# Sudaraka88/LDWeaver

Hardware: NVIDIA B200
Metric: weighted SNP-pair MI/sec (higher is better)
Workload: dtype int8 (tcgen05 kind::i8 with int32 accumulation of 28-bit fixed-point weights; fp32 MI epilogue, fp64 refinement of long-range links)

## Files before the change

include/ldw.h:

```cpp
#ifndef LDW_H
#define LDW_H

#include <stddef.h>
#include <stdint.h>

#ifdef __cplusplus
extern "C" {
#endif

#define LDW_ABI_VERSION 2

#if defined(__GNUC__)
#define LDW_API __attribute__((visibility("default")))
#else
#define LDW_API
#endif

enum {
  LDW_OK = 0,
  LDW_ERR_ARG = 1,
  LDW_ERR_CUDA = 2,
  LDW_ERR_NOMEM = 3,
  LDW_ERR_UNSUPPORTED = 4,
  LDW_ERR_INTERNAL = 5
};

enum {
  LDW_SCAN_SR_ONLY = 1,
  LDW_SCAN_IDEAL_Q = 2,
  LDW_SCAN_NO_LINKS = 4,
  LDW_SCAN_NO_D2H = 8,
  LDW_SCAN_SR_EXACT = 16,
  LDW_SCAN_SR_ON_DEVICE = 64,
  LDW_SCAN_LR_ONLY = 32
};

typedef struct ldw_ctx ldw_ctx;
typedef struct ldw_mi_plan ldw_mi_plan;

LDW_API int ldw_abi_version(void);
LDW_API const char* ldw_last_error(void);

LDW_API int ldw_create(int device, ldw_ctx** out);
LDW_API void ldw_destroy(ldw_ctx* ctx);
LDW_API int ldw_device_count(void);

LDW_API int ldw_aln_param(ldw_ctx* ctx, const uint8_t* aln, int64_t nseq, int64_t seq_len, int filter, double gap_thresh,
                  double maf_thresh, int32_t* pos_out, int64_t* n_snp_out, double* counts_out);
LDW_API int ldw_extract_snps(ldw_ctx* ctx, const uint8_t* aln, int64_t nseq, int64_t seq_len, const int32_t* pos,
                     int64_t n_snp, uint8_t* codes_out, double* table_out);
LDW_API int ldw_encode_alignment(ldw_ctx* ctx, const uint8_t* aln, int64_t nseq, int64_t seq_len, int filter, double gap_thresh,
                         double maf_thresh, int64_t* n_snp_out, int32_t** pos_out, uint8_t** codes_out, double** table_out);
LDW_API int ldw_read_fasta(const char* path, int64_t* nseq_out, int64_t* seq_len_out, uint8_t* aln_out, int64_t aln_cap,
                   char* names_out, int64_t names_cap);
LDW_API int ldw_read_fasta_alloc(const char* path, int64_t* nseq_out, int64_t* seq_len_out, uint8_t** aln_out, char** names_out,
                         int64_t* names_len_out);
LDW_API void ldw_buffer_free(void* p);

LDW_API int ldw_acgtn2num(ldw_ctx* ctx, double* nv, const char* ref, int64_t n);

LDW_API int ldw_hdw(ldw_ctx* ctx, const uint8_t* codes, int64_t n_snp, int64_t nseq, double threshold, int32_t* cnt_out,
            double* hdw_out, int32_t* dist_out);

typedef struct ldw_links {
  int64_t n;
  const int32_t* pos1;
  const int32_t* pos2;
  const int32_t* clust1;
  const int32_t* clust2;
  const int32_t* len;
  const double* MI;
  const int32_t* block;
} ldw_links;

typedef struct ldw_scan_stats {
  int64_t n_blocks;
  int64_t n_pairs;
  int64_t n_sr;
  int64_t n_lr_total;
  int64_t n_lr_kept;
  int64_t n_borderline;
  int64_t n_reruns;
  int64_t n_candidates;
  double t_pack_ms, t_scan_ms, t_select_ms, t_d2h_ms;
  double t_kernel_ms;
  int64_t n_scan_launches;
  int64_t n_launches;
  int64_t n_tiles;
  double exec_int8_ops;
  double t_host_prep_ms;
  double exec_mufu_ops;
  double eps_obs_max;
} ldw_scan_stats;

LDW_API int ldw_mi_plan_create(ldw_ctx* ctx, const uint8_t* codes, int64_t n_snp, int64_t nseq, const double* hdw,
                       const int32_t* pos, const int32_t* paint, int64_t blk, ldw_mi_plan** out);
LDW_API void ldw_mi_plan_destroy(ldw_mi_plan* plan);

LDW_API int ldw_mi_scan(ldw_mi_plan* plan, double g, double sr_dist, double lr_retain_links, double lr_links_approx,
                int flags, int n_parts, int part, ldw_links* sr_out, ldw_links* lr_out, ldw_links* borderline_out,
                double* thr_out, double* prob_out, ldw_scan_stats* stats_out);

LDW_API int ldw_write_lr_tsv(const char* path, const ldw_links* lr, int append);
LDW_API int ldw_format_r_real(double x, char* out, int cap);

typedef struct ldw_sr_post {
  int64_t n_df;
  const int32_t* clust_c;
  const int64_t* row;
  const double* srp_max;
  int64_t n_red;
  const int64_t* red;
  int64_t n_chk;
  const int64_t* chk;
  int32_t nclust;
  const int64_t* fit_off;
  const int32_t* fit_len;
  const double* fit_q95;
  const double* fit_val;
  const double* coef;
  const double* shape;
  const double* start;
  const int64_t* n_pos;
  const int32_t* nm_evals;
  const int32_t* nm_fail;
  void* priv;
} ldw_sr_post;
LDW_API int ldw_sr_postprocess(const ldw_links* sr, int32_t nclust, double sr_dist, double srp_cutoff, ldw_sr_post* out);
LDW_API void ldw_sr_post_free(ldw_sr_post* p);

LDW_API int ldw_sr_postprocess_dev(ldw_ctx* ctx, int32_t nclust, double sr_dist, double srp_cutoff, ldw_sr_post* out, ldw_links* df_rows_out);

LDW_API int ldw_nm_rosenbrock(const double* start, double* par_out, double* value_out, int* count_out);
LDW_API int ldw_neg_log_pbeta_upper(const double* x, int64_t n, double shape1, double shape2, double* out);

LDW_API int ldw_run_aracne(int64_t n_chk, const double* chk_pos1, const double* chk_pos2, const double* chk_MI, int64_t n_full,
                   const double* full_pos1, const double* full_pos2, const double* full_MI, uint8_t* aracne_out);

LDW_API int ldw_write_sr_tsv(const char* path, const ldw_links* sr, int64_t n, const int64_t* rows, const int32_t* clust_c,
                     const double* srp_max, const double* aracne, int append);

LDW_API int ldw_read_numeric_tsv(const char* path, int ncols, int64_t* nrows_out, double** cols_out);
LDW_API void ldw_table_free(double* cols);

LDW_API int ldw_links_to_cells(const int32_t* pos, int64_t n_snp, int64_t blk, const ldw_links* links, int32_t* from_local,
                       int32_t* to_local);

LDW_API int ldw_links_copy(const ldw_links* src, int32_t* pos1, int32_t* pos2, int32_t* clust1, int32_t* clust2, int32_t* len,
                   double* MI, int32_t* block);

LDW_API int ldw_mi_block_dense(ldw_mi_plan* plan, int64_t block_index, double* mi_out, int64_t* nf_out, int64_t* nt_out);

LDW_API int ldw_mi_pairs_exact(ldw_mi_plan* plan, int64_t block_index, const int32_t* from_local, const int32_t* to_local,
                       int64_t n_pairs, double* mi_out);

typedef struct ldw_group ldw_group;
#define LDW_GROUP_ID_BYTES 128
enum { LDW_HDW_FORCE_SHARD = 1 };
LDW_API int ldw_group_create(const int* devices, int n_devices, ldw_group** out);
LDW_API int ldw_group_unique_id(char* id_out );
LDW_API int ldw_group_create_rank(int device, int rank, int world, const char* id , ldw_group** out);
LDW_API void ldw_group_destroy(ldw_group* g);
LDW_API int ldw_group_info(const ldw_group* g, int* world_out, int* n_local_out, int* first_rank_out);
LDW_API ldw_ctx* ldw_group_ctx(ldw_group* g, int local_index);
LDW_API int ldw_group_load_codes(ldw_group* g, const uint8_t* codes, int64_t n_snp, int64_t nseq);
LDW_API int ldw_group_hdw(ldw_group* g, double threshold, int flags, int32_t* cnt_out, double* hdw_out, int* sharded_out);
LDW_API int ldw_group_mi_scan(ldw_group* g, const double* hdw, const int32_t* pos, const int32_t* paint, int64_t blk, double g_len,
                      double sr_dist, double lr_retain_links, double lr_links_approx, int flags, ldw_links* sr_out,
                      ldw_links* lr_out, ldw_links* borderline_out, double* thr_out, double* prob_out,
                      ldw_scan_stats* stats_out, double* t_plan_ms_out);

#ifdef __cplusplus
}
#endif
#endif
```

ldweaver_b200/_lib.py:

```python
from __future__ import annotations

import ctypes as C
import os

import numpy as np

_HERE = os.path.dirname(os.path.abspath(__file__))
LIB_PATH = os.environ.get("LDW_LIBRARY_PATH") or os.path.join(_HERE, "libldwgpu.so")

i64 = C.c_int64
f64 = C.c_double
P = C.POINTER


class LdwError(RuntimeError):
    def __init__(self, code: int, msg: str):
        super().__init__(f"libldwgpu error {code}: {msg}")
        self.code = code


class Links(C.Structure):
    _fields_ = [("n", i64), ("pos1", P(C.c_int32)), ("pos2", P(C.c_int32)), ("clust1", P(C.c_int32)),
                ("clust2", P(C.c_int32)), ("len", P(C.c_int32)), ("MI", P(f64)), ("block", P(C.c_int32))]

    @classmethod
    def from_dict(cls, d: dict):
        self = cls()
        keep = {}
        for name, dt, ct in (("pos1", np.int32, C.c_int32), ("pos2", np.int32, C.c_int32), ("clust1", np.int32, C.c_int32),
                             ("clust2", np.int32, C.c_int32), ("len", np.int32, C.c_int32), ("MI", np.float64, f64),
                             ("block", np.int32, C.c_int32)):
            a = np.ascontiguousarray(d[name] if name in d else np.zeros(len(d["MI"]), dtype=dt), dtype=dt)
            keep[name] = a
            setattr(self, name, a.ctypes.data_as(P(ct)))
        self.n = len(keep["MI"])
        self._keep = keep
        return self

    def views(self) -> dict:
        if hasattr(self, "_keep"):
            return self._keep
        n = int(self.n)
        out = {}
        for name, _ in self._fields_[1:]:
            ptr = getattr(self, name)
            if n and ptr:
                out[name] = np.ctypeslib.as_array(ptr, shape=(n,))
        return out

    def to_dict(self) -> dict:
        n = int(self.n)
        cols = (("pos1", np.int32), ("pos2", np.int32), ("clust1", np.int32), ("clust2", np.int32), ("len", np.int32),
                ("MI", np.float64), ("block", np.int32))
        out = {name: np.empty(n if (n and getattr(self, name)) else 0, dtype=dt) for name, dt in cols}
        if n:
            dst = [out[name].ctypes.data_as(C.c_void_p) if len(out[name]) else None for name, _ in cols]
            check(lib().ldw_links_copy(C.byref(self), *dst))
        return out


class ScanStats(C.Structure):
    _fields_ = [("n_blocks", i64), ("n_pairs", i64), ("n_sr", i64), ("n_lr_total", i64), ("n_lr_kept", i64),
                ("n_borderline", i64), ("n_reruns", i64), ("n_candidates", i64), ("t_pack_ms", f64), ("t_scan_ms", f64), ("t_select_ms", f64),
                ("t_d2h_ms", f64), ("t_kernel_ms", f64), ("n_scan_launches", i64), ("n_launches", i64), ("n_tiles", i64),
                ("exec_int8_ops", f64), ("t_host_prep_ms", f64), ("exec_mufu_ops", f64), ("eps_obs_max", f64)]

    def to_dict(self) -> dict:
        return {k: getattr(self, k) for k, _ in self._fields_}


class SrPost(C.Structure):
    _fields_ = [("n_df", i64), ("clust_c", P(C.c_int32)), ("row", P(i64)), ("srp_max", P(f64)),
                ("n_red", i64), ("red", P(i64)), ("n_chk", i64), ("chk", P(i64)), ("nclust", C.c_int32),
                ("fit_off", P(i64)), ("fit_len", P(C.c_int32)), ("fit_q95", P(f64)), ("fit_val", P(f64)),
                ("coef", P(f64)), ("shape", P(f64)), ("start", P(f64)), ("n_pos", P(i64)), ("nm_evals", P(C.c_int32)),
                ("nm_fail", P(C.c_int32)), ("priv", C.c_void_p)]


def copy_array(ptr, n: int, dtype) -> np.ndarray:
    if n == 0 or not ptr:
        return np.zeros(0, dtype=dtype)
    return np.ctypeslib.as_array(ptr, shape=(n,)).astype(dtype, copy=True)


_lib = None


def lib():
    global _lib
    if _lib is not None:
        return _lib
    if not os.path.exists(LIB_PATH):
        raise ImportError(f"{LIB_PATH} not found: build it with `python -c 'import __graft_entry__ as g; g.build()'`. "
                          "ldweaver_b200 has no CPU fallback.")
    L = C.CDLL(LIB_PATH)
    L.ldw_last_error.restype = C.c_char_p
    L.ldw_create.argtypes = [C.c_int, P(C.c_void_p)]
    L.ldw_destroy.argtypes = [C.c_void_p]
    L.ldw_destroy.restype = None
    L.ldw_aln_param.argtypes = [C.c_void_p, C.c_void_p, i64, i64, C.c_int, f64, f64, C.c_void_p, P(i64), C.c_void_p]
    L.ldw_extract_snps.argtypes = [C.c_void_p, C.c_void_p, i64, i64, C.c_void_p, i64, C.c_void_p, C.c_void_p]
    L.ldw_encode_alignment.argtypes = [C.c_void_p, C.c_void_p, i64, i64, C.c_int, f64, f64, P(i64), P(C.c_void_p), P(C.c_void_p),
                                       P(C.c_void_p)]
    L.ldw_read_fasta.argtypes = [C.c_char_p, P(i64), P(i64), C.c_void_p, i64, C.c_void_p, i64]
    L.ldw_read_fasta_alloc.argtypes = [C.c_char_p, P(i64), P(i64), P(C.c_void_p), P(C.c_void_p), P(i64)]
    L.ldw_buffer_free.argtypes = [C.c_void_p]
    L.ldw_buffer_free.restype = None
    L.ldw_acgtn2num.argtypes = [C.c_void_p, C.c_void_p, C.c_char_p, i64]
    L.ldw_hdw.argtypes = [C.c_void_p, C.c_void_p, i64, i64, f64, C.c_void_p, C.c_void_p, C.c_void_p]
    L.ldw_mi_plan_create.argtypes = [C.c_void_p, C.c_void_p, i64, i64, C.c_void_p, C.c_void_p, C.c_void_p, i64,
                                     P(C.c_void_p)]
    L.ldw_mi_plan_destroy.argtypes = [C.c_void_p]
    L.ldw_mi_plan_destroy.restype = None
    L.ldw_mi_scan.argtypes = [C.c_void_p, f64, f64, f64, f64, C.c_int, C.c_int, C.c_int, P(Links), P(Links), P(Links),
                              C.c_void_p, C.c_void_p, P(ScanStats)]
    L.ldw_mi_block_dense.argtypes = [C.c_void_p, i64, C.c_void_p, P(i64), P(i64)]
    L.ldw_write_lr_tsv.argtypes = [C.c_char_p, P(Links), C.c_int]
    L.ldw_format_r_real.argtypes = [f64, C.c_char_p, C.c_int]
    L.ldw_sr_postprocess.argtypes = [P(Links), C.c_int32, f64, f64, P(SrPost)]
    L.ldw_sr_postprocess_dev.argtypes = [C.c_void_p, C.c_int32, f64, f64, P(SrPost), P(Links)]
    L.ldw_sr_post_free.argtypes = [P(SrPost)]
    L.ldw_sr_post_free.restype = None
    L.ldw_run_aracne.argtypes = [i64, C.c_void_p, C.c_void_p, C.c_void_p, i64, C.c_void_p, C.c_void_p, C.c_void_p, C.c_void_p]
    L.ldw_write_sr_tsv.argtypes = [C.c_char_p, P(Links), i64, C.c_void_p, C.c_void_p, C.c_void_p, C.c_void_p, C.c_int]
    L.ldw_read_numeric_tsv.argtypes = [C.c_char_p, C.c_int, P(i64), P(P(f64))]
    L.ldw_table_free.argtypes = [P(f64)]
    L.ldw_table_free.restype = None
    L.ldw_links_to_cells.argtypes = [C.c_void_p, i64, i64, P(Links), C.c_void_p, C.c_void_p]
    L.ldw_links_copy.argtypes = [P(Links)] + [C.c_void_p] * 7
    L.ldw_nm_rosenbrock.argtypes = [C.c_void_p, C.c_void_p, P(f64), P(C.c_int)]
    L.ldw_neg_log_pbeta_upper.argtypes = [C.c_void_p, i64, f64, f64, C.c_void_p]
    L.ldw_mi_pairs_exact.argtypes = [C.c_void_p, i64, C.c_void_p, C.c_void_p, i64, C.c_void_p]
    L.ldw_group_create.argtypes = [C.c_void_p, C.c_int, P(C.c_void_p)]
    L.ldw_group_unique_id.argtypes = [C.c_char_p]
    L.ldw_group_create_rank.argtypes = [C.c_int, C.c_int, C.c_int, C.c_char_p, P(C.c_void_p)]
    L.ldw_group_destroy.argtypes = [C.c_void_p]
    L.ldw_group_destroy.restype = None
    L.ldw_group_info.argtypes = [C.c_void_p, P(C.c_int), P(C.c_int), P(C.c_int)]
    L.ldw_group_ctx.argtypes = [C.c_void_p, C.c_int]
    L.ldw_group_ctx.restype = C.c_void_p
    L.ldw_group_load_codes.argtypes = [C.c_void_p, C.c_void_p, i64, i64]
    L.ldw_group_hdw.argtypes = [C.c_void_p, f64, C.c_int, C.c_void_p, C.c_void_p, P(C.c_int)]
    L.ldw_group_mi_scan.argtypes = [C.c_void_p, C.c_void_p, C.c_void_p, C.c_void_p, i64, f64, f64, f64, f64, C.c_int,
                                    P(Links), P(Links), P(Links), C.c_void_p, C.c_void_p, C.c_void_p, P(f64)]
    _lib = L
    return L


_nccl_preloaded = False


def preload_nccl() -> None:
    global _nccl_preloaded
    if _nccl_preloaded:
        return
    _nccl_preloaded = True
    try:
        import importlib.util
        spec = importlib.util.find_spec("nvidia.nccl")
        for base in (spec.submodule_search_locations if spec and spec.submodule_search_locations else []):
            so = os.path.join(base, "lib", "libnccl.so.2")
            if os.path.exists(so):
                C.CDLL(so, mode=C.RTLD_GLOBAL)
                return
    except Exception:
        pass


def check(rc: int) -> None:
    if rc != 0:
        raise LdwError(rc, lib().ldw_last_error().decode(errors="replace"))


def ptr(a: np.ndarray):
    return a.ctypes.data_as(C.c_void_p)


class Context:

    def __init__(self, device: int = 0):
        self.handle = C.c_void_p()
        check(lib().ldw_create(device, C.byref(self.handle)))
        self.device = device

    def close(self):
        if self.handle:
            lib().ldw_destroy(self.handle)
            self.handle = C.c_void_p()

    def __del__(self):
        try:
            self.close()
        except Exception:
            pass


_default_ctx = {}


def default_context(device: int = 0) -> Context:
    if device not in _default_ctx:
        _default_ctx[device] = Context(device)
    return _default_ctx[device]
```

ldweaver_b200/api.py:

```python
from __future__ import annotations

import ctypes as C
import os
import warnings
from dataclasses import dataclass
from typing import List, Optional, Sequence

import numpy as np

from . import _lib
from ._lib import check, ptr

ALLELES = "ACGTN"


@dataclass
class SnpDat:
    codes: np.ndarray
    g: Optional[int]
    nsnp: int
    nseq: int
    seq_names: List[str]
    r: np.ndarray
    uqe: np.ndarray
    POS: np.ndarray

    def snp_matrix(self, allele: str):
        import scipy.sparse as sp
        return sp.csc_matrix(self.codes == ALLELES.index(allele))

    @property
    def snp_matrix_A(self): return self.snp_matrix("A")
    @property
    def snp_matrix_C(self): return self.snp_matrix("C")
    @property
    def snp_matrix_G(self): return self.snp_matrix("G")
    @property
    def snp_matrix_T(self): return self.snp_matrix("T")
    @property
    def snp_matrix_N(self): return self.snp_matrix("N")


def _method_to_filter(method: str) -> int:
    if method == "default":
        return 0
    if method == "relaxed":
        return 1
    warnings.warn("Unkown filtering method, using default...")
    return 0


class _LibraryBuffer:

    def __init__(self, addr: int, nbytes: int):
        self._addr = addr
        self.__array_interface__ = {"data": (addr, False), "shape": (nbytes,), "typestr": "|u1", "version": 3}

    def __del__(self):
        try:
            _lib.lib().ldw_buffer_free(self._addr)
        except Exception:
            pass


def read_fasta_matrix(aln_path: str):
    L = _lib.lib()
    nseq, slen, nlen = C.c_int64(), C.c_int64(), C.c_int64()
    aln_p, names_p = C.c_void_p(), C.c_void_p()
    check(L.ldw_read_fasta_alloc(os.fsencode(aln_path), C.byref(nseq), C.byref(slen), C.byref(aln_p), C.byref(names_p), C.byref(nlen)))
    try:
        raw = C.string_at(names_p, nlen.value) if names_p else b""
    finally:
        L.ldw_buffer_free(names_p)
    owner = _LibraryBuffer(aln_p.value, nseq.value * max(slen.value, 0)) if aln_p else None
    if slen.value == -1:
        raise ValueError("Error! sequences are of different lengths!")
    if nseq.value == 0:
        raise ValueError("File does not contain any sequences!")
    if owner is None:
        aln = np.empty((nseq.value, 0), dtype=np.uint8)
    else:
        aln = np.asarray(owner).reshape(nseq.value, slen.value)
    name_list = raw.split(b"\0")[:nseq.value]
    return [n.decode(errors="replace") for n in name_list], aln


def _build_snp_dat(aln: np.ndarray, names: Sequence[str], filt: int, gap_freq: float, maf_freq: float,
                   pos: Optional[np.ndarray], device: int) -> SnpDat:
    L = _lib.lib()
    ctx = _lib.default_context(device)
    aln = np.ascontiguousarray(aln, dtype=np.uint8)
    nseq, slen = aln.shape
    n_snp = C.c_int64()
    pos_p, codes_p, table_p = C.c_void_p(), C.c_void_p(), C.c_void_p()
    check(L.ldw_encode_alignment(ctx.handle, ptr(aln), nseq, slen, filt, gap_freq, maf_freq, C.byref(n_snp), C.byref(pos_p),
                                 C.byref(codes_p), C.byref(table_p)))
    n = int(n_snp.value)
    if n == 0:
        raise ValueError("File does not contain any SNPs")
    if pos is not None and len(pos) != slen:
        for p_ in (pos_p, codes_p, table_p):
            L.ldw_buffer_free(p_)
        raise ValueError("Error! Number of positions do not match the fasta sequence length")
    try:
        pos_idx = np.frombuffer(C.string_at(pos_p, n * 4), dtype=np.int32).copy()
        table = np.frombuffer(C.string_at(table_p, n * 5 * 8), dtype=np.float64).copy()
    finally:
        L.ldw_buffer_free(pos_p)
        L.ldw_buffer_free(table_p)
    codes = np.asarray(_LibraryBuffer(codes_p.value, n * nseq)).reshape(n, nseq)
    table = table.reshape(n, 5)
    uqe = (table > 0).astype(np.float64)
    if pos is None:
        POS, g = pos_idx.astype(np.int32), int(slen)
    else:
        POS, g = np.asarray(pos)[pos_idx.astype(np.int64) - 1].astype(np.int32), None
    return SnpDat(codes=codes, g=g, nsnp=n, nseq=int(nseq), seq_names=[s.lstrip(">") for s in names],
                  r=uqe.sum(axis=1), uqe=uqe, POS=POS)


def parse_fasta_alignment(aln_path: str, gap_freq: float = 0.15, maf_freq: float = 0.01, method: str = "default",
                          mega_dset: bool = False, device: int = 0) -> SnpDat:
    aln_path = os.path.abspath(os.path.expanduser(aln_path))
    if not os.path.exists(aln_path):
        raise FileNotFoundError(f"Can't locate file {aln_path}")
    filt = _method_to_filter(method)
    names, aln = read_fasta_matrix(aln_path)
    return _build_snp_dat(aln, names, filt, gap_freq, maf_freq, None, device)


def parse_fasta_SNP_alignment(aln_path: str, pos: Sequence[int], gap_freq: float = 0.15, maf_freq: float = 0.01,
                              method: str = "default", mega_dset: bool = False, device: int = 0) -> SnpDat:
    aln_path = os.path.abspath(os.path.expanduser(aln_path))
    if not os.path.exists(aln_path):
        raise FileNotFoundError(f"Can't locate file {aln_path}")
    filt = _method_to_filter(method)
    names, aln = read_fasta_matrix(aln_path)
    return _build_snp_dat(aln, names, filt, gap_freq, maf_freq, np.asarray(pos), device)


def snp_dat_from_alignment_matrix(aln: np.ndarray, names: Optional[Sequence[str]] = None, pos=None, gap_freq=0.15,
                                  maf_freq=0.01, method="default", device: int = 0) -> SnpDat:
    names = list(names) if names is not None else [f"s{i}" for i in range(aln.shape[0])]
    return _build_snp_dat(aln, names, _method_to_filter(method), gap_freq, maf_freq,
                          None if pos is None else np.asarray(pos), device)


def snp_dat_from_codes(codes: np.ndarray, POS: np.ndarray, g: Optional[int], seq_names=None) -> SnpDat:
    codes = np.ascontiguousarray(codes, dtype=np.uint8)
    nsnp, nseq = codes.shape
    uqe = np.stack([(codes == a).any(axis=1) for a in range(5)], axis=1).astype(np.float64)
    return SnpDat(codes=codes, g=g, nsnp=nsnp, nseq=nseq, seq_names=list(seq_names) if seq_names is not None else
                  [f"s{i}" for i in range(nseq)], r=uqe.sum(axis=1), uqe=uqe, POS=np.asarray(POS, dtype=np.int32))


def acgtn2num(nv: np.ndarray, cv, ncores: int = 1, device: int = 0) -> None:
    if not (nv.dtype == np.float64 and nv.flags["F_CONTIGUOUS"] and nv.shape[0] == 5):
        raise ValueError("nv must be a Fortran-ordered float64 [5, n] matrix (R column-major)")
    ref = "".join((c[0] if len(c) else " ") for c in cv).encode("latin-1") if not isinstance(cv, (bytes, bytearray)) else bytes(cv)
    if len(ref) != nv.shape[1]:
        raise ValueError("cv length does not match ncol(nv)")
    ctx = _lib.default_context(device)
    check(_lib.lib().ldw_acgtn2num(ctx.handle, ptr(nv), ref, nv.shape[1]))


def estimate_Hamming_distance_weights(snp_dat: SnpDat, threshold: float = 0.1, mega_dset: bool = False,
                                      device: int = 0, return_parts: bool = False, devices: Optional[Sequence[int]] = None):
    if devices is None and not return_parts:
        devices = devices_from_env()
    if devices is not None and len(devices) > 1:
        if return_parts:
            raise ValueError("the distance matrix (return_parts) is a single-device output")
        grp = default_group(devices)
        grp.load_codes(snp_dat.codes)
        return grp.hdw(threshold)
    ctx = _lib.default_context(device)
    codes = np.ascontiguousarray(snp_dat.codes, dtype=np.uint8)
    n, S = codes.shape
    cnt = np.empty(S, dtype=np.int32)
    hdw = np.empty(S, dtype=np.float64)
    dist = np.empty((S, S), dtype=np.int32, order="F") if return_parts else None
    check(_lib.lib().ldw_hdw(ctx.handle, ptr(codes), n, S, float(threshold), ptr(cnt), ptr(hdw),
                             ptr(dist) if return_parts else None))
    if return_parts:
        return hdw, cnt, dist
    return hdw


SCAN_SR_ONLY, SCAN_IDEAL_Q, SCAN_NO_LINKS, SCAN_NO_D2H, SCAN_SR_EXACT, SCAN_LR_ONLY, SCAN_SR_ON_DEVICE = 1, 2, 4, 8, 16, 32, 64


@dataclass
class CdsVar:
    paint: np.ndarray
    nclust: int


@dataclass
class MIScanResult:
    sr: dict
    lr: dict
    borderline: dict
    nclust: int
    thr: np.ndarray
    prob: np.ndarray
    stats: dict
    lr_links_approx: Optional[float]
    sr_links_red: Optional[dict] = None
    sr_post: Optional["SrLinks"] = None
    _by_cluster: Optional[List[np.ndarray]] = None

    @property
    def sr_links(self) -> List[np.ndarray]:
        if self._by_cluster is None:
            self._by_cluster = [np.nonzero((self.sr["clust1"] == c) | (self.sr["clust2"] == c))[0]
                                for c in range(1, self.nclust + 1)]
        return self._by_cluster


def round_half_even_thousands(x: float) -> int:
    return int(np.round(x / 1000.0) * 1000)


def make_blocks(nsnp: int, max_blk_sz: int):
    import math
    p = int(math.ceil(nsnp / max_blk_sz))
    fs = [(i - 1) * max_blk_sz + 1 for i in range(1, p + 1)]
    fe = [min(i * max_blk_sz, nsnp) for i in range(1, p + 1)]
    return [(fs[i], fe[i], fs[j], fe[j]) for i in range(p) for j in range(i, p)]


def partition_blocks(nsnp: int, blk: int, n_parts: int, part: int) -> List[int]:
    if n_parts < 1 or not (0 <= part < n_parts):
        raise ValueError("bad partition")
    items = []
    for idx, (fs, fe, ts, te) in enumerate(make_blocks(nsnp, blk)):
        ni, nj = fe - fs + 1, te - ts + 1
        items.append((ni * (ni - 1) // 2 if fs == ts else ni * nj, idx))
    load = [0] * n_parts
    owner = {}
    for cost, idx in sorted(items, key=lambda t: (-t[0], t[1])):
        best = min(range(n_parts), key=lambda p: (load[p], p))
        owner[idx] = best
        load[best] += cost
    return [idx for _, idx in items if owner[idx] == part]


def sr_pair_indices(pos: np.ndarray, blk: int, sr: dict):
    pos = np.asarray(pos)
    blocks = make_blocks(len(pos), blk)
    b = np.asarray(sr["block"])
    n = len(b)
    links = _lib.Links.from_dict({"pos1": sr["pos1"], "pos2": sr["pos2"], "block": b, "MI": np.zeros(n)})
    pos32 = np.ascontiguousarray(pos, dtype=np.int32)
    il, jl = np.zeros(n, dtype=np.int32), np.zeros(n, dtype=np.int32)
    check(_lib.lib().ldw_links_to_cells(ptr(pos32), len(pos32), int(blk), C.byref(links), ptr(il), ptr(jl)))
    if n == 0 or np.all(b[1:] >= b[:-1]):
        order = None
        bounds = np.searchsorted(b, np.arange(len(blocks) + 1))
    else:
        order = np.argsort(b, kind="stable")
        bounds = np.searchsorted(b[order], np.arange(len(blocks) + 1))
    for k in range(len(blocks)):
        if bounds[k + 1] > bounds[k]:
            idx = slice(int(bounds[k]), int(bounds[k + 1])) if order is None else order[bounds[k]:bounds[k + 1]]
            yield k, idx, il[idx], jl[idx]


class MIPlan:

    def __init__(self, snp_dat: SnpDat, hdw: np.ndarray, paint: np.ndarray, blk: int, device: int = 0):
        self.ctx = _lib.default_context(device)
        self.codes = np.ascontiguousarray(snp_dat.codes, dtype=np.uint8)
        self.hdw = np.ascontiguousarray(hdw, dtype=np.float64)
        self.pos = np.ascontiguousarray(snp_dat.POS, dtype=np.int32)
        self.paint = np.ascontiguousarray(paint, dtype=np.int32)
        n, S = self.codes.shape
        if len(self.hdw) != S or len(self.pos) != n or len(self.paint) != n:
            raise ValueError("snp.dat / hdw / cds_var size mismatch")
        self.n, self.S, self.blk = n, S, int(blk)
        self.handle = C.c_void_p()
        check(_lib.lib().ldw_mi_plan_create(self.ctx.handle, ptr(self.codes), n, S, ptr(self.hdw), ptr(self.pos),
                                            ptr(self.paint), int(blk), C.byref(self.handle)))
        nr = -(-n // self.blk)
        self.n_blocks = nr * (nr + 1) // 2

    def close(self):
        if self.handle:
            _lib.lib().ldw_mi_plan_destroy(self.handle)
            self.handle = C.c_void_p()

    def __del__(self):
        try:
            self.close()
        except Exception:
            pass

    def scan(self, g: float, sr_dist: float, lr_retain_links: float, lr_links_approx: float, flags: int = 0,
             n_parts: int = 1, part: int = 0, copy: bool = True):
        sr, lr, bd = _lib.Links(), _lib.Links(), _lib.Links()
        thr = np.full(self.n_blocks, np.nan)
        prob = np.full(self.n_blocks, np.nan)
        st = _lib.ScanStats()
        check(_lib.lib().ldw_mi_scan(self.handle, float(g), float(sr_dist), float(lr_retain_links),
                                     float(lr_links_approx if lr_links_approx else 0.0), int(flags), int(n_parts), int(part),
                                     C.byref(sr), C.byref(lr), C.byref(bd), ptr(thr), ptr(prob), C.byref(st)))
        if copy:
            return sr.to_dict(), lr.to_dict(), bd.to_dict(), thr, prob, st.to_dict()
        return sr, lr, bd, thr, prob, st.to_dict()

    def sr_exact(self, sr: dict, inplace: bool = False) -> np.ndarray:
        mi = sr["MI"]
        if inplace and isinstance(mi, np.ndarray) and mi.dtype == np.float64 and mi.flags.c_contiguous and mi.flags.writeable:
            out = mi
        else:
            out = np.array(mi, dtype=np.float64, copy=True)
        for k, idx, il, jl in sr_pair_indices(self.pos, self.blk, sr):
            if isinstance(idx, slice):
                self.pairs_exact(k, il, jl, out=out[idx])
            else:
                out[idx] = self.pairs_exact(k, il, jl)
        return out

    def block_dense(self, block_index: int) -> np.ndarray:
        nf, nt = C.c_int64(), C.c_int64()
        check(_lib.lib().ldw_mi_block_dense(self.handle, block_index, None, C.byref(nf), C.byref(nt)))
        out = np.zeros((nf.value, nt.value), dtype=np.float64, order="F")
        check(_lib.lib().ldw_mi_block_dense(self.handle, block_index, ptr(out), C.byref(nf), C.byref(nt)))
        return out

    def pairs_exact(self, block_index: int, from_local: np.ndarray, to_local: np.ndarray, out: Optional[np.ndarray] = None) -> np.ndarray:
        f = np.ascontiguousarray(from_local, dtype=np.int32)
        t = np.ascontiguousarray(to_local, dtype=np.int32)
        if out is None:
            out = np.zeros(len(f), dtype=np.float64)
        elif not (out.dtype == np.float64 and out.flags.c_contiguous and out.flags.writeable and out.shape == (len(f),)):
            raise ValueError("out must be a writeable C-contiguous float64 array with one element per pair")
        check(_lib.lib().ldw_mi_pairs_exact(self.handle, block_index, ptr(f), ptr(t), len(f), ptr(out)))
        return out


def _format_r(x) -> str:
    x = float(x)
    if x != x:
        return "NA"
    if x in (float("inf"), float("-inf")):
        return "Inf" if x > 0 else "-Inf"
    if x == 0:
        return "0"
    m, e = f"{x:.14e}".split("e")
    neg = m.startswith("-")
    digits = m.lstrip("-").replace(".", "").rstrip("0") or "0"
    nsig, k = len(digits), int(e)
    left, rgt = (k + 1, max(0, nsig - k - 1)) if k >= 0 else (1, nsig - k - 1)
    if 0 < k <= 22 and abs(x) < 10.0 ** k:
        left -= 1
    w_fixed = neg + left + (rgt + 1 if rgt else 0)
    w_sci = neg + (nsig + 1 if nsig > 1 else 1) + (5 if abs(k) >= 100 else 4)
    return f"{x:.{rgt}f}" if w_fixed <= w_sci else f"{x:.{nsig - 1}e}"


def format_r_real_native(x: float) -> str:
    buf = C.create_string_buffer(512)
    check(_lib.lib().ldw_format_r_real(float(x), buf, 512))
    return buf.value.decode()


def write_lr_tsv(path: str, lr, append: bool = True) -> None:
    links = lr if isinstance(lr, _lib.Links) else _lib.Links.from_dict(lr)
    check(_lib.lib().ldw_write_lr_tsv(os.fsencode(path), C.byref(links), 1 if append else 0))


class DeviceGroup:

    def __init__(self, devices: Sequence[int]):
        devs = np.ascontiguousarray(list(devices), dtype=np.int32)
        self.handle = C.c_void_p()
        if len(devs) > 1:
            _lib.preload_nccl()
        check(_lib.lib().ldw_group_create(ptr(devs), len(devs), C.byref(self.handle)))
        self._after_create()

    def _after_create(self):
        w, nl, fr = C.c_int(), C.c_int(), C.c_int()
        check(_lib.lib().ldw_group_info(self.handle, C.byref(w), C.byref(nl), C.byref(fr)))
        self.world, self.n_local, self.first_rank = w.value, nl.value, fr.value
        self.n_snp = self.nseq = 0

    @staticmethod
    def unique_id() -> bytes:
        buf = C.create_string_buffer(128)
        _lib.preload_nccl()
        check(_lib.lib().ldw_group_unique_id(buf))
        return buf.raw

    @classmethod
    def from_rank(cls, device: int, rank: int, world: int, unique_id: Optional[bytes]):
        self = cls.__new__(cls)
        self.handle = C.c_void_p()
        _lib.preload_nccl()
        check(_lib.lib().ldw_group_create_rank(int(device), int(rank), int(world), unique_id, C.byref(self.handle)))
        self._after_create()
        return self

    def close(self):
        if getattr(self, "handle", None):
            _lib.lib().ldw_group_destroy(self.handle)
            self.handle = C.c_void_p()

    def __del__(self):
        try:
            self.close()
        except Exception:
            pass

    def load_codes(self, codes: Optional[np.ndarray], n_snp: Optional[int] = None, nseq: Optional[int] = None) -> None:
        if codes is not None:
            codes = np.ascontiguousarray(codes, dtype=np.uint8)
            n_snp, nseq = codes.shape
        check(_lib.lib().ldw_group_load_codes(self.handle, ptr(codes) if codes is not None else None, int(n_snp), int(nseq)))
        self.n_snp, self.nseq = int(n_snp), int(nseq)

    def hdw(self, threshold: float = 0.1, force_shard: bool = False, return_parts: bool = False):
        cnt = np.empty(self.nseq, dtype=np.int32)
        w = np.empty(self.nseq, dtype=np.float64)
        sharded = C.c_int()
        check(_lib.lib().ldw_group_hdw(self.handle, float(threshold), 1 if force_shard else 0, ptr(cnt), ptr(w), C.byref(sharded)))
        return (w, cnt, bool(sharded.value)) if return_parts else w

    def mi_scan(self, hdw, pos, paint, blk: int, g: float, sr_dist: float, lr_retain_links: float, lr_links_approx: float,
                flags: int = 0, copy: bool = True):
        hdw = np.ascontiguousarray(hdw, dtype=np.float64)
        pos = np.ascontiguousarray(pos, dtype=np.int32)
        paint = np.ascontiguousarray(paint, dtype=np.int32)
        if len(hdw) != self.nseq or len(pos) != self.n_snp or len(paint) != self.n_snp:
            raise ValueError("hdw / POS / paint do not match the matrix given to load_codes")
        nr = -(-self.n_snp // int(blk))
        nblk = nr * (nr + 1) // 2
        sr, lr, bd = _lib.Links(), _lib.Links(), _lib.Links()
        thr, prob = np.full(nblk, np.nan), np.full(nblk, np.nan)
        stats = (_lib.ScanStats * self.n_local)()
        t_plan = _lib.f64()
        check(_lib.lib().ldw_group_mi_scan(self.handle, ptr(hdw), ptr(pos), ptr(paint), int(blk), float(g), float(sr_dist),
                                           float(lr_retain_links), float(lr_links_approx if lr_links_approx else 0.0), int(flags),
                                           C.byref(sr), C.byref(lr), C.byref(bd), ptr(thr), ptr(prob), stats, C.byref(t_plan)))
        st = [s_.to_dict() for s_ in stats]
        for d in st:
            d["t_plan_ms"] = t_plan.value
        if copy:
            return sr.to_dict(), lr.to_dict(), bd.to_dict(), thr, prob, st
        return sr, lr, bd, thr, prob, st


_groups = {}


def default_group(devices: Sequence[int]) -> DeviceGroup:
    key = tuple(int(d) for d in devices)
    if key not in _groups:
        _groups[key] = DeviceGroup(key)
    return _groups[key]


def devices_from_env() -> Optional[List[int]]:
    v = os.environ.get("LDW_GPUS", "").strip()
    if not v:
        return None
    if "," in v:
        return [int(x) for x in v.split(",") if x.strip() != ""]
    n = int(v)
    return list(range(n)) if n > 1 else None


@dataclass
class SrLinks:
    df: dict
    red: np.ndarray
    chk: np.ndarray
    fits: List[dict]
    borderline_red: Optional[np.ndarray] = None
    borderline_chk: Optional[np.ndarray] = None


def _unpack_sr_post(out, nclust: int, cols: dict, row_is_position: bool, plt_path: Optional[str], srp_cutoff: float) -> SrLinks:
    cp = _lib.copy_array
    row = cp(out.row, out.n_df, np.int64)
    df = {"clust_c": cp(out.clust_c, out.n_df, np.int32), "row": row, "srp_max": cp(out.srp_max, out.n_df, np.float64)}
    for k in ("pos1", "pos2", "clust1", "clust2", "len", "MI"):
        df[k] = np.array(cols[k], copy=True) if row_is_position else np.asarray(cols[k])[row]
    off = cp(out.fit_off, nclust + 1, np.int64)
    nfit = int(off[-1])
    fl, fq, fv = cp(out.fit_len, nfit, np.int32), cp(out.fit_q95, nfit, np.float64), cp(out.fit_val, nfit, np.float64)
    coef, shape, start = (cp(x, 2 * nclust, np.float64).reshape(nclust, 2) for x in (out.coef, out.shape, out.start))
    npos, ev, fail = cp(out.n_pos, nclust, np.int64), cp(out.nm_evals, nclust, np.int32), cp(out.nm_fail, nclust, np.int32)
    fits = [dict(len=fl[off[c]:off[c + 1]], max=fq[off[c]:off[c + 1]], fit=fv[off[c]:off[c + 1]], coef=coef[c],
                 shape=shape[c], start=start[c], n_pos=int(npos[c]), nm_evals=int(ev[c]), nm_fail=int(fail[c]))
            for c in range(nclust)]
    if plt_path is not None:
        os.makedirs(plt_path, exist_ok=True)
        for c, f in enumerate(fits, start=1):
            with open(os.path.join(plt_path, f"c{c}_fit_data.tsv"), "w") as fh:
                fh.write("len\tmax\tfit\n")
                fh.writelines(f"{int(a)}\t{b:.15g}\t{v:.15g}\n" for a, b, v in zip(f["len"], f["max"], f["fit"]))
    red, chk = cp(out.red, out.n_red, np.int64), cp(out.chk, out.n_chk, np.int64)
    b_red = np.nonzero(np.abs(df["srp_max"] - srp_cutoff) <= 1e-9 * max(abs(float(srp_cutoff)), 1.0))[0]
    b_chk = np.nonzero(np.abs(df["MI"] - df["MI"][red].min()) <= 1e-12)[0] if len(red) else np.zeros(0, np.int64)
    return SrLinks(df=df, red=red, chk=chk, fits=fits, borderline_red=b_red, borderline_chk=b_chk)


def mergeNsort_sr_links(cds_var, sr_links, sr_dist: float, plt_path: Optional[str] = None, srp_cutoff: float = 3) -> SrLinks:
    nclust = int(cds_var.nclust if hasattr(cds_var, "nclust") else cds_var["nclust"])
    links = sr_links if isinstance(sr_links, _lib.Links) else _lib.Links.from_dict(sr_links)
    out = _lib.SrPost()
    check(_lib.lib().ldw_sr_postprocess(C.byref(links), nclust, float(sr_dist), float(srp_cutoff), C.byref(out)))
    try:
        return _unpack_sr_post(out, nclust, links.views(), False, plt_path, srp_cutoff)
    finally:
        _lib.lib().ldw_sr_post_free(C.byref(out))


def mergeNsort_sr_links_device(cds_var, sr_dist: float, plt_path: Optional[str] = None, srp_cutoff: float = 3, device: int = 0) -> SrLinks:
    nclust = int(cds_var.nclust if hasattr(cds_var, "nclust") else cds_var["nclust"])
    ctx = _lib.default_context(device)
    out, rows = _lib.SrPost(), _lib.Links()
    check(_lib.lib().ldw_sr_postprocess_dev(ctx.handle, nclust, float(sr_dist), float(srp_cutoff), C.byref(out), C.byref(rows)))
    try:
        return _unpack_sr_post(out, nclust, rows.views() if int(rows.n) else {k: np.zeros(0) for k in ("pos1", "pos2", "clust1", "clust2", "len", "MI")},
                               True, plt_path, srp_cutoff)
    finally:
        _lib.lib().ldw_sr_post_free(C.byref(out))


def runARACNE(links_to_check, links_full) -> np.ndarray:
    f64 = lambda a: np.ascontiguousarray(np.asarray(a), dtype=np.float64)
    c1, c2, cm = f64(links_to_check["pos1"]), f64(links_to_check["pos2"]), f64(links_to_check["MI"])
    p1, p2, pm = f64(links_full["pos1"]), f64(links_full["pos2"]), f64(links_full["MI"])
    out = np.ones(len(c1), dtype=np.uint8)
    check(_lib.lib().ldw_run_aracne(len(c1), ptr(c1), ptr(c2), ptr(cm), len(p1), ptr(p1), ptr(p2), ptr(pm), ptr(out)))
    return out.astype(bool)


def write_sr_tsv(path: str, sr, rows: np.ndarray, clust_c: np.ndarray, srp_max: np.ndarray, aracne: np.ndarray,
                 append: bool = True) -> None:
    links = sr if isinstance(sr, _lib.Links) else _lib.Links.from_dict(sr)
    rows = np.ascontiguousarray(rows, dtype=np.int64)
    cc = np.ascontiguousarray(clust_c, dtype=np.int32)
    sp = np.ascontiguousarray(srp_max, dtype=np.float64)
    ar = np.ascontiguousarray(aracne, dtype=np.float64)
    check(_lib.lib().ldw_write_sr_tsv(os.fsencode(path), C.byref(links), len(rows), ptr(rows), ptr(cc), ptr(sp), ptr(ar),
                                      1 if append else 0))


def _read_numeric_tsv(path: str, names: Sequence[str]) -> dict:
    n, cols = _lib.i64(0), _lib.P(_lib.f64)()
    check(_lib.lib().ldw_read_numeric_tsv(os.fsencode(path), len(names), C.byref(n), C.byref(cols)))
    try:
        flat = _lib.copy_array(cols, int(n.value) * len(names), np.float64).reshape(len(names), int(n.value))
    finally:
        _lib.lib().ldw_table_free(cols)
    return {k: flat[i] for i, k in enumerate(names)}


def read_LongRangeLinks(lr_links_path: str, links_from_spydrpick: bool = False, sr_dist: float = 20000) -> dict:
    if links_from_spydrpick:
        tab = np.loadtxt(lr_links_path, dtype=np.float64, ndmin=2)
        names = {5: ["pos1", "pos2", "len", "ARACNE", "MI"], 4: ["pos1", "pos2", "len", "MI"]}.get(tab.shape[1])
        if names is None:
            raise ValueError(f"spydrpick link files have 4 or 5 columns, {lr_links_path} has {tab.shape[1]}")
        d = {k: np.ascontiguousarray(tab[:, i]) for i, k in enumerate(names)}
    else:
        d = _read_numeric_tsv(lr_links_path, ["pos1", "pos2", "c1", "c2", "len", "MI"])
    keep = ~(d["len"] < sr_dist)
    return {k: v[keep] for k, v in d.items()} if not keep.all() else d


def read_ShortRangeLinks(sr_links_path: str) -> dict:
    return _read_numeric_tsv(sr_links_path, ["clust_c", "pos1", "pos2", "clust1", "clust2", "len", "MI", "srp_max", "ARACNE"])


def _quantile7(x: np.ndarray, prob: float) -> float:
    n = len(x)
    index = 1 + max(n - 1, 0) * prob
    lo, hi = int(np.floor(index)), int(np.ceil(index))
    part = np.partition(x, sorted({lo - 1, hi - 1}))
    qs = float(part[lo - 1])
    if index > lo and part[hi - 1] != qs:
        h = index - lo
        qs = (1 - h) * qs + h * float(part[hi - 1])
    return qs


def analyse_long_range_links(lr_links: dict, sr_links: dict, are_lrlinks_ordered: bool = False) -> dict:
    mi = np.asarray(lr_links["MI"], dtype=np.float64)
    q1, q3 = _quantile7(mi, 0.25), _quantile7(mi, 0.75)
    thresholds = q3 + np.array([1.5, 3.0]) * (q3 - q1)
    red = mi > thresholds.min()
    if red.sum() < 5000 and len(mi) >= 5000:
        import warnings
        warnings.warn("Not enough lr links pass the Tukey criteria, ~5000 top links were retained instead")
        thresholds = np.array([_quantile7(mi, 1 - (1 / len(mi) * k)) for k in (4000, 5000)])
        red = mi > thresholds.min()
    out = {k: np.asarray(v)[red] for k, v in lr_links.items()}
    if "ARACNE" not in lr_links:
        chk = {k: np.concatenate([np.asarray(lr_links[k], dtype=np.float64), np.asarray(sr_links[k], dtype=np.float64)])
               for k in ("pos1", "pos2", "MI")}
        m = chk["MI"] > thresholds.min()
        out["ARACNE"] = runARACNE(out, {k: v[m] for k, v in chk.items()})
    if not are_lrlinks_ordered:
        o = np.argsort(-out["MI"], kind="stable")
        out = {k: v[o] for k, v in out.items()}
    out["thresholds"] = thresholds
    return out


def finish_sr_links(sr: Optional[dict], cds_var, sr_dist: float, srp_cutoff: float = 3, run_aracne: bool = True,
                    order_links: bool = True, sr_save_path: Optional[str] = None, plt_folder: Optional[str] = None,
                    post: Optional[SrLinks] = None):
    if post is None:
        post = mergeNsort_sr_links(cds_var, sr, sr_dist, plt_folder, srp_cutoff)
    red = {k: v[post.red] for k, v in post.df.items()}
    if run_aracne:
        chk = {k: post.df[k][post.chk] for k in ("pos1", "pos2", "MI")}
        red["ARACNE"] = runARACNE(red, chk).astype(np.float64)
    else:
        import warnings
        warnings.warn("ARACNE not run, all values will be set to 1")
        red["ARACNE"] = np.ones(len(post.red))
    if order_links:
        o = np.argsort(-red["srp_max"], kind="stable")
        red = {k: v[o] for k, v in red.items()}
    if sr_save_path is not None:
        write_sr_tsv(sr_save_path, red, np.arange(len(red["row"]), dtype=np.int64), red["clust_c"], red["srp_max"], red["ARACNE"], append=True)
    return red, post


def perform_MI_computation(snp_dat: SnpDat, hdw: np.ndarray, cds_var, ncores: int = 1, lr_save_path: Optional[str] = None,
                           sr_save_path: Optional[str] = None, plt_folder: Optional[str] = None, sr_dist: float = 20000,
                           lr_retain_links: float = 1e6, max_blk_sz: float = 10000, srp_cutoff: float = 3,
                           runARACNE: bool = True, perform_SR_analysis_only: bool = False, order_links: bool = True,
                           mega_dset: bool = False, lr_links_approx: Optional[float] = None, device: int = 0,
                           write_tsv: bool = True, plan: Optional[MIPlan] = None,
                           postprocess: Optional[bool] = None, exact_sr: Optional[bool] = None,
                           devices: Optional[Sequence[int]] = None, scan_flags: int = 0,
                           device_post: bool = False) -> MIScanResult:
    if snp_dat.g is None:
        raise ValueError("snp.dat$g is NULL: set the genome length first (R/BacGWES.R:338-345)")
    paint = np.asarray(cds_var.paint if hasattr(cds_var, "paint") else cds_var["paint"])
    nclust = int(cds_var.nclust if hasattr(cds_var, "nclust") else cds_var["nclust"])
    if lr_save_path is None:
        lr_save_path = os.path.join(os.getcwd(), "lr_links.tsv")
    blk = round_half_even_thousands(max_blk_sz)
    if not perform_SR_analysis_only and lr_links_approx is None:
        from .rrng import lr_links_approx as _lra
        lr_links_approx = _lra(np.asarray(snp_dat.POS), float(snp_dat.g), float(sr_dist))
    if devices is None and plan is None:
        devices = devices_from_env()
    multi = devices is not None and len(devices) > 1
    do_post = postprocess if postprocess is not None else write_tsv
    if multi:
        grp = default_group(devices)
        grp.load_codes(snp_dat.codes)
        flags = (SCAN_SR_ONLY if perform_SR_analysis_only else 0) | int(scan_flags)
        if exact_sr is None:
            exact_sr = do_post
        if exact_sr:
            flags |= SCAN_SR_EXACT
        sr, lr, bd, thr, prob, st_list = grp.mi_scan(hdw, snp_dat.POS, paint, blk, float(snp_dat.g), sr_dist, lr_retain_links,
                                                     lr_links_approx or 0.0, flags)
        stats = dict(st_list[0])
        for k in ("n_blocks", "n_pairs", "n_sr", "n_lr_total", "n_lr_kept", "n_borderline", "n_reruns", "n_candidates",
                  "n_scan_launches", "n_launches", "n_tiles", "exec_int8_ops", "exec_mufu_ops"):
            stats[k] = sum(d[k] for d in st_list)
        for k in ("t_pack_ms", "t_scan_ms", "t_select_ms", "t_d2h_ms", "t_kernel_ms", "t_host_prep_ms"):
            stats[k] = max(d[k] for d in st_list)
        stats["per_device"] = st_list
        return _finish_mi_computation(sr, lr, bd, thr, prob, stats, nclust, lr_links_approx, cds_var, sr_dist, srp_cutoff,
                                      runARACNE, order_links, write_tsv, do_post, lr_save_path, sr_save_path, plt_folder)
    own = plan is None
    import time as _time
    t_phase = {}
    _t0 = _time.perf_counter()
    if own:
        plan = MIPlan(snp_dat, hdw, paint, blk, device)
    t_phase["plan_create_s"] = _time.perf_counter() - _t0
    try:
        flags = (SCAN_SR_ONLY if perform_SR_analysis_only else 0) | int(scan_flags)
        if exact_sr is None:
            exact_sr = ("in_scan" if perform_SR_analysis_only else True) if do_post else False
        if device_post and do_post:
            flags |= SCAN_SR_ON_DEVICE
            if exact_sr:
                exact_sr = "in_scan"
        if exact_sr == "in_scan":
            flags |= SCAN_SR_EXACT
            exact_sr = False
        _t0 = _time.perf_counter()
        sr, lr, bd, thr, prob, stats = plan.scan(float(snp_dat.g), sr_dist, lr_retain_links, lr_links_approx or 0.0, flags, copy=False)
        t_phase["scan_call_s"] = _time.perf_counter() - _t0
        _t0 = _time.perf_counter()
        sr, lr, bd = sr.to_dict(), lr.to_dict(), bd.to_dict()
        t_phase["copy_links_s"] = _time.perf_counter() - _t0
        if exact_sr:
            if perform_SR_analysis_only:
                raise ValueError("exact_sr is not available with perform_SR_analysis_only")
            _t0 = _time.perf_counter()
            sr["MI"] = plan.sr_exact(sr, inplace=True)
            t_phase["exact_sr_host_driven_s"] = _time.perf_counter() - _t0
    finally:
        if own:
            plan.close()
    stats["phases"] = t_phase
    post = None
    if device_post and do_post:
        _t0 = _time.perf_counter()
        post = mergeNsort_sr_links_device(cds_var, sr_dist, plt_folder, srp_cutoff, device)
        t_phase["sr_post_device_s"] = _time.perf_counter() - _t0
    return _finish_mi_computation(sr, lr, bd, thr, prob, stats, nclust, lr_links_approx, cds_var, sr_dist, srp_cutoff,
                                  runARACNE, order_links, write_tsv, do_post, lr_save_path, sr_save_path, plt_folder, post)


def _finish_mi_computation(sr, lr, bd, thr, prob, stats, nclust, lr_links_approx, cds_var, sr_dist, srp_cutoff, run_aracne,
                           order_links, write_tsv, do_post, lr_save_path, sr_save_path, plt_folder, post=None) -> MIScanResult:
    import time as _time
    ph = stats.setdefault("phases", {})
    _t0 = _time.perf_counter()
    if write_tsv and len(lr["MI"]):
        write_lr_tsv(lr_save_path, lr, append=True)
    ph["write_lr_tsv_s"] = _time.perf_counter() - _t0
    _t0 = _time.perf_counter()
    res = MIScanResult(sr=sr, lr=lr, borderline=bd, nclust=nclust, thr=thr, prob=prob, stats=stats,
                       lr_links_approx=lr_links_approx)
    if do_post:
        if write_tsv and sr_save_path is None:
            sr_save_path = os.path.join(os.getcwd(), "sr_links.tsv")
        res.sr_links_red, res.sr_post = finish_sr_links(sr, cds_var, sr_dist, srp_cutoff, run_aracne, order_links,
                                                        sr_save_path if write_tsv else None, plt_folder, post)
    ph["finish_sr_links_s"] = _time.perf_counter() - _t0
    return res
```

ldweaver_b200/csrc/mi_kernel.cuh:

```cuda
#pragma once
#include "mi_types.h"
#include "umma.cuh"

namespace ldw {

constexpr int MI_EXP_WARPS = 6;
constexpr int MI_EXP_THREADS = 32 * MI_EXP_WARPS;
constexpr int MI_EPI_WARP0 = 8;
constexpr int MI_EPI_GROUPS = 4;
constexpr int MI_EPI_WARPS = 4 * MI_EPI_GROUPS;
constexpr int MI_EPI_THREADS = 32 * MI_EPI_WARPS;
constexpr int MI_THREADS = 32 * (MI_EPI_WARP0 + MI_EPI_WARPS);
#define LDW_STR2(x) #x
#define LDW_STR(x) LDW_STR2(x)
#define MI_REGS_CTRL 48
#define MI_REGS_EPI 96
static_assert(MI_EPI_WARP0 * 32 * MI_REGS_CTRL + MI_EPI_THREADS * MI_REGS_EPI <= MI_THREADS * ((65536 / MI_THREADS) & ~7), "register budget");
constexpr int MI_MAX_STAGES = 4;
constexpr uint32_t MI_ARR_BYTES = 128 * 128;
constexpr uint32_t MI_STAGE_REGION = 12 * MI_ARR_BYTES;
__host__ __device__ constexpr uint32_t mi_stage_need(int pa, int pb, int njlog2) {
  return (uint32_t)pa * MI_ARR_BYTES + 4u * (uint32_t)pb * (64u << njlog2);
}
__host__ __device__ constexpr int mi_stage_geo(int pa, int pb, int njlog2) {
  return mi_stage_need(pa, pb, njlog2) <= 3 * MI_ARR_BYTES ? 0 : mi_stage_need(pa, pb, njlog2) <= 4 * MI_ARR_BYTES ? 1 : 2;
}
__host__ __device__ constexpr int mi_geo_stages(int geo) { return 4 - geo; }
__host__ __device__ constexpr uint32_t mi_geo_bytes(int geo) { return geo == 0 ? 3 * MI_ARR_BYTES : geo == 1 ? 4 * MI_ARR_BYTES : 6 * MI_ARR_BYTES; }
constexpr uint32_t MI_JREC_BYTES = 128 * sizeof(Rec);
constexpr uint32_t MI_JDYN_BYTES = 128 * sizeof(ColDyn);
constexpr uint32_t MI_IREC_BYTES = 128 * sizeof(Rec);
constexpr uint32_t MI_IDYN_BYTES = 128 * sizeof(RowDyn);
constexpr uint32_t MI_BAR_BYTES = 512;
constexpr uint32_t MI_SMEM_BYTES = MI_STAGE_REGION + 2 * (MI_JREC_BYTES + MI_JDYN_BYTES) + MI_IREC_BYTES + MI_IDYN_BYTES + MI_BAR_BYTES + 1024;
static_assert(MI_SMEM_BYTES <= 232448, "shared memory budget (227 KB opt-in)");

__device__ __forceinline__ float lg2_fast(float x) {
  float y;
  asm("lg2.approx.ftz.f32 %0, %1;" : "=f"(y) : "f"(x));
  return y;
}
__device__ __forceinline__ uint32_t ld_volatile_u32(const uint32_t* p) {
  uint32_t v;
  asm volatile("ld.volatile.global.u32 %0, [%1];" : "=r"(v) : "l"(p));
  return v;
}

__host__ __device__ constexpr int mi_jc(int pa, int pb) {
  return (pa + 1) * (pb + 1) <= 4 ? 8 : (pa + 1) * (pb + 1) <= 9 ? 4 : (pa + 1) * (pb + 1) <= 12 ? 2 : 1;
}
__host__ __device__ constexpr int mi_njlog2(int pa, int pb) {
  return pa * pb == 1 ? 7 : pa * pb == 2 ? 6 : pa * pb <= 4 ? 5 : 4;
}

__device__ __noinline__ void lr_raise_threshold(const ScanParams& p, int lane) {
  constexpr int PER = MI_HIST_BINS / 32;
  uint32_t s = 0;
  for (int k = 0; k < PER; k++) s += ld_volatile_u32(p.hist + lane * PER + k);
  uint32_t suf = s;
#pragma unroll
  for (int o = 1; o < 32; o <<= 1) {
    uint32_t v = __shfl_down_sync(0xffffffffu, suf, o);
    if (lane + o < 32) suf += v;
  }
  unsigned m = __ballot_sync(0xffffffffu, suf >= p.kprime);
  if (m == 0) return;
  int sel = 31 - __clz(m);
  if (lane == sel) {
    uint32_t run = suf - s;
    for (int k = PER - 1; k >= 0; k--) {
      run += ld_volatile_u32(p.hist + lane * PER + k);
      if (run >= p.kprime) {
        atomicMax(p.tcand_bits, (uint32_t)(lane * PER + k) << 19);
        break;
      }
    }
  }
}

template <bool DBG>
__device__ __forceinline__ void timed_wait(uint64_t* bar, uint32_t parity, int tag, long long& acc) {
  if constexpr (DBG) {
    long long c0 = clock64();
    mbar_wait(bar, parity, tag);
    acc += clock64() - c0;
  } else {
    mbar_wait(bar, parity, tag);
  }
}

struct EpiCtx {
  int q, cg, lane, rank;
  uint32_t tflags;
  uint32_t tmem_base;
  uint32_t jrec_saddr;
  uint32_t jdyn_saddr;
  uint32_t irec_saddr, idyn_saddr;
  uint32_t rempty_saddr;
  uint32_t scr_saddr;
};

__device__ __forceinline__ uint4 lds128(uint32_t saddr) {
  uint4 v;
  asm volatile("ld.shared.v4.u32 {%0, %1, %2, %3}, [%4];" : "=r"(v.x), "=r"(v.y), "=r"(v.z), "=r"(v.w) : "r"(saddr));
  return v;
}

__device__ __forceinline__ uint2 lds64(uint32_t saddr) {
  uint2 v;
  asm volatile("ld.shared.v2.u32 {%0, %1}, [%2];" : "=r"(v.x), "=r"(v.y) : "r"(saddr));
  return v;
}

__device__ __forceinline__ void sts128(uint32_t saddr, uint4 v) {
  asm volatile("st.shared.v4.u32 [%0], {%1, %2, %3, %4};" ::"r"(saddr), "r"(v.x), "r"(v.y), "r"(v.z), "r"(v.w) : "memory");
}

__device__ __forceinline__ float rcp_fast(float x) {
  float y;
  asm("rcp.approx.ftz.f32 %0, %1;" : "=f"(y) : "f"(x));
  return y;
}

template <bool QC>
__device__ __forceinline__ float mi_term(float acc, uint32_t t, float ra, float rb, float dq) {
  const float x = __uint2float_rn(t);
  const float ratio = QC ? x * rcp_fast(fmaf(ra, rb, dq)) : x * (ra * rb);
  return fmaf(x, lg2_fast(ratio), acc);
}

template <bool QC, int NB>
__device__ __forceinline__ float mi_row(float acc, const uint32_t (&t)[NB], float ra, const float (&rb)[NB], float dq) {
  if constexpr (!QC) {
#pragma unroll
    for (int b = 0; b < NB; b++) acc = mi_term<false>(acc, t[b], ra, rb[b], dq);
    return acc;
  } else {
    float d[NB], inv[NB];
#pragma unroll
    for (int b = 0; b < NB; b++) d[b] = fmaf(ra, rb[b], dq);
#pragma unroll
    for (int b = 0; b + 1 < NB; b += 2) {
      const float r = rcp_fast(d[b] * d[b + 1]);
      inv[b] = r * d[b + 1];
      inv[b + 1] = r * d[b];
    }
    if (NB & 1) inv[NB - 1] = rcp_fast(d[NB - 1]);
#pragma unroll
    for (int b = 0; b < NB; b++) {
      const float x = __uint2float_rn(t[b]);
      acc = fmaf(x, lg2_fast(x * inv[b]), acc);
    }
    return acc;
  }
}

__device__ __noinline__ void lr_emit(const ScanParams& p, bool em, int il, int jl, float mi, int lane) {
  const unsigned bal = __ballot_sync(0xffffffffu, em);
  if (bal == 0) return;
  const int leader = __ffs(bal) - 1;
  uint32_t base = 0;
  const uint32_t n_new = (uint32_t)__popc(bal);
  if (lane == leader) base = atomicAdd(p.cand_count, n_new);
  base = __shfl_sync(0xffffffffu, base, leader);
  if (em) {
    uint32_t idx = base + (uint32_t)__popc(bal & ((1u << lane) - 1));
    if (idx < p.cand_cap) {
      Cand cc;
      cc.il = il; cc.jl = jl; cc.mi = mi;
      p.cand[idx] = cc;
    } else {
      *p.overflow = 1;
    }
    uint32_t bits = __float_as_uint(mi);
    atomicAdd(p.hist + ((bits & 0x80000000u) ? 0u : (bits >> 19)), 1u);
  }
  if (!p.emit_all && (base / p.delta) != ((base + n_new) / p.delta)) {
    __threadfence();
    lr_raise_threshold(p, lane);
  }
}

__device__ __noinline__ void sr_store(float* sr_out, uint4 d0, uint4 d1, int il, int jl, float mi) {
  const int a0 = (int)d0.z, a1 = (int)d0.w, b0 = (int)d1.x, b1 = (int)d1.y;
  const int la = a1 - a0, lb = b1 - b0;
  int below = min(max(il - a0, 0), la) + min(max(il - b0, 0), lb);
  uint32_t slot;
  if (il < jl) {
    slot = d1.z + (uint32_t)below;
  } else {
    int bj = min(max(jl + 1 - a0, 0), la) + min(max(jl + 1 - b0, 0), lb);
    slot = d1.w + (uint32_t)(below - bj);
  }
  sr_out[slot] = mi;
}

template <int RA>
struct TileRegs {
  uint32_t Ti[RA];
  float rpad[RA];
  float scale, q0, qod, rtlq, tcand;
  uint32_t mul_a, sb, jl_lim, M;
  int il, nf, nt;
  bool ragged, dense, do_lr, has_sr;
  float* sr_out;
};

template <int PA, int PB, int JC>
__device__ __forceinline__ void epi_load(uint32_t tmem_base, int NJ, int j0, uint32_t (&H)[PA][PB][JC],
                                         uint32_t (&L)[PA][PB][JC]) {
  const int NJh = NJ >> 1;
  const int half = j0 >= NJh ? 1 : 0;
  const uint32_t base = tmem_base + (uint32_t)(half * PB * NJ + (j0 - half * NJh));
#pragma unroll
  for (int a = 0; a < PA; a++)
#pragma unroll
    for (int b = 0; b < PB; b++) {
      tmem_ldn<JC>(base + (uint32_t)(a * 2 * PB * NJ + b * NJh), H[a][b]);
      tmem_ldn<JC>(base + (uint32_t)(a * 2 * PB * NJ + (PB + b) * NJh), L[a][b]);
    }
}

template <int PA, int PB, int JC>
__device__ __forceinline__ void epi_counts(const uint32_t (&H)[PA][PB][JC], const uint32_t (&L)[PA][PB][JC], uint32_t mul_a,
                                           uint32_t sb, uint32_t M, uint32_t (&T)[PA][PB][JC]) {
#pragma unroll
  for (int a = 0; a < PA; a++)
#pragma unroll
    for (int b = 0; b < PB; b++)
#pragma unroll
      for (int jj = 0; jj < JC; jj++) T[a][b][jj] = H[a][b][jj] * mul_a + ((L[a][b][jj] >> sb) + M);
}

template <int PA, int PB, int JC, bool QC, bool RG>
__device__ __forceinline__ void epi_batch(const ScanParams& p, const EpiCtx& c, const TileRegs<PA + 1>& k, int j0,
                                          const uint32_t (&T)[PA][PB][JC]) {
  constexpr int RB = PB + 1;
  uint32_t rpj[JC][RB];
  int jl[JC];
  float dq[JC];
#pragma unroll
  for (int jj = 0; jj < JC; jj++) {
    const uint32_t ra_ = c.jrec_saddr + (uint32_t)(j0 + jj) * (uint32_t)sizeof(Rec);
    const uint4 w1 = lds128(ra_ + (QC ? 32 : 16));
    uint32_t w4 = 0;
    if (RB == 5) asm volatile("ld.shared.u32 %0, [%1];" : "=r"(w4) : "r"(ra_ + (QC ? 56 : 52)));
    const uint32_t tr[5] = {w1.x, w1.y, w1.z, w1.w, w4};
#pragma unroll
    for (int b = 0; b < RB; b++) rpj[jj][b] = tr[b];
    const uint2 d0 = lds64(c.jdyn_saddr + (uint32_t)(j0 + jj) * (uint32_t)sizeof(ColDyn));
    jl[jj] = (int)d0.x;
    dq[jj] = 0.f;
    if (QC) {
      if (RG) {
        float v = k.q0;
        if (k.il >= 0 && jl[jj] >= 0) {
          uint64_t lin = (uint64_t)k.il + (uint64_t)jl[jj] * (uint64_t)k.nf;
          uint32_t cdiv = (uint32_t)(lin / (uint32_t)k.nt), cmod = (uint32_t)(lin % (uint32_t)k.nt);
          v = (float)p.rfl_arr[cdiv] * (float)p.rtl_arr[cmod] * k.qod;
        }
        dq[jj] = v - k.q0;
      } else {
        dq[jj] = fmaf(k.rtlq, __uint_as_float(d0.y), -k.q0);
      }
    }
  }
  float acc[JC];
  uint32_t col[JC][PB], tot[JC];
#pragma unroll
  for (int jj = 0; jj < JC; jj++) {
    acc[jj] = 0.f; tot[jj] = 0;
#pragma unroll
    for (int b = 0; b < PB; b++) col[jj][b] = 0;
  }
#pragma unroll
  for (int a = 0; a < PA; a++) {
    uint32_t row[JC][RB];
#pragma unroll
    for (int jj = 0; jj < JC; jj++) {
      uint32_t rsum = 0;
#pragma unroll
      for (int b = 0; b < PB; b++) {
        const uint32_t t = T[a][b][jj];
        rsum += t;
        col[jj][b] += t;
        row[jj][b] = t;
      }
      row[jj][PB] = k.Ti[a] - rsum;
      tot[jj] += rsum;
    }
#pragma unroll
    for (int jj = 0; jj < JC; jj++) {
      float rbv[RB];
#pragma unroll
      for (int b = 0; b < RB; b++) rbv[b] = __uint_as_float(rpj[jj][b]);
      acc[jj] = mi_row<QC, RB>(acc[jj], row[jj], k.rpad[a], rbv, dq[jj]);
    }
  }
#pragma unroll
  for (int jj = 0; jj < JC; jj++) {
    const uint4 w0 = lds128(c.jrec_saddr + (uint32_t)(j0 + jj) * (uint32_t)sizeof(Rec));
    const uint32_t tj[4] = {w0.x, w0.y, w0.z, w0.w};
    uint32_t row[RB], sj = 0;
    float rbv[RB];
#pragma unroll
    for (int b = 0; b < PB; b++) { row[b] = tj[b] - col[jj][b]; sj += tj[b]; }
#pragma unroll
    for (int b = 0; b < RB; b++) rbv[b] = __uint_as_float(rpj[jj][b]);
    const uint32_t rest = sj - tot[jj];
    row[PB] = k.Ti[PA] >= rest ? max(k.Ti[PA] - rest, k.M) : k.M;
    acc[jj] = mi_row<QC, RB>(acc[jj], row, k.rpad[PA], rbv, dq[jj]);
  }
  float mi[JC];
#pragma unroll
  for (int jj = 0; jj < JC; jj++) mi[jj] = acc[jj] * k.scale;
  if (k.dense) {
#pragma unroll
    for (int jj = 0; jj < JC; jj++)
      if (k.il >= 0 && jl[jj] >= 0) p.dense_out[(size_t)k.il + (size_t)jl[jj] * (size_t)k.nf] = mi[jj];
    return;
  }
  bool live[JC];
#pragma unroll
  for (int jj = 0; jj < JC; jj++) live[jj] = ((uint32_t)jl[jj] < k.jl_lim) && (jl[jj] != k.il);
  if (k.has_sr) {
#pragma unroll
    for (int jj = 0; jj < JC; jj++) {
      const uint4 d0 = lds128(c.jdyn_saddr + (uint32_t)(j0 + jj) * (uint32_t)sizeof(ColDyn));
      const uint4 d1 = lds128(c.jdyn_saddr + (uint32_t)(j0 + jj) * (uint32_t)sizeof(ColDyn) + 16);
      const uint32_t la = d0.w - d0.z, lb = d1.y - d1.x;
      const bool sr = live[jj] && (((uint32_t)k.il - d0.z < la) || ((uint32_t)k.il - d1.x < lb));
      if (sr) sr_store(k.sr_out, d0, d1, k.il, jl[jj], mi[jj]);
      live[jj] = live[jj] && !sr;
    }
  }
  if (k.do_lr) {
    bool any = false;
#pragma unroll
    for (int jj = 0; jj < JC; jj++) {
      live[jj] = live[jj] && (mi[jj] >= k.tcand);
      any = any || live[jj];
    }
    if (__any_sync(0xffffffffu, any)) {
#pragma unroll
      for (int jj = 0; jj < JC; jj++) lr_emit(p, live[jj], k.il, jl[jj], mi[jj], c.lane);
    }
  }
}

template <int PA, int PB, bool QC, bool RG, class Rel>
__device__ __forceinline__ void epi_tile(const ScanParams& p, const EpiCtx& c, Rel&& release_acc) {
  constexpr int RA = PA + 1, RB = PB + 1;
  constexpr int JC = mi_jc(PA, PB);
  constexpr int NJ = 1 << mi_njlog2(PA, PB);
  constexpr int NB = (NJ / MI_EPI_GROUPS) / JC;
  static_assert(NB >= 1 && NB * JC * MI_EPI_GROUPS == NJ, "column split must be exact");
  const int row = c.q * 32 + c.lane;
  TileRegs<RA> k;
  k.scale = p.scale[RA - 2][RB - 2]; k.q0 = p.q0s[RA - 2][RB - 2];
  k.qod = p.qod[RA - 2][RB - 2];
  k.M = p.M;
  k.nf = p.nf; k.nt = p.nt;
  k.mul_a = 1u << p.sa; k.sb = p.sb;
  k.ragged = p.ragged != 0; k.dense = p.dense != 0;
  k.do_lr = !p.sr_only && !p.dense;
  k.has_sr = (c.tflags & TILE_HAS_SR) != 0;
  k.sr_out = p.sr_out;
  k.tcand = (k.do_lr && !p.emit_all) ? __uint_as_float(ld_volatile_u32(p.tcand_bits)) : -3.0e38f;
  uint32_t r0, r1;
  {
    const uint32_t rv = c.irec_saddr + (uint32_t)row * (uint32_t)sizeof(Rec);
    const uint4 v0 = lds128(rv), v1 = lds128(rv + (QC ? 32 : 16));
    uint4 v3 = make_uint4(0, 0, 0, 0);
    if (RA == 5) v3 = lds128(rv + 48);
    asm volatile("ld.shared.v2.u32 {%0, %1}, [%2];" : "=r"(r0), "=r"(r1) : "r"(c.idyn_saddr + (uint32_t)row * (uint32_t)sizeof(RowDyn)));
    {
      const uint32_t dep = (v0.x ^ v0.y ^ v0.z ^ v0.w ^ v1.x ^ v1.y ^ v1.z ^ v1.w ^ v3.x ^ v3.y ^ v3.z ^ r0 ^ r1);
      asm volatile("st.volatile.shared.u32 [%0], %1;" ::"r"(c.scr_saddr), "r"(dep) : "memory");
      __syncwarp();
      if (c.lane == 0) asm volatile("mbarrier.arrive.shared::cta.b64 _, [%0];" ::"r"(c.rempty_saddr) : "memory");
    }
    const uint32_t tt[5] = {v0.x, v0.y, v0.z, v0.w, v3.x}, tr[5] = {v1.x, v1.y, v1.z, v1.w, QC ? v3.z : v3.y};
    const float rf = QC ? p.rp_qc[RA - 2][RB - 2] : p.rp_plain[RA - 2][RB - 2];
#pragma unroll
    for (int a = 0; a < RA; a++) {
      k.Ti[a] = tt[a];
      k.rpad[a] = __uint_as_float(tr[a]) * rf;
    }
  }
  k.il = (int)r0;
  k.rtlq = __uint_as_float(r1) * k.qod;
  k.jl_lim = k.il < 0 ? 0u : (p.diag ? (uint32_t)k.il : (uint32_t)p.nt);

  const int jbeg = c.cg * (NJ / MI_EPI_GROUPS);
  uint32_t H[PA][PB][JC], L[PA][PB][JC];
#pragma unroll 1
  for (int bi = 0; bi < NB; bi++) {
    const int j0 = jbeg + bi * JC;
    epi_load<PA, PB, JC>(c.tmem_base, NJ, j0, H, L);
    tmem_ld_wait();
    if (bi + 1 == NB) release_acc();
    uint32_t T[PA][PB][JC];
    epi_counts<PA, PB, JC>(H, L, k.mul_a, k.sb, k.M, T);
    epi_batch<PA, PB, JC, QC, RG>(p, c, k, j0, T);
  }
}

template <bool QC, bool RG, class Rel>
__device__ __forceinline__ void epi_dispatch(const ScanParams& p, int pa, int pb, const EpiCtx& c, Rel&& rel) {
  switch (pa * 4 + pb - 5) {
    case 0: epi_tile<1, 1, QC, RG>(p, c, rel); break;
    case 1: epi_tile<1, 2, QC, RG>(p, c, rel); break;
    case 2: epi_tile<1, 3, QC, RG>(p, c, rel); break;
    case 3: epi_tile<1, 4, QC, RG>(p, c, rel); break;
    case 4: epi_tile<2, 1, QC, RG>(p, c, rel); break;
    case 5: epi_tile<2, 2, QC, RG>(p, c, rel); break;
    case 6: epi_tile<2, 3, QC, RG>(p, c, rel); break;
    case 7: epi_tile<2, 4, QC, RG>(p, c, rel); break;
    case 8: epi_tile<3, 1, QC, RG>(p, c, rel); break;
    case 9: epi_tile<3, 2, QC, RG>(p, c, rel); break;
    case 10: epi_tile<3, 3, QC, RG>(p, c, rel); break;
    case 11: epi_tile<3, 4, QC, RG>(p, c, rel); break;
    case 12: epi_tile<4, 1, QC, RG>(p, c, rel); break;
    case 13: epi_tile<4, 2, QC, RG>(p, c, rel); break;
    case 14: epi_tile<4, 3, QC, RG>(p, c, rel); break;
    case 15: epi_tile<4, 4, QC, RG>(p, c, rel); break;
    default: break;
  }
}

template <bool DBG>
__global__ void __cluster_dims__(2, 1, 1) __launch_bounds__(MI_THREADS, 1)
mi_scan_kernel(const __grid_constant__ TmapSet tm, const __grid_constant__ ScanParams p) {
  extern __shared__ uint8_t smem_raw[];
  uint8_t* smem = reinterpret_cast<uint8_t*>((reinterpret_cast<uintptr_t>(smem_raw) + 1023) & ~(uintptr_t)1023);
  uint8_t* stage_base = smem;
  Rec* jrec = reinterpret_cast<Rec*>(smem + MI_STAGE_REGION);
  ColDyn* jdyn = reinterpret_cast<ColDyn*>(smem + MI_STAGE_REGION + 2 * MI_JREC_BYTES);
  Rec* irec = reinterpret_cast<Rec*>(smem + MI_STAGE_REGION + 2 * (MI_JREC_BYTES + MI_JDYN_BYTES));
  RowDyn* idyn = reinterpret_cast<RowDyn*>(smem + MI_STAGE_REGION + 2 * (MI_JREC_BYTES + MI_JDYN_BYTES) + MI_IREC_BYTES);
  uint64_t* bars = reinterpret_cast<uint64_t*>(smem + MI_STAGE_REGION + 2 * (MI_JREC_BYTES + MI_JDYN_BYTES) + MI_IREC_BYTES + MI_IDYN_BYTES);
  uint64_t* full = bars;
  uint64_t* empty = bars + 4;
  uint64_t* ready = bars + 8;
  uint64_t* tfull = bars + 12;
  uint64_t* tempty = bars + 14;
  uint64_t* jfull = bars + 16;
  uint64_t* jempty = bars + 18;
  uint64_t* drained = bars + 20;
  uint64_t* rfull = bars + 21;
  uint64_t* rempty = bars + 22;
  uint32_t* tmem_slot = reinterpret_cast<uint32_t*>(bars + 23);
  uint32_t* thdr = reinterpret_cast<uint32_t*>(bars + 24);

  const int warp = threadIdx.x >> 5, lane = threadIdx.x & 31;
  const uint32_t rank = cluster_ctarank();
  if (warp == 0 && lane == 0) {
    tma_prefetch_desc(&tm.a);
    for (int i = 0; i < MI_MAX_STAGES; i++) {
      mbar_init(&full[i], 1); mbar_init(&empty[i], 1); mbar_init(&ready[i], 2 * MI_EXP_WARPS);
    }
    mbar_init(drained, 1);
    mbar_init(rfull, 1); mbar_init(rempty, MI_EPI_WARPS);
    for (int i = 0; i < 2; i++) {
      mbar_init(&tfull[i], 1); mbar_init(&tempty[i], 2 * MI_EPI_WARPS);
      mbar_init(&jfull[i], 1); mbar_init(&jempty[i], MI_EPI_WARPS);
    }
    fence_barrier_init();
  }
  if (warp == 2) tmem_alloc_pair(tmem_slot, 512);
  tc_fence_before();
  cluster_sync_all();
  tc_fence_after();
  const uint32_t tmem_base = *tmem_slot;
  const int tile0 = (int)(blockIdx.x >> 1), tstep = (int)(gridDim.x >> 1);

  if (warp < MI_EPI_WARP0) {
  asm volatile("setmaxnreg.dec.sync.aligned.u32 " LDW_STR(MI_REGS_CTRL) ";");
  if (warp == 0) {
    int st = 0; uint32_t phb = 0; int geo = -1; uint32_t dph = 0;
    int it = 0, rit = 0;
    long long w_jempty = 0, w_empty = 0, t_begin = DBG ? clock64() : 0;
    for (int t = tile0; t < p.n_tiles; t += tstep, it++) {
      const TileDesc td = p.tiles[t];
      const int PA = td.PA, PB = td.PB, NJ = 1 << td.njlog2, NJh = NJ >> 1;
      const int njidx = 7 - td.njlog2;
      const int g = mi_stage_geo(PA, PB, td.njlog2);
      const int nst = mi_geo_stages(g);
      const uint32_t sbytes = mi_geo_bytes(g);
      if (g != geo) {
        if (geo >= 0) { mbar_wait(drained, dph, 12); dph ^= 1; }
        geo = g; st = 0;
      }
      {
        const uint32_t stage_tx = (uint32_t)PA * MI_ARR_BYTES + (uint32_t)(PB * NJh * 128);
        const int a_row = td.a_row0 + (int)rank * 128, b_row = td.b_row0 + (int)rank * NJh;
        for (int kb = 0; kb < p.nkb; kb++) {
          timed_wait<DBG>(&empty[st], ((phb >> st) & 1) ^ 1, 11, w_empty);
          if (elect_one()) {
            uint8_t* sb = stage_base + st * sbytes;
            mbar_arrive_expect_tx(&full[st], stage_tx);
            for (int a = 0; a < PA; a++)
              tma_load_2d(sb + a * MI_ARR_BYTES, &tm.a, &full[st], kb * 128, a_row + a * td.a_pstride);
            uint8_t* sbB = sb + PA * MI_ARR_BYTES;
            for (int b = 0; b < PB; b++)
              tma_load_2d(sbB + b * NJh * 128, &tm.b[njidx], &full[st], kb * 128, b_row + b * td.b_pstride);
          }
          __syncwarp();
          phb ^= 1u << st;
          if (++st == nst) st = 0;
        }
      }
      const int jb = it & 1;
      timed_wait<DBG>(&jempty[jb], ((it >> 1) & 1) ^ 1, 10, w_jempty);
      if (elect_one()) {
        thdr[jb] = (uint32_t)PA | ((uint32_t)PB << 8) | ((uint32_t)td.njlog2 << 16) | ((uint32_t)(rank ? td.flags1 : td.flags) << 24);
        mbar_arrive_expect_tx(&jfull[jb], (uint32_t)NJ * (uint32_t)(sizeof(Rec) + sizeof(ColDyn)));
        bulk_load_1d(jrec + jb * 128, p.rec + (int64_t)(PA + 1 - 2) * p.rec_vstride + td.j_slot0, NJ * sizeof(Rec), &jfull[jb]);
        bulk_load_1d(jdyn + jb * 128, p.coldyn + td.j_dyn0, NJ * sizeof(ColDyn), &jfull[jb]);
      }
      __syncwarp();
      if (!((rank ? td.flags1 : td.flags) & TILE_NULL)) {
        timed_wait<DBG>(rempty, (uint32_t)(rit & 1) ^ 1, 13, w_jempty);
        if (elect_one()) {
          mbar_arrive_expect_tx(rfull, MI_IREC_BYTES + MI_IDYN_BYTES);
          bulk_load_1d(irec, p.rec + (int64_t)(PB + 1 - 2) * p.rec_vstride + td.i_slot0 + (int)rank * 128, MI_IREC_BYTES, rfull);
          bulk_load_1d(idyn, p.rowdyn + td.i_dyn0 + (int)rank * 128, MI_IDYN_BYTES, rfull);
        }
        __syncwarp();
        rit++;
      }
    }
    if (DBG && p.dbg && lane == 0) {
      p.dbg[blockIdx.x * 16 + 0] = (unsigned long long)(clock64() - t_begin);
      p.dbg[blockIdx.x * 16 + 1] = (unsigned long long)w_jempty;
      p.dbg[blockIdx.x * 16 + 2] = (unsigned long long)w_empty;
    }
  } else if (warp == 1) {
    if (rank == 0) {
    int st = 0; uint32_t phb = 0; int geo = -1; int as = 0; uint32_t aph = 0;
    long long w_tempty = 0, w_ready = 0, t_begin = DBG ? clock64() : 0;
    const uint32_t desc_hi = (uint32_t)(make_smem_desc_sw128(0) >> 32);
    for (int t = tile0; t < p.n_tiles; t += tstep) {
      const TileDesc td = p.tiles[t];
      const int PA = td.PA, PB = td.PB, NJ = 1 << td.njlog2;
      const int g = mi_stage_geo(PA, PB, td.njlog2);
      const int nst = mi_geo_stages(g);
      const uint32_t sbytes = mi_geo_bytes(g);
      if (g != geo) { geo = g; st = 0; }
      bool sw = false;
      if (t + tstep < p.n_tiles) {
        const TileDesc tn = p.tiles[t + tstep];
        sw = mi_stage_geo(tn.PA, tn.PB, tn.njlog2) != g;
      }
      const bool big = 2 * PA * PB * NJ > 256;
      const uint32_t ncols = (uint32_t)(2 * PB * NJ);
      const uint32_t idesc_u = make_idesc_u8(256, ncols);
      const uint32_t idesc_s = make_idesc_s8u8(256, ncols);
      uint32_t dbase;
      if (big) {
        for (int s2 = 0; s2 < 2; s2++) {
          timed_wait<DBG>(&tempty[as], aph ^ 1, 20, w_tempty);
          if (++as == 2) { as = 0; aph ^= 1; }
        }
        dbase = tmem_base;
      } else {
        timed_wait<DBG>(&tempty[as], aph ^ 1, 21, w_tempty);
        dbase = tmem_base + as * 256;
      }
      tc_fence_after();
      {
        const uint32_t boff = (uint32_t)PA * MI_ARR_BYTES;
        const uint32_t b2off = boff + (uint32_t)(PB * NJ * 128);
        for (int kb = 0; kb < p.nkb; kb++) {
          timed_wait<DBG>(&ready[st], (phb >> st) & 1, 22, w_ready);
          tc_fence_after();
          const uint32_t lo = ((smem_u32(stage_base + st * sbytes) & 0x3FFFFu) >> 4) | (1u << 16);
          if (elect_one()) {
            const uint64_t dBa = ((uint64_t)desc_hi << 32) | (lo + (boff >> 4));
            const uint64_t dBb = ((uint64_t)desc_hi << 32) | (lo + (b2off >> 4));
            const uint32_t acc0 = kb > 0 ? 1u : 0u;
            for (int a = 0; a < PA; a++) {
              const uint64_t dx = ((uint64_t)desc_hi << 32) | (lo + (uint32_t)((a * MI_ARR_BYTES) >> 4));
              const uint32_t dHL = dbase + (uint32_t)(a * 2 * PB * NJ);
              umma_i8_pair(dHL, dx, dBa, idesc_u, acc0);
              umma_i8_pair(dHL, dx, dBb, idesc_s, 1u);
#pragma unroll
              for (int kk = 1; kk < 4; kk++) {
                umma_i8_pair(dHL, dx + 2 * kk, dBa + 2 * kk, idesc_u, 1u);
                umma_i8_pair(dHL, dx + 2 * kk, dBb + 2 * kk, idesc_s, 1u);
              }
            }
            umma_commit_pair(&empty[st]);
          }
          __syncwarp();
          phb ^= 1u << st;
          if (++st == nst) st = 0;
        }
      }
      if (elect_one()) {
        if (sw) umma_commit_pair(drained);
        if (big) {
          umma_commit_pair(&tfull[0]);
          umma_commit_pair(&tfull[1]);
        } else {
          umma_commit_pair(&tfull[as]);
        }
      }
      __syncwarp();
      if (!big) {
        if (++as == 2) { as = 0; aph ^= 1; }
      }
    }
    if (DBG && p.dbg && lane == 0) {
      p.dbg[blockIdx.x * 16 + 3] = (unsigned long long)(clock64() - t_begin);
      p.dbg[blockIdx.x * 16 + 4] = (unsigned long long)w_tempty;
      p.dbg[blockIdx.x * 16 + 5] = (unsigned long long)w_ready;
    }
    }
  } else {
    const int h = (warp - 2) * 32 + lane;
    int st = 0; uint32_t phb = 0; int geo = -1;
    long long w_full = 0, t_begin = DBG ? clock64() : 0;
    for (int t = tile0; t < p.n_tiles; t += tstep) {
      const TileDesc td = p.tiles[t];
      const int PA = td.PA, PB = td.PB, NJh = (1 << td.njlog2) >> 1;
      const int brows = PB * NJh;
      const int g = mi_stage_geo(PA, PB, td.njlog2);
      const int nst = mi_geo_stages(g);
      const uint32_t sbytes = mi_geo_bytes(g);
      if (g != geo) { geo = g; st = 0; }
      for (int kb = 0; kb < p.nkb; kb++) {
        const int cl = h & 7;
        const uint8_t* dg = p.dig + (int64_t)kb * 128 + cl * 16;
        const uint4 g0 = __ldg(reinterpret_cast<const uint4*>(dg));
        const uint4 g1 = __ldg(reinterpret_cast<const uint4*>(dg + p.kpad));
        const uint4 g2 = __ldg(reinterpret_cast<const uint4*>(dg + 2 * p.kpad));
        const uint4 g3 = __ldg(reinterpret_cast<const uint4*>(dg + 3 * p.kpad));
        timed_wait<DBG>(&full[st], (phb >> st) & 1, 40, w_full);
        const uint32_t yb = smem_u32(stage_base + st * sbytes) + (uint32_t)PA * MI_ARR_BYTES;
        const uint32_t slot = (uint32_t)brows * 128u;
        for (int r = h >> 3; r < brows; r += MI_EXP_THREADS / 8) {
          const uint32_t addr = yb + (uint32_t)r * 128u + (uint32_t)((cl ^ (r & 7)) * 16);
          const uint4 y = lds128(addr);
          sts128(addr + slot, make_uint4(y.x & g1.x, y.y & g1.y, y.z & g1.z, y.w & g1.w));
          sts128(addr + 2 * slot, make_uint4(y.x & g2.x, y.y & g2.y, y.z & g2.z, y.w & g2.w));
          sts128(addr + 3 * slot, make_uint4(y.x & g3.x, y.y & g3.y, y.z & g3.z, y.w & g3.w));
          sts128(addr, make_uint4(y.x & g0.x, y.y & g0.y, y.z & g0.z, y.w & g0.w));
        }
        fence_proxy_async_smem();
        __syncwarp();
        if (lane == 0) mbar_arrive_cluster(&ready[st], 0);
        phb ^= 1u << st;
        if (++st == nst) st = 0;
      }
    }
    if (DBG && p.dbg && h == 0) {
      p.dbg[blockIdx.x * 16 + 12] = (unsigned long long)(clock64() - t_begin);
      p.dbg[blockIdx.x * 16 + 13] = (unsigned long long)w_full;
    }
  }
  } else {
    asm volatile("setmaxnreg.inc.sync.aligned.u32 " LDW_STR(MI_REGS_EPI) ";");
    EpiCtx c;
    c.q = warp & 3;
    c.cg = (warp - MI_EPI_WARP0) >> 2;
    c.lane = lane;
    c.rank = (int)rank;
    int as = 0; uint32_t aph = 0;
    int it = 0, rit = 0;
    long long w_jfull = 0, w_tfull = 0, t_begin = DBG ? clock64() : 0;
    c.irec_saddr = smem_u32(irec);
    c.idyn_saddr = smem_u32(idyn);
    c.rempty_saddr = smem_u32(rempty);
    c.scr_saddr = smem_u32(bars + 32) + (uint32_t)(warp - MI_EPI_WARP0) * 4u;
    for (int t = tile0; t < p.n_tiles; t += tstep, it++) {
      const int jb = it & 1;
      timed_wait<DBG>(&jfull[jb], (it >> 1) & 1, 30, w_jfull);
      uint32_t hdr;
      asm volatile("ld.shared.u32 %0, [%1];" : "=r"(hdr) : "r"(smem_u32(&thdr[jb])));
      const int tPA = (int)(hdr & 0xFF), tPB = (int)((hdr >> 8) & 0xFF);
      c.tflags = hdr >> 24;
      const int NJ = 1 << ((hdr >> 16) & 0xFF);
      const bool big = 2 * tPA * tPB * NJ > 256;
      if (!(c.tflags & TILE_NULL)) { timed_wait<DBG>(rfull, (uint32_t)(rit & 1), 34, w_jfull); rit++; }
      long long c1 = DBG ? clock64() : 0;
      c.jrec_saddr = smem_u32(jrec + jb * 128);
      c.jdyn_saddr = smem_u32(jdyn + jb * 128);
      if (big) {
        uint32_t ph0 = aph;
        mbar_wait(&tfull[as], ph0, 31);
        int as1 = as ^ 1;
        uint32_t ph1 = (as == 1) ? (aph ^ 1) : aph;
        mbar_wait(&tfull[as1], ph1, 32);
        c.tmem_base = tmem_base + ((uint32_t)(c.q * 32) << 16);
      } else {
        mbar_wait(&tfull[as], aph, 33);
        c.tmem_base = tmem_base + ((uint32_t)(c.q * 32) << 16) + as * 256;
      }
      if constexpr (DBG) w_tfull += clock64() - c1;
      tc_fence_after();
      bool released = false;
      auto release_acc = [&]() {
        tc_fence_before();
        __syncwarp();
        if (big) {
          if (lane == 0) { mbar_arrive_cluster(&tempty[0], 0); mbar_arrive_cluster(&tempty[1], 0); }
          aph ^= 1;
        } else {
          if (lane == 0) mbar_arrive_cluster(&tempty[as], 0);
          if (++as == 2) { as = 0; aph ^= 1; }
        }
        released = true;
      };
      if (!(c.tflags & TILE_NULL)) {
        if (!p.qcorr) epi_dispatch<false, false>(p, tPA, tPB, c, release_acc);
        else if (p.ragged) epi_dispatch<true, true>(p, tPA, tPB, c, release_acc);
        else epi_dispatch<true, false>(p, tPA, tPB, c, release_acc);
      }
      if (!released) release_acc();
      __syncwarp();
      if (lane == 0) mbar_arrive(&jempty[jb]);
    }
    if (DBG && p.dbg && lane == 0 && (warp == MI_EPI_WARP0 || warp == MI_EPI_WARP0 + MI_EPI_WARPS - 1)) {
      int o = warp == MI_EPI_WARP0 ? 6 : 9;
      p.dbg[blockIdx.x * 16 + o] = (unsigned long long)(clock64() - t_begin);
      p.dbg[blockIdx.x * 16 + o + 1] = (unsigned long long)w_jfull;
      p.dbg[blockIdx.x * 16 + o + 2] = (unsigned long long)w_tfull;
    }
  }
  tc_fence_before();
  cluster_sync_all();
  if (warp == 2) {
    tc_fence_after();
    tmem_dealloc_pair(tmem_base, 512);
  }
}

}
```

ldweaver_b200/csrc/mi_scan.cu:

```cuda
#include <algorithm>
#include <chrono>
#include <cmath>
#include <cub/cub.cuh>
#include <vector>

#include "../../include/ldw.h"
#include "ctx.h"
#include "hdw.h"
#include "mi_aux.cuh"
#include "mi_kernel.cuh"
#include "mi_scan.h"

using namespace ldw;

namespace {

struct Group {
  int32_t slot0 = 0, nslots = 0, row0 = 0, count = 0;
};

struct DevLinks {
  DevBuf pos1, pos2, c1, c2, len, blk, mi;
  int ensure(int64_t m) {
    size_t b4 = (size_t)(m > 0 ? m : 1) * 4, b8 = (size_t)(m > 0 ? m : 1) * 8;
    LDW_TRY(pos1.ensure(b4)); LDW_TRY(pos2.ensure(b4)); LDW_TRY(c1.ensure(b4)); LDW_TRY(c2.ensure(b4));
    LDW_TRY(len.ensure(b4)); LDW_TRY(blk.ensure(b4)); LDW_TRY(mi.ensure(b8));
    return 0;
  }
};

struct BlockDev {
  DevBuf rowdyn, coldyn, colinfo, tiles, from_idx, to_idx, rfl, rtl;
  PinnedBuf stage;
  cudaEvent_t uploaded = nullptr;
  cudaEvent_t done = nullptr, done2 = nullptr;
  bool used = false, used2 = false;
};

struct BlockHost {
  std::vector<RowDyn> rowdyn;
  std::vector<ColDyn> coldyn;
  std::vector<ColInfo> colinfo;
  std::vector<TileDesc> tiles;
  std::vector<int32_t> from_idx, to_idx;
  std::vector<uint8_t> rfl, rtl;
  int32_t nf = 0, nt = 0;
  int32_t n_real_tiles = 0;
  int diag = 0, ragged = 0;
  int64_t n_pairs = 0, n_sr = 0, n_lr = 0;
};

}

struct ScanWS {
  static constexpr int RING = 4;
  BlockDev ring[RING];
  BlockHost hring[RING];
  DevBuf d_dbg;
  struct LrBuf {
    DevBuf cand, vcand, mi64, state , hist;
    cudaEvent_t scan_done = nullptr, sel_done = nullptr;
    bool used = false, chain_valid = false;
  } lr[3];
  static constexpr int NLR = 3;
  DevBuf d_state , d_sr_f32, d_dense;
  PinnedBuf h_results, h_pub;
  DevBuf d_kept_key, d_kept_gi, d_kept_gj, d_kept_mi, d_kept_count, d_sort_tmp, d_keys_sorted, d_order_in, d_order_out;
  DevLinks d_sr, d_lr;
  bool events_ready = false;
  ~ScanWS() {
    for (auto& b : ring) {
      if (b.done) cudaEventDestroy(b.done);
      if (b.done2) cudaEventDestroy(b.done2);
      if (b.uploaded) cudaEventDestroy(b.uploaded);
    }
    for (auto& l : lr) {
      if (l.scan_done) cudaEventDestroy(l.scan_done);
      if (l.sel_done) cudaEventDestroy(l.sel_done);
    }
  }
};

static void scan_ws_free(void* p) { delete static_cast<ScanWS*>(p); }

static ScanWS* get_ws(ldw_ctx* ctx) {
  if (!ctx->scan_ws) {
    ctx->scan_ws = new ScanWS();
    ctx->scan_ws_free = scan_ws_free;
  }
  return static_cast<ScanWS*>(ctx->scan_ws);
}

struct ldw_mi_plan {
  ldw_ctx* ctx = nullptr;
  int64_t n = 0, S = 0, blk = 0, Kpad = 0;
  int nranges = 0;
  std::vector<int32_t> pos, paint;
  std::vector<uint8_t> r, mask;
  std::vector<double> w;
  std::vector<Group> groups;
  std::vector<int32_t> range_slot0;
  std::vector<int32_t> slot_snp;
  int64_t nslots = 0, nrows = 0;
  double neff = 0, scale = 0;
  int32_t neffH = 0, neffL = 0;
  uint32_t sa = 0, sb = 0;
  uint32_t M = 0;
  bool pos_sorted = true;
  DevBuf d_codes, d_w, d_p64, d_rec, d_r, d_mask, d_pos, d_paint, d_ops, d_dig;
  const uint8_t* codes_dev = nullptr;
  TmapSet tm;
  std::vector<BlockResult> results;
  double t_pack_ms = 0;
};

namespace {

int build_plan(ldw_mi_plan* P, const uint8_t* codes, const uint8_t* codes_dev, const double* hdw, const int32_t* pos,
               const int32_t* paint) {
  ldw_ctx* ctx = P->ctx;
  cudaStream_t st = ctx->stream;
  const int64_t n = P->n, S = P->S, blk = P->blk;
  cudaEvent_t e0, e1;
  LDW_CUDA(cudaEventCreate(&e0));
  LDW_CUDA(cudaEventCreate(&e1));
  LDW_CUDA(cudaEventRecord(e0, st));
  const bool dbg_t = getenv("LDW_DBG_TIMING") != nullptr;
  auto bt0 = std::chrono::steady_clock::now();
  auto blap = [&](const char* what) {
    if (!dbg_t) return;
    auto t = std::chrono::steady_clock::now();
    fprintf(stderr, "ldw timing: plan %-22s %8.3f ms\n", what, std::chrono::duration<double, std::milli>(t - bt0).count());
    bt0 = t;
  };
  P->pos.assign(pos, pos + n);
  P->paint.assign(paint, paint + n);
  P->w.assign(hdw, hdw + S);
  for (int64_t i = 1; i < n; i++)
    if (pos[i] < pos[i - 1]) P->pos_sorted = false;
  double wmax = 0, neff = 0;
  for (int64_t s = 0; s < S; s++) {
    if (!(hdw[s] > 0) || !std::isfinite(hdw[s])) return set_error(LDW_ERR_ARG, "hdw[%lld] = %g is not a positive finite weight", (long long)s, hdw[s]);
    wmax = std::max(wmax, hdw[s]);
    neff += hdw[s];
  }
  P->neff = neff;
  {
    const double total = (neff + 12.5) * 268435456.0 / wmax;
    int bits = 0;
    while (std::ldexp(1.0, bits) <= total) bits++;
    int sb_ = std::max(0, bits - 32);
    if (sb_ > 14) sb_ = 14;
    P->sb = (uint32_t)sb_;
    P->sa = (uint32_t)(14 - sb_);
  }
  {
    const double unit2 = std::ldexp(1.0, (int)P->sb + 1);
    double M = std::floor(268435455.0 / wmax / unit2);
    if (M < 1) return set_error(LDW_ERR_UNSUPPORTED, "largest weight %g too large for the fixed-point count unit", wmax);
    if (M > 1073741823.0) M = 1073741823.0;
    P->M = (uint32_t)M;
    P->scale = M * unit2;
    if ((neff + 12.5) * P->scale / std::ldexp(1.0, (int)P->sb) >= 4294967295.0) {
      while (P->M > 1 && (neff + 12.5) * (P->M * unit2) / std::ldexp(1.0, (int)P->sb) >= 4294967295.0) P->M >>= 1;
      P->scale = P->M * unit2;
    }
  }
  P->Kpad = round_up(S, 128);
  std::vector<uint8_t> da(16384), db(16384);
  {
    for (int h = 0; h < 16384; h++) {
      int a = (h + 254) / 255, b = 255 * a - h;
      da[h] = (uint8_t)a;
      db[h] = (uint8_t)b;
    }
  }
  std::vector<uint8_t> dig((size_t)4 * P->Kpad, 0);
  std::vector<int32_t> wH(S), wL(S);
  int64_t sumH = 0, sumL = 0;
  std::vector<int64_t> Wq(S);
  {
    std::vector<int32_t> order(S);
    for (int64_t s = 0; s < S; s++) order[s] = (int32_t)s;
    std::stable_sort(order.begin(), order.end(), [&](int32_t a, int32_t b) { return hdw[a] < hdw[b]; });
    double carry = 0.0;
    for (int64_t k = 0; k < S; k++) {
      const int32_t s = order[k];
      const double x = hdw[s] * P->scale + carry;
      int64_t W = (int64_t)std::llround(x);
      if (W < 0) W = 0;
      if (W > 268435455) W = 268435455;
      carry = x - (double)W;
      if (carry > 1.0) carry = 1.0;
      if (carry < -1.0) carry = -1.0;
      Wq[s] = W;
    }
  }
  for (int64_t s = 0; s < S; s++) {
    int64_t W = Wq[s];
    int32_t H = (int32_t)(W >> 14), L = (int32_t)(W & 16383);
    wH[s] = H; wL[s] = L;
    sumH += H; sumL += L;
    dig[0 * P->Kpad + s] = da[H];
    dig[1 * P->Kpad + s] = da[L];
    dig[2 * P->Kpad + s] = db[H];
    dig[3 * P->Kpad + s] = db[L];
  }
  if (sumH > 0x7fffffffLL || sumL > 0x7fffffffLL) return set_error(LDW_ERR_UNSUPPORTED, "too many sequences for int32 accumulation (nseq=%lld)", (long long)S);
  P->neffH = (int32_t)sumH;
  P->neffL = (int32_t)sumL;
  blap("weights/digits");
  if (codes) {
    LDW_TRY(P->d_codes.alloc((size_t)n * S));
    P->codes_dev = static_cast<const uint8_t*>(P->d_codes.p);
  } else {
    P->codes_dev = codes_dev;
  }
  LDW_TRY(P->d_mask.alloc((size_t)n));
  LDW_TRY(P->d_r.alloc((size_t)n));
  DevBuf d_table;
  LDW_TRY(d_table.alloc((size_t)n * 5 * 4));
  if (codes) LDW_CUDA(cudaMemcpyAsync(P->d_codes.p, codes, (size_t)n * S, cudaMemcpyHostToDevice, st));
  LDW_TRY(snp_allele_stats(st, P->codes_dev, n, S, d_table.as<int32_t>(), P->d_mask.as<uint8_t>(), P->d_r.as<uint8_t>()));
  P->r.resize(n);
  P->mask.resize(n);
  LDW_CUDA(cudaMemcpyAsync(P->r.data(), P->d_r.p, (size_t)n, cudaMemcpyDeviceToHost, st));
  LDW_CUDA(cudaMemcpyAsync(P->mask.data(), P->d_mask.p, (size_t)n, cudaMemcpyDeviceToHost, st));
  LDW_CUDA(cudaStreamSynchronize(st));
  blap("upload + allele stats");
  for (int64_t i = 0; i < n; i++)
    if (P->r[i] < 2)
      return set_error(LDW_ERR_UNSUPPORTED, "SNP %lld is monomorphic (r=%d); the reference's filters never retain such sites "
                       "and this implementation does not support them", (long long)i, (int)P->r[i]);

  if (n >= (1 << 28)) return set_error(LDW_ERR_UNSUPPORTED, "nsnp >= 2^28 not supported");
  P->nranges = (int)((n + blk - 1) / blk);
  P->groups.assign((size_t)P->nranges * 4, Group());
  P->range_slot0.assign(P->nranges + 1, 0);
  int64_t slot = 0, row = 0;
  std::vector<int32_t> snp_slot(n);
  for (int b = 0; b < P->nranges; b++) {
    P->range_slot0[b] = (int32_t)slot;
    int64_t lo = (int64_t)b * blk, hi = std::min<int64_t>(n, lo + blk);
    for (int pc = 1; pc <= 4; pc++) {
      Group& G = P->groups[(size_t)b * 4 + pc - 1];
      G.slot0 = (int32_t)slot;
      G.row0 = (int32_t)row;
      int cnt = 0;
      for (int64_t i = lo; i < hi; i++)
        if (P->r[i] - 1 == pc) snp_slot[i] = (int32_t)(slot + cnt++);
      G.count = cnt;
      G.nslots = (int32_t)round_up(cnt, 128);
      slot += G.nslots;
      row += (int64_t)G.nslots * pc;
      if (slot > 0x3fffffff || row > 0x3fffffff) return set_error(LDW_ERR_UNSUPPORTED, "problem too large for 32-bit slot indices");
    }
  }
  P->range_slot0[P->nranges] = (int32_t)slot;
  P->nslots = slot;
  P->nrows = row;
  P->slot_snp.assign(slot, -1);
  for (int64_t i = 0; i < n; i++) P->slot_snp[snp_slot[i]] = (int32_t)i;
  std::vector<uint32_t> row_info((size_t)std::max<int64_t>(row, 1), 0xFFFFFFFFu);
  for (int b = 0; b < P->nranges; b++)
    for (int pc = 1; pc <= 4; pc++) {
      const Group& G = P->groups[(size_t)b * 4 + pc - 1];
      for (int k = 0; k < G.count; k++) {
        int32_t snp = P->slot_snp[G.slot0 + k];
        int m = P->mask[snp], q = 0;
        for (int a = 0; a < 5 && q < pc; a++)
          if (m & (1 << a)) {
            row_info[(size_t)G.row0 + (size_t)q * G.nslots + k] = (uint32_t)snp | ((uint32_t)a << 28);
            q++;
          }
      }
    }
  blap("slots + row_info (host)");
  DevBuf d_slot_snp, d_wH, d_wL, d_row_info;
  LDW_TRY(P->d_w.alloc((size_t)S * 8));
  LDW_TRY(d_wH.alloc((size_t)S * 4));
  LDW_TRY(d_wL.alloc((size_t)S * 4));
  LDW_TRY(d_slot_snp.alloc((size_t)std::max<int64_t>(slot, 1) * 4));
  LDW_TRY(d_row_info.alloc(row_info.size() * 4));
  LDW_TRY(P->d_p64.alloc((size_t)n * 5 * 8));
  LDW_TRY(P->d_rec.alloc((size_t)std::max<int64_t>(slot, 1) * 4 * sizeof(Rec)));
  LDW_TRY(P->d_pos.alloc((size_t)n * 4));
  LDW_TRY(P->d_paint.alloc((size_t)n * 4));
  LDW_CUDA(cudaMemcpyAsync(P->d_w.p, hdw, (size_t)S * 8, cudaMemcpyHostToDevice, st));
  LDW_CUDA(cudaMemcpyAsync(d_wH.p, wH.data(), (size_t)S * 4, cudaMemcpyHostToDevice, st));
  LDW_CUDA(cudaMemcpyAsync(d_wL.p, wL.data(), (size_t)S * 4, cudaMemcpyHostToDevice, st));
  LDW_CUDA(cudaMemcpyAsync(d_slot_snp.p, P->slot_snp.data(), (size_t)slot * 4, cudaMemcpyHostToDevice, st));
  LDW_CUDA(cudaMemcpyAsync(d_row_info.p, row_info.data(), row_info.size() * 4, cudaMemcpyHostToDevice, st));
  LDW_CUDA(cudaMemcpyAsync(P->d_pos.p, pos, (size_t)n * 4, cudaMemcpyHostToDevice, st));
  LDW_CUDA(cudaMemcpyAsync(P->d_paint.p, paint, (size_t)n * 4, cudaMemcpyHostToDevice, st));
  {
    int wpb = 8;
    mi_build_rec_kernel<<<(unsigned)((slot + wpb - 1) / wpb), wpb * 32, 0, st>>>(
        P->codes_dev, S, d_slot_snp.as<int32_t>(), slot, P->d_mask.as<uint8_t>(), P->d_w.as<double>(),
        d_wH.as<int32_t>(), d_wL.as<int32_t>(), P->d_rec.as<Rec>(), slot, P->d_p64.as<double>(), P->sa, P->sb, P->M);
    LDW_CUDA(cudaGetLastError());
  }
  size_t op_bytes = (size_t)std::max<int64_t>(row, 128) * P->Kpad;
  LDW_TRY(P->d_ops.alloc(op_bytes));
  LDW_TRY(P->d_dig.alloc(dig.size()));
  LDW_CUDA(cudaMemcpyAsync(P->d_dig.p, dig.data(), dig.size(), cudaMemcpyHostToDevice, st));
  {
    int64_t total = row * (P->Kpad / 16);
    if (total > 0) {
      mi_pack_operands_kernel<<<(unsigned)((total + 255) / 256), 256, 0, st>>>(P->codes_dev, S, P->Kpad,
                                                                               d_row_info.as<uint32_t>(), row,
                                                                               P->d_ops.as<uint8_t>());
      LDW_CUDA(cudaGetLastError());
    }
  }
  uint64_t trows = (uint64_t)std::max<int64_t>(row, 128);
  LDW_TRY(make_tmap_u8_sw128(&P->tm.a, P->d_ops.p, trows, (uint64_t)P->Kpad, 128));
  for (int j = 0; j < 4; j++) LDW_TRY(make_tmap_u8_sw128(&P->tm.b[j], P->d_ops.p, trows, (uint64_t)P->Kpad, 64u >> j));
  {
    ScanWS* W = get_ws(ctx);
    if (!W->events_ready) {
      for (auto& b : W->ring) {
        LDW_CUDA(cudaEventCreateWithFlags(&b.done, cudaEventDisableTiming));
        LDW_CUDA(cudaEventCreateWithFlags(&b.done2, cudaEventDisableTiming));
        LDW_CUDA(cudaEventCreateWithFlags(&b.uploaded, cudaEventDisableTiming));
      }
      for (auto& l : W->lr) {
        LDW_CUDA(cudaEventCreateWithFlags(&l.scan_done, cudaEventDisableTiming));
        LDW_CUDA(cudaEventCreateWithFlags(&l.sel_done, cudaEventDisableTiming));
      }
      W->events_ready = true;
    }
  }
  LDW_CUDA(cudaEventRecord(e1, st));
  LDW_CUDA(cudaStreamSynchronize(st));
  blap("records + pack + tmaps");
  float ms = 0;
  cudaEventElapsedTime(&ms, e0, e1);
  P->t_pack_ms = ms;
  cudaEventDestroy(e0);
  cudaEventDestroy(e1);
  LDW_CUDA(cudaFuncSetAttribute(mi_scan_kernel<false>, cudaFuncAttributeMaxDynamicSharedMemorySize, MI_SMEM_BYTES));
  LDW_CUDA(cudaFuncSetAttribute(mi_scan_kernel<true>, cudaFuncAttributeMaxDynamicSharedMemorySize, MI_SMEM_BYTES));
  return 0;
}

struct ScanCfg {
  double g, sr_dist, lr_retain, lr_approx;
  int flags;
  int dense = 0;
};

inline double circ_len_d(double p1, double p2, double g) {
  double m = std::fmod(p1 - p2, g);
  if (m < 0) m += g;
  return 0.5 * g - std::fabs(m - 0.5 * g);
}

int prepare_block(const ldw_mi_plan* P, int bf, int bt, const ScanCfg& cfg, BlockHost& H, bool sizes_only = false) {
  const int64_t n = P->n, blk = P->blk;
  const bool sr_only = (cfg.flags & LDW_SCAN_SR_ONLY) != 0;
  const double g = cfg.g, sr = cfg.sr_dist;
  int64_t flo = (int64_t)bf * blk, fhi = std::min<int64_t>(n, flo + blk);
  int64_t tlo = (int64_t)bt * blk, thi = std::min<int64_t>(n, tlo + blk);
  H.from_idx.clear();
  H.to_idx.clear();
  if (!sr_only) {
    for (int64_t i = flo; i < fhi; i++) H.from_idx.push_back((int32_t)i);
    for (int64_t i = tlo; i < thi; i++) H.to_idx.push_back((int32_t)i);
  } else {
    auto keep = [&](int64_t lo, int64_t hi, int64_t olo, int64_t ohi, std::vector<int32_t>& out) {
      for (int64_t i = lo; i < hi; i++) {
        double x = P->pos[i];
        bool k = false;
        auto it = std::lower_bound(P->pos.begin() + olo, P->pos.begin() + ohi, (int32_t)x);
        int64_t c = it - P->pos.begin();
        for (int64_t j : {c - 1, c, olo, ohi - 1})
          if (j >= olo && j < ohi && std::fabs(circ_len_d(P->pos[j], x, g)) < sr) k = true;
        if (k) out.push_back((int32_t)i);
      }
    };
    keep(flo, fhi, tlo, thi, H.from_idx);
    keep(tlo, thi, flo, fhi, H.to_idx);
  }
  const int32_t nf = (int32_t)H.from_idx.size(), nt = (int32_t)H.to_idx.size();
  H.nf = nf; H.nt = nt;
  H.diag = (nf == nt) && std::equal(H.from_idx.begin(), H.from_idx.end(), H.to_idx.begin());
  H.ragged = (nf != nt);
  H.n_pairs = H.n_sr = H.n_lr = 0;
  if (nf == 0 || nt == 0) return 1;
  H.n_pairs = H.diag ? (int64_t)nf * (nf - 1) / 2 : (int64_t)nf * nt - std::min(nf, nt);

  const int32_t fs0 = P->range_slot0[bf], fs1 = P->range_slot0[bf + 1];
  const int32_t ts0 = P->range_slot0[bt], ts1 = P->range_slot0[bt + 1];
  H.colinfo.assign(nt, ColInfo{0, 0, 0, 0, 0, 0});
  const bool all_sr = !(sr < 0.5 * g);
  {
    int64_t a0 = 0, a1 = 0, w1 = 0, w0 = 0;
    uint64_t accU = 0, accL = 0;
    std::vector<uint32_t> cu(nt), cl(nt);
    for (int j = 0; j < nt; j++) {
      const double pj = P->pos[H.to_idx[j]];
      int32_t ia0, ia1, ib0, ib1;
      if (all_sr) {
        ia0 = 0; ia1 = nf; ib0 = ib1 = 0;
      } else {
        while (a0 < nf && (double)P->pos[H.from_idx[a0]] < pj - sr) a0++;
        while (a1 < nf && (double)P->pos[H.from_idx[a1]] <= pj + sr) a1++;
        while (w1 < nf && (double)P->pos[H.from_idx[w1]] <= pj - (g - sr)) w1++;
        while (w0 < nf && (double)P->pos[H.from_idx[w0]] < pj + (g - sr)) w0++;
        int32_t x0 = (int32_t)a0, x1 = (int32_t)std::max(a0, a1);
        if (w1 > 0) {
          if ((int32_t)w1 >= x0) { ia0 = 0; ia1 = std::max<int32_t>((int32_t)w1, x1); ib0 = ib1 = 0; }
          else { ia0 = 0; ia1 = (int32_t)w1; ib0 = x0; ib1 = x1; }
        } else if (w0 < nf) {
          if ((int32_t)w0 <= x1) { ia0 = x0; ia1 = nf; if ((int32_t)w0 < x0) ia0 = (int32_t)w0; ib0 = ib1 = 0; }
          else { ia0 = x0; ia1 = x1; ib0 = (int32_t)w0; ib1 = nf; }
        } else {
          ia0 = x0; ia1 = x1; ib0 = ib1 = 0;
        }
      }
      ColInfo& c = H.colinfo[j];
      c.a0 = ia0; c.a1 = ia1; c.b0 = ib0; c.b1 = ib1;
      auto below = [&](int x) {
        return std::min(std::max(x - ia0, 0), ia1 - ia0) + std::min(std::max(x - ib0, 0), ib1 - ib0);
      };
      int tot = (ia1 - ia0) + (ib1 - ib0);
      cu[j] = H.diag ? 0u : (uint32_t)below(std::min(j, nf));
      cl[j] = (uint32_t)(tot - below(std::min(j + 1, nf)));
      accU += cu[j];
      accL += cl[j];
    }
    if (accU + accL > 0xFFFFFFF0ull) return set_error(LDW_ERR_UNSUPPORTED, "more than 2^32 short-range links in one block");
    uint32_t ru = 0, rl = (uint32_t)accU;
    for (int j = 0; j < nt; j++) {
      H.colinfo[j].baseU = ru;
      H.colinfo[j].baseL = rl;
      ru += cu[j];
      rl += cl[j];
    }
    H.n_sr = (int64_t)(accU + accL);
    H.n_lr = H.n_pairs - H.n_sr;
  }
  if (sizes_only) return 0;
  H.rfl.resize(nf);
  H.rtl.resize(nt);
  for (int k = 0; k < nf; k++) H.rfl[k] = P->r[H.from_idx[k]];
  for (int k = 0; k < nt; k++) H.rtl[k] = P->r[H.to_idx[k]];
  std::vector<int32_t> il_of(fhi - flo, -1), jl_of(thi - tlo, -1);
  for (int k = 0; k < nf; k++) il_of[H.from_idx[k] - flo] = k;
  for (int k = 0; k < nt; k++) jl_of[H.to_idx[k] - tlo] = k;
  H.rowdyn.assign(fs1 - fs0, RowDyn{-1, 0.f});
  for (int32_t s = fs0; s < fs1; s++) {
    int32_t snp = P->slot_snp[s];
    if (snp < 0) continue;
    int32_t il = il_of[snp - flo];
    RowDyn rd;
    rd.il = il;
    rd.rtl = (il >= 0 && il < nt) ? (float)H.rtl[il] : 0.f;
    H.rowdyn[s - fs0] = rd;
  }
  H.coldyn.assign(ts1 - ts0, ColDyn{-1, 0.f, 0, 0, 0, 0, 0, 0});
  for (int32_t s = ts0; s < ts1; s++) {
    int32_t snp = P->slot_snp[s];
    if (snp < 0) continue;
    int32_t jl = jl_of[snp - tlo];
    ColDyn cd{-1, 0.f, 0, 0, 0, 0, 0, 0};
    cd.jl = jl;
    if (jl >= 0) {
      cd.rfl = jl < nf ? (float)H.rfl[jl] : 0.f;
      const ColInfo& c = H.colinfo[jl];
      cd.a0 = c.a0; cd.a1 = c.a1; cd.b0 = c.b0; cd.b1 = c.b1; cd.baseU = c.baseU; cd.baseL = c.baseL;
    }
    H.coldyn[s - ts0] = cd;
  }

  const int nfc = (fs1 - fs0) / 16, ntc = (ts1 - ts0) / 16;
  std::vector<int32_t> f_first(nfc, -1), f_last(nfc, -1), t_first(ntc, -1), t_last(ntc, -1);
  for (int c = 0; c < nfc; c++)
    for (int k = 0; k < 16; k++)
      if (H.rowdyn[c * 16 + k].il >= 0) { if (f_first[c] < 0) f_first[c] = c * 16 + k; f_last[c] = c * 16 + k; }
  for (int c = 0; c < ntc; c++)
    for (int k = 0; k < 16; k++)
      if (H.coldyn[c * 16 + k].jl >= 0) { if (t_first[c] < 0) t_first[c] = c * 16 + k; t_last[c] = c * 16 + k; }
  auto extent = [](const std::vector<int32_t>& first, const std::vector<int32_t>& last, int off0, int nsl, int& lo, int& hi) {
    lo = hi = -1;
    for (int c = off0 / 16; c < (off0 + nsl) / 16; c++)
      if (first[c] >= 0) { if (lo < 0) lo = first[c]; hi = last[c]; }
  };
  H.tiles.clear();
  for (int pa = 1; pa <= 4; pa++) {
    const Group& Gi = P->groups[(size_t)bf * 4 + pa - 1];
    if (Gi.count == 0) continue;
    for (int pb = 1; pb <= 4; pb++) {
      const Group& Gj = P->groups[(size_t)bt * 4 + pb - 1];
      if (Gj.count == 0) continue;
      const int njl = mi_njlog2(pa, pb), NJ = 1 << njl;
      const int n_ti = (Gi.count + 127) / 128, n_tj = (Gj.count + NJ - 1) / NJ;
      struct Ext { int lo, hi, lmin, lmax; double p0, p1; };
      std::vector<Ext> ei(n_ti), ej(n_tj);
      for (int ti = 0; ti < n_ti; ti++) {
        Ext& e = ei[ti];
        extent(f_first, f_last, Gi.slot0 - fs0 + ti * 128, 128, e.lo, e.hi);
        if (e.lo >= 0) {
          e.lmin = H.rowdyn[e.lo].il; e.lmax = H.rowdyn[e.hi].il;
          e.p0 = P->pos[P->slot_snp[fs0 + e.lo]]; e.p1 = P->pos[P->slot_snp[fs0 + e.hi]];
        }
      }
      for (int tj = 0; tj < n_tj; tj++) {
        Ext& e = ej[tj];
        extent(t_first, t_last, Gj.slot0 - ts0 + tj * NJ, NJ, e.lo, e.hi);
        if (e.lo >= 0) {
          e.lmin = H.coldyn[e.lo].jl; e.lmax = H.coldyn[e.hi].jl;
          e.p0 = P->pos[P->slot_snp[ts0 + e.lo]]; e.p1 = P->pos[P->slot_snp[ts0 + e.hi]];
        }
      }
      auto make_tile = [&](int ti, int tj, uint32_t flags) {
        TileDesc td;
        memset(&td, 0, sizeof(td));
        td.a_row0 = Gi.row0 + ti * 128;
        td.a_pstride = Gi.nslots;
        td.b_row0 = Gj.row0 + tj * NJ;
        td.b_pstride = Gj.nslots;
        td.i_slot0 = Gi.slot0 + ti * 128;
        td.j_slot0 = Gj.slot0 + tj * NJ;
        td.i_dyn0 = td.i_slot0 - fs0;
        td.j_dyn0 = td.j_slot0 - ts0;
        td.PA = (uint8_t)pa; td.PB = (uint8_t)pb; td.njlog2 = (uint8_t)njl;
        td.flags = (uint8_t)flags;
        return td;
      };
      auto wanted = [&](int ti, int tj, uint32_t& flags) -> bool {
        if (ti >= n_ti || tj >= n_tj) return false;
        const Ext &a = ei[ti], &b = ej[tj];
        if (a.lo < 0 || b.lo < 0) return false;
        if (H.diag && !cfg.dense && a.lmax <= b.lmin) return false;
        const double gap = std::max(0.0, std::max(a.p0, b.p0) - std::min(a.p1, b.p1));
        const double span = std::max(a.p1, b.p1) - std::min(a.p0, b.p0);
        const bool has_sr = all_sr || gap <= sr || (g - span) <= sr;
        if (sr_only && !has_sr) return false;
        flags = has_sr ? TILE_HAS_SR : 0;
        return true;
      };
      for (int ti = 0; ti < n_ti; ti += 2)
        for (int tj = 0; tj < n_tj; tj++) {
          uint32_t fl0 = 0, fl1 = 0;
          const bool w0 = wanted(ti, tj, fl0), w1 = wanted(ti + 1, tj, fl1);
          if (!w0 && !w1) continue;
          TileDesc td = make_tile(ti, tj, w0 ? fl0 : (uint32_t)TILE_NULL);
          td.flags1 = (uint8_t)(w1 ? fl1 : (uint32_t)TILE_NULL);
          H.tiles.push_back(td);
        }
    }
  }
  {
    size_t cnt[16] = {0}, beg[16];
    for (const TileDesc& t : H.tiles) cnt[(t.PA - 1) * 4 + (t.PB - 1)]++;
    int ord[16];
    for (int k = 0; k < 16; k++) ord[k] = k;
    auto geo = [](int k) { return mi_stage_geo(k / 4 + 1, k % 4 + 1, mi_njlog2(k / 4 + 1, k % 4 + 1)); };
    std::stable_sort(ord, ord + 16, [&](int a, int b) { return geo(a) != geo(b) ? geo(a) > geo(b) : cnt[a] < cnt[b]; });
    size_t off = 0;
    for (int k = 0; k < 16; k++) { beg[ord[k]] = off; off += cnt[ord[k]]; }
    std::vector<TileDesc> sorted(H.tiles.size());
    for (const TileDesc& t : H.tiles) sorted[beg[(t.PA - 1) * 4 + (t.PB - 1)]++] = t;
    H.tiles.swap(sorted);
  }
  H.n_real_tiles = (int32_t)H.tiles.size();
  if (!cfg.dense && H.n_real_tiles >= 1024) {
    const int np = 64;
    for (int k = 0; k < np; k++) H.tiles.push_back(H.tiles[(size_t)((2 * k + 1) * (int64_t)H.n_real_tiles / (2 * np))]);
  }
  return 0;
}

int upload_block(cudaStream_t st, BlockDev& D, const BlockHost& H) {
  struct Part { DevBuf* d; const void* src; size_t bytes; };
  Part parts[8] = {{&D.rowdyn, H.rowdyn.data(), H.rowdyn.size() * sizeof(RowDyn)},
                   {&D.coldyn, H.coldyn.data(), H.coldyn.size() * sizeof(ColDyn)},
                   {&D.colinfo, H.colinfo.data(), H.colinfo.size() * sizeof(ColInfo)},
                   {&D.tiles, H.tiles.data(), H.tiles.size() * sizeof(TileDesc)},
                   {&D.from_idx, H.from_idx.data(), H.from_idx.size() * 4},
                   {&D.to_idx, H.to_idx.data(), H.to_idx.size() * 4},
                   {&D.rfl, H.rfl.data(), H.rfl.size()},
                   {&D.rtl, H.rtl.data(), H.rtl.size()}};
  size_t total = 0;
  for (auto& p : parts) total += (p.bytes + 255) & ~(size_t)255;
  LDW_TRY(D.stage.ensure(total + 256));
  size_t off = 0;
  for (auto& p : parts) {
    LDW_TRY(p.d->ensure(std::max<size_t>(p.bytes, 16)));
    if (p.bytes) {
      memcpy(D.stage.as<uint8_t>() + off, p.src, p.bytes);
      LDW_CUDA(cudaMemcpyAsync(p.d->p, D.stage.as<uint8_t>() + off, p.bytes, cudaMemcpyHostToDevice, st));
    }
    off += (p.bytes + 255) & ~(size_t)255;
  }
  return 0;
}

void fill_scan_params(const ldw_mi_plan* P, const BlockDev& D, const BlockHost& H, const ScanCfg& cfg, ScanParams& sp) {
  memset(&sp, 0, sizeof(sp));
  sp.tiles = D.tiles.as<TileDesc>();
  sp.n_tiles = H.n_real_tiles;
  sp.rec = P->d_rec.as<Rec>();
  sp.rec_vstride = P->nslots;
  sp.rowdyn = D.rowdyn.as<RowDyn>();
  sp.coldyn = D.coldyn.as<ColDyn>();
  sp.nkb = (int32_t)(P->Kpad / 128);
  sp.nf = H.nf; sp.nt = H.nt;
  sp.diag = H.diag; sp.ragged = H.ragged;
  sp.qcorr = (!H.diag && !(cfg.flags & LDW_SCAN_IDEAL_Q)) ? 1 : 0;
  sp.sr_only = (cfg.flags & LDW_SCAN_SR_ONLY) ? 1 : 0;
  sp.dig = P->d_dig.as<uint8_t>();
  sp.kpad = P->Kpad;
  sp.rfl_arr = D.rfl.as<uint8_t>();
  sp.rtl_arr = D.rtl.as<uint8_t>();
  sp.sa = P->sa;
  sp.sb = P->sb;
  sp.kT = (float)(std::ldexp(1.0, (int)P->sb) / P->scale);
  sp.M = P->M;
  for (int a = 0; a < 4; a++)
    for (int b = 0; b < 4; b++) {
      double ri = a + 2, rj = b + 2;
      double den = P->neff + 0.5 * ri * rj;
      const float den_f = (float)den, rkT = 1.0f / sp.kT, rden = 1.0f / den_f;
      sp.scale[a][b] = (float)(M_LN2 / den) * sp.kT;
      sp.q0s[a][b] = (float)(0.25 * ri * rj / den) * rkT;
      sp.qod[a][b] = (float)(0.25 / den) * rkT;
      sp.rp_qc[a][b] = rden * rkT;
      sp.rp_plain[a][b] = den_f * sp.kT;
    }
}

int launch_scan(const ldw_mi_plan* P, const ScanParams& sp, cudaStream_t st, int reserve = 0) {
  if (sp.n_tiles <= 0) return 0;
  int grid = 2 * std::min<int>(sp.n_tiles, std::max(1, (P->ctx->num_sms - reserve) / 2));
  if (sp.dbg) mi_scan_kernel<true><<<grid, MI_THREADS, MI_SMEM_BYTES, st>>>(P->tm, sp);
  else mi_scan_kernel<false><<<grid, MI_THREADS, MI_SMEM_BYTES, st>>>(P->tm, sp);
  LDW_CUDA(cudaGetLastError());
  return 0;
}

RefineParams make_refine_params(const ldw_mi_plan* P, const BlockDev& D, const BlockHost& H, const ScanCfg& cfg) {
  RefineParams R;
  R.codes = P->codes_dev;
  R.S = P->S;
  R.w = P->d_w.as<double>();
  R.p64 = P->d_p64.as<double>();
  R.r = P->d_r.as<uint8_t>();
  R.mask = P->d_mask.as<uint8_t>();
  R.from_idx = D.from_idx.as<int32_t>();
  R.to_idx = D.to_idx.as<int32_t>();
  R.rfl_arr = D.rfl.as<uint8_t>();
  R.rtl_arr = D.rtl.as<uint8_t>();
  R.nf = H.nf; R.nt = H.nt;
  R.ideal_q = (cfg.flags & LDW_SCAN_IDEAL_Q) ? 1 : 0;
  R.neff = P->neff;
  return R;
}

int validate_scan(const ldw_mi_plan* P, const ScanCfg& cfg) {
  if (!(cfg.g > 0) || cfg.g != std::floor(cfg.g) || cfg.g > 9.0e15) return set_error(LDW_ERR_ARG, "genome length g=%g must be a positive integer", cfg.g);
  if (!(cfg.sr_dist >= 0)) return set_error(LDW_ERR_ARG, "sr_dist must be >= 0");
  if (!P->pos_sorted) return set_error(LDW_ERR_UNSUPPORTED, "POS must be non-decreasing (the short-range slot layout relies on it)");
  if (P->n > 0 && ((double)P->pos.back() - (double)P->pos.front()) >= cfg.g) return set_error(LDW_ERR_UNSUPPORTED, "POS span must be smaller than the genome length g");
  return 0;
}

}

extern "C" {

int ldw_mi_plan_create(ldw_ctx* ctx, const uint8_t* codes, int64_t n_snp, int64_t nseq, const double* hdw,
                       const int32_t* pos, const int32_t* paint, int64_t blk, ldw_mi_plan** out) {
  if (!codes) return set_error(LDW_ERR_ARG, "ldw_mi_plan_create: null argument");
  return ldw::mi_plan_create_impl(ctx, codes, nullptr, n_snp, nseq, hdw, pos, paint, blk, out);
}

}

int ldw::mi_plan_create_impl(ldw_ctx* ctx, const uint8_t* codes, const uint8_t* codes_dev, int64_t n_snp, int64_t nseq,
                             const double* hdw, const int32_t* pos, const int32_t* paint, int64_t blk, ldw_mi_plan** out) {
  LDW_TRY(ctx_bind(ctx));
  if (!out) return set_error(LDW_ERR_ARG, "ldw_mi_plan_create: null out");
  *out = nullptr;
  if ((!codes && !codes_dev) || !hdw || !pos || !paint) return set_error(LDW_ERR_ARG, "ldw_mi_plan_create: null argument");
  if (n_snp < 2 || nseq < 1) return set_error(LDW_ERR_ARG, "ldw_mi_plan_create: need at least 2 SNPs and 1 sequence");
  if (nseq > 65535) return set_error(LDW_ERR_UNSUPPORTED, "ldw_mi_plan_create: nseq > 65535 not supported by the 15-bit digit accumulation");
  if (blk < 128 || blk > 65535) return set_error(LDW_ERR_UNSUPPORTED, "ldw_mi_plan_create: block size %lld outside [128, 65535]", (long long)blk);
  if (codes) {
    const int64_t total = n_snp * nseq;
    const int64_t chunk = (int64_t)1 << 22;
    const int64_t nchunks = (total + chunk - 1) / chunk;
    std::vector<int64_t> bad_at(nchunks, -1);
    parallel_for(nchunks, 8, [&](int64_t c) {
      int64_t i = c * chunk;
      const int64_t end = std::min<int64_t>(total, i + chunk);
      for (; i + 8 <= end; i += 8) {
        uint64_t x;
        memcpy(&x, codes + i, 8);
        if ((((x & 0x7F7F7F7F7F7F7F7Full) + 0x7B7B7B7B7B7B7B7Bull) | x) & 0x8080808080808080ull) break;
      }
      for (; i < end; i++)
        if (codes[i] > 4) { bad_at[c] = i; break; }
    });
    for (int64_t c = 0; c < nchunks; c++)
      if (bad_at[c] >= 0)
        return set_error(LDW_ERR_ARG, "ldw_mi_plan_create: codes[%lld] = %d outside 0..4", (long long)bad_at[c], (int)codes[bad_at[c]]);
  }
  ldw_mi_plan* P = new ldw_mi_plan();
  P->ctx = ctx;
  P->n = n_snp; P->S = nseq; P->blk = blk;
  int rc = build_plan(P, codes, codes_dev, hdw, pos, paint);
  if (rc != 0) { delete P; return rc; }
  *out = P;
  return 0;
}

extern "C" {

void ldw_mi_plan_destroy(ldw_mi_plan* plan) {
  if (!plan) return;
  cudaSetDevice(plan->ctx->device);
  delete plan;
}

int ldw_mi_block_dense(ldw_mi_plan* P, int64_t block_index, double* mi_out, int64_t* nf_out, int64_t* nt_out) {
  if (!P) return set_error(LDW_ERR_ARG, "null plan");
  LDW_TRY(ctx_bind(P->ctx));
  cudaStream_t st = P->ctx->stream;
  ScanWS* W = get_ws(P->ctx);
  int bf = 0, bt = 0;
  {
    int64_t k = block_index;
    bool found = false;
    for (int i = 0; i < P->nranges && !found; i++)
      for (int j = i; j < P->nranges; j++) {
        if (k == 0) { bf = i; bt = j; found = true; break; }
        k--;
      }
    if (!found) return set_error(LDW_ERR_ARG, "block index out of range");
  }
  ScanCfg cfg{1e15, 0.0, 0, 0, 0};
  cfg.dense = 1;
  BlockHost& H = W->hring[0];
  BlockDev& D = W->ring[0];
  int e = prepare_block(P, bf, bt, cfg, H);
  if (e > 1) return e;
  if (nf_out) *nf_out = H.nf;
  if (nt_out) *nt_out = H.nt;
  if (!mi_out) return 0;
  LDW_TRY(upload_block(st, D, H));
  size_t cells = (size_t)H.nf * H.nt;
  LDW_TRY(W->d_dense.ensure(cells * 4));
  LDW_CUDA(cudaMemsetAsync(W->d_dense.p, 0, cells * 4, st));
  ScanParams sp;
  fill_scan_params(P, D, H, cfg, sp);
  sp.dense = 1;
  sp.dense_out = W->d_dense.as<float>();
  LDW_TRY(launch_scan(P, sp, st));
  DevBuf d64;
  LDW_TRY(d64.alloc(cells * 8));
  f32_to_f64_kernel<<<(unsigned)((cells + 255) / 256), 256, 0, st>>>(W->d_dense.as<float>(), (int64_t)cells, d64.as<double>());
  LDW_CUDA(cudaMemcpyAsync(mi_out, d64.p, cells * 8, cudaMemcpyDeviceToHost, st));
  LDW_CUDA(cudaStreamSynchronize(st));
  return 0;
}

int ldw_mi_pairs_exact(ldw_mi_plan* P, int64_t block_index, const int32_t* from_local, const int32_t* to_local,
                       int64_t n_pairs, double* mi_out) {
  if (!P) return set_error(LDW_ERR_ARG, "null plan");
  LDW_TRY(ctx_bind(P->ctx));
  cudaStream_t st = P->ctx->stream;
  ScanWS* W = get_ws(P->ctx);
  int bf = 0, bt = 0;
  {
    int64_t k = block_index;
    bool found = false;
    for (int i = 0; i < P->nranges && !found; i++)
      for (int j = i; j < P->nranges; j++) {
        if (k == 0) { bf = i; bt = j; found = true; break; }
        k--;
      }
    if (!found) return set_error(LDW_ERR_ARG, "block index out of range");
  }
  if (n_pairs <= 0) return 0;
  ScanCfg cfg{1e15, 0.0, 0, 0, 0};
  BlockHost& H = W->hring[0];
  BlockDev& D = W->ring[0];
  int e = prepare_block(P, bf, bt, cfg, H);
  if (e != 0) return e == 1 ? set_error(LDW_ERR_ARG, "empty block") : e;
  for (int64_t k = 0; k < n_pairs; k++)
    if (from_local[k] < 0 || from_local[k] >= H.nf || to_local[k] < 0 || to_local[k] >= H.nt)
      return set_error(LDW_ERR_ARG, "pair %lld outside the block", (long long)k);
  LDW_TRY(upload_block(st, D, H));
  DevBuf di, dj, dout;
  LDW_TRY(di.alloc((size_t)n_pairs * 4));
  LDW_TRY(dj.alloc((size_t)n_pairs * 4));
  LDW_TRY(dout.alloc((size_t)n_pairs * 8));
  LDW_CUDA(cudaMemcpyAsync(di.p, from_local, (size_t)n_pairs * 4, cudaMemcpyHostToDevice, st));
  LDW_CUDA(cudaMemcpyAsync(dj.p, to_local, (size_t)n_pairs * 4, cudaMemcpyHostToDevice, st));
  RefineParams R = make_refine_params(P, D, H, cfg);
  int grid = (int)std::min<int64_t>((n_pairs + REFINE_WARPS - 1) / REFINE_WARPS, 148 * 8);
  mi_refine_pairs_kernel<<<grid, 32 * REFINE_WARPS, 0, st>>>(R, di.as<int32_t>(), dj.as<int32_t>(), n_pairs, dout.as<double>());
  LDW_CUDA(cudaGetLastError());
  LDW_CUDA(cudaMemcpyAsync(mi_out, dout.p, (size_t)n_pairs * 8, cudaMemcpyDeviceToHost, st));
  LDW_CUDA(cudaStreamSynchronize(st));
  return 0;
}

int ldw_mi_scan(ldw_mi_plan* P, double g, double sr_dist, double lr_retain_links, double lr_links_approx, int flags,
                int n_parts, int part, ldw_links* sr_out, ldw_links* lr_out, ldw_links* borderline_out, double* thr_out,
                double* prob_out, ldw_scan_stats* stats_out) {
  return ldw::mi_scan_impl(P, g, sr_dist, lr_retain_links, lr_links_approx, flags, n_parts, part, nullptr, sr_out, lr_out,
                           borderline_out, thr_out, prob_out, stats_out);
}

}

int ldw::mi_block_sizes(const ldw_mi_plan* P, double g, double sr_dist, int flags, std::vector<BlockSizes>& out) {
  if (!P) return set_error(LDW_ERR_ARG, "null plan");
  ScanCfg cfg{g, sr_dist, 0, 0, flags};
  LDW_TRY(validate_scan(P, cfg));
  std::vector<std::pair<int, int>> bl;
  for (int i = 0; i < P->nranges; i++)
    for (int j = i; j < P->nranges; j++) bl.push_back({i, j});
  out.assign(bl.size(), BlockSizes{0, 0, 0, 0});
  parallel_for((int64_t)bl.size(), 16, [&](int64_t b) {
    BlockHost tmp;
    int e = prepare_block(P, bl[b].first, bl[b].second, cfg, tmp, true);
    out[b] = BlockSizes{tmp.n_pairs, tmp.n_sr, tmp.n_lr, e};
  });
  for (size_t b = 0; b < bl.size(); b++)
    if (out[b].err > 1) {
      BlockHost t2;
      return prepare_block(P, bl[b].first, bl[b].second, cfg, t2, true);
    }
  return 0;
}

void ldw::mi_block_owners(const ldw_mi_plan* P, int n_parts, std::vector<int>& owner) {
  struct Item { int64_t cost, idx; };
  std::vector<Item> items;
  int64_t idx = 0;
  for (int i = 0; i < P->nranges; i++)
    for (int j = i; j < P->nranges; j++, idx++) {
      const int64_t ni = std::min<int64_t>(P->n, (int64_t)(i + 1) * P->blk) - (int64_t)i * P->blk;
      const int64_t nj = std::min<int64_t>(P->n, (int64_t)(j + 1) * P->blk) - (int64_t)j * P->blk;
      items.push_back({i == j ? ni * (ni - 1) / 2 : ni * nj, idx});
    }
  std::vector<Item> order = items;
  std::stable_sort(order.begin(), order.end(), [](const Item& a, const Item& b) { return a.cost > b.cost; });
  std::vector<int64_t> load(n_parts, 0);
  owner.assign(items.size(), 0);
  for (const Item& it : order) {
    int best = 0;
    for (int p = 1; p < n_parts; p++)
      if (load[p] < load[best]) best = p;
    owner[it.idx] = best;
    load[best] += it.cost;
  }
}

int64_t ldw::mi_plan_nblocks(const ldw_mi_plan* P) { return (int64_t)P->nranges * (P->nranges + 1) / 2; }

int ldw::mi_scan_impl(ldw_mi_plan* P, double g, double sr_dist, double lr_retain_links, double lr_links_approx, int flags,
                      int n_parts, int part, const ScanShared* shared, ldw_links* sr_out, ldw_links* lr_out,
                      ldw_links* borderline_out, double* thr_out, double* prob_out, ldw_scan_stats* stats_out) {
  if (!P) return set_error(LDW_ERR_ARG, "null plan");
  const auto t_entry = std::chrono::steady_clock::now();
  LDW_TRY(ctx_bind(P->ctx));
  cudaStream_t st = P->ctx->stream;
  ScanWS* W = get_ws(P->ctx);
  ScanCfg cfg{g, sr_dist, lr_retain_links, lr_links_approx, flags};
  LDW_TRY(validate_scan(P, cfg));
  const bool sr_only = (flags & LDW_SCAN_SR_ONLY) != 0;
  if (!sr_only && !(lr_links_approx > 0)) return set_error(LDW_ERR_ARG, "lr_links_approx must be > 0");
  if (n_parts < 1 || part < 0 || part >= n_parts) return set_error(LDW_ERR_ARG, "bad partition %d of %d", part, n_parts);

  struct Blk { int bf, bt; int64_t index; };
  std::vector<Blk> blocks;
  {
    std::vector<int> owner;
    mi_block_owners(P, n_parts, owner);
    int64_t idx = 0;
    for (int i = 0; i < P->nranges; i++)
      for (int j = i; j < P->nranges; j++, idx++)
        if (owner[idx] == part) blocks.push_back({i, j, idx});
  }
  const int64_t nblk_total = (int64_t)P->nranges * (P->nranges + 1) / 2;
  if (thr_out) for (int64_t b = 0; b < nblk_total; b++) thr_out[b] = NAN;
  if (prob_out) for (int64_t b = 0; b < nblk_total; b++) prob_out[b] = NAN;

  cudaEvent_t ev0, ev1, ev2, ev3;
  LDW_CUDA(cudaEventCreate(&ev0)); LDW_CUDA(cudaEventCreate(&ev1)); LDW_CUDA(cudaEventCreate(&ev2)); LDW_CUDA(cudaEventCreate(&ev3));

  struct Sel { int64_t n_lr = 0, n_sr = 0, n_pairs = 0; double prob = NAN; uint64_t k_lo = 0, k_hi = 0; double h = 0; int interp = 0;
               int emit_all = 0; uint32_t kprime = 0, delta = 1, cap = 0; int64_t sr_base = 0, sr_hbase = 0; int skip = 0; };
  std::vector<Sel> sel(blocks.size());
  int64_t total_sr = 0, total_pairs = 0, total_lr = 0;
  uint64_t max_cap = 1, sum_keep = 0;
  int64_t first_guess = -1;
  int first_rc = -1;
  {
    std::vector<int> perr(blocks.size(), 0);
    for (size_t b = 0; b < blocks.size() && first_guess < 0; b++)
      if (blocks[b].bt - blocks[b].bf <= 1) first_guess = (int64_t)b;
    if (first_guess < 0 && !blocks.empty()) first_guess = 0;
    parallel_for((int64_t)blocks.size() + 1, 8, [&](int64_t b) {
      if (b == (int64_t)blocks.size()) {
        if (first_guess >= 0) first_rc = prepare_block(P, blocks[first_guess].bf, blocks[first_guess].bt, cfg, W->hring[0]);
        return;
      }
      Sel& s = sel[b];
      if (shared) {
        const BlockSizes& z = shared->sizes[blocks[b].index];
        perr[b] = z.err;
        s.n_lr = z.n_lr; s.n_sr = z.n_sr; s.n_pairs = z.n_pairs;
        return;
      }
      BlockHost tmp;
      int e = prepare_block(P, blocks[b].bf, blocks[b].bt, cfg, tmp, true);
      perr[b] = e;
      s.n_lr = tmp.n_lr; s.n_sr = tmp.n_sr; s.n_pairs = tmp.n_pairs;
    });
    for (size_t b = 0; b < blocks.size(); b++) {
      const int e = perr[b];
      if (e > 1) {
        BlockHost t2;
        return prepare_block(P, blocks[b].bf, blocks[b].bt, cfg, t2, true);
      }
      Sel& s = sel[b];
      s.skip = (e == 1);
      struct { int64_t n_lr, n_sr, n_pairs; } tmp{s.n_lr, s.n_sr, s.n_pairs};
      s.sr_base = total_sr;
      s.sr_hbase = shared ? shared->sr_hbase[blocks[b].index] : total_sr;
      total_sr += tmp.n_sr; total_pairs += tmp.n_pairs; total_lr += tmp.n_lr;
      if (!sr_only && tmp.n_lr > 0) {
        const double m = (double)tmp.n_lr;
        double prob = 1 - ((lr_retain_links * (m / lr_links_approx)) / m);
        if (prob < 0) prob = 0;
        s.prob = prob;
        double index = 1 + (m - 1 > 0 ? m - 1 : 0) * prob;
        double lo = std::floor(index), hi = std::ceil(index);
        s.k_lo = (uint64_t)(tmp.n_lr - (int64_t)lo + 1);
        s.k_hi = (uint64_t)(tmp.n_lr - (int64_t)hi + 1);
        s.h = index - lo;
        s.interp = index > lo;
        uint64_t K = s.k_lo;
        if (2 * K + 65536 >= (uint64_t)tmp.n_lr) {
          s.emit_all = 1;
          if ((uint64_t)tmp.n_lr > 0xFFFFFFF0ull) return set_error(LDW_ERR_UNSUPPORTED, "block keeps more than 2^32 long-range links");
          s.cap = (uint32_t)tmp.n_lr;
          s.kprime = (uint32_t)std::min<uint64_t>(K, 0xFFFFFFFFull);
        } else {
          uint64_t kp = K + std::max<uint64_t>(1024, K / 8);
          uint64_t delta = std::max<uint64_t>(2 * kp, 32768);
          uint64_t cap = std::min<uint64_t>((uint64_t)tmp.n_lr, 16 * kp + (4u << 20));
          if (cap > 0xFFFFFFF0ull) return set_error(LDW_ERR_UNSUPPORTED, "long-range candidate buffer exceeds 2^32 entries");
          s.kprime = (uint32_t)kp; s.delta = (uint32_t)delta; s.cap = (uint32_t)cap;
        }
        max_cap = std::max<uint64_t>(max_cap, s.cap);
        sum_keep += K;
      }
    }
  }
  const uint64_t kept_cap = 2 * sum_keep + (1u << 20);

  for (auto& l : W->lr) {
    LDW_TRY(l.cand.ensure(max_cap * sizeof(Cand)));
    LDW_TRY(l.mi64.ensure(max_cap * 8));
    LDW_TRY(l.vcand.ensure(max_cap * sizeof(Cand)));
    LDW_TRY(l.state.ensure(64));
    LDW_TRY(l.hist.ensure(MI_HIST_BINS * 4));
    l.used = false; l.chain_valid = false;
  }
  LDW_TRY(W->d_state.ensure(64));
  LDW_TRY(W->h_results.ensure(std::max<size_t>(blocks.size(), 1) * sizeof(BlockResult)));
  LDW_TRY(W->h_pub.ensure(64));
  memset(W->h_results.p, 0, std::max<size_t>(blocks.size(), 1) * sizeof(BlockResult));
  LDW_TRY(W->d_sr_f32.ensure((size_t)std::max<int64_t>(total_sr, 1) * 4));
  LDW_TRY(W->d_kept_key.ensure(kept_cap * 8));
  LDW_TRY(W->d_kept_gi.ensure(kept_cap * 4));
  LDW_TRY(W->d_kept_gj.ensure(kept_cap * 4));
  LDW_TRY(W->d_kept_mi.ensure(kept_cap * 8));
  LDW_TRY(W->d_kept_count.ensure(16));
  const bool sr_rows = !(flags & (LDW_SCAN_NO_LINKS | LDW_SCAN_LR_ONLY));
  if (sr_rows) LDW_TRY(W->d_sr.ensure(total_sr));
  LDW_CUDA(cudaMemsetAsync(W->d_kept_count.p, 0, 16, st));
  uint32_t* d_kept_overflow = W->d_state.as<uint32_t>() + 3;
  uint32_t* d_chain2 = W->d_state.as<uint32_t>() + 8;
  LDW_CUDA(cudaMemsetAsync(W->d_state.p, 0, 64, st));
  cudaStream_t sst = P->ctx->select_stream;

  const bool want_host = !(flags & (LDW_SCAN_NO_LINKS | LDW_SCAN_NO_D2H));
  const bool sr_to_host = want_host && !(flags & LDW_SCAN_SR_ON_DEVICE);
  P->ctx->dev_sr.n = -1;
  cudaStream_t cst = P->ctx->copy_stream;
  cudaEvent_t ev_blk = nullptr;
  HostLinks& hsr = shared ? *shared->h_sr : P->ctx->h_sr;
  if (sr_to_host) {
    if (!shared && sr_rows) LDW_TRY(hsr.ensure(total_sr));
    LDW_CUDA(cudaEventCreateWithFlags(&ev_blk, cudaEventDisableTiming));
  }
  auto tpre = std::chrono::steady_clock::now();
  LDW_CUDA(cudaEventRecord(ev0, st));
  int64_t n_reruns = 0, n_launches = 0, n_scan_launches = 0, n_tiles = 0;
  double exec_ops = 0, exec_mufu = 0;
  std::vector<cudaEvent_t> kev;
  auto kev_cleanup = [&]() { for (auto e : kev) cudaEventDestroy(e); kev.clear(); };
  int64_t dbg_block = -1;
  {
    const char* e = getenv("LDW_DBG_BLOCK");
    if (e) dbg_block = atoll(e);
  }
  double host_prep_ms = 0;
  int scan_reserve = 2;
  if (const char* e = getenv("LDW_SCAN_RESERVE")) scan_reserve = atoi(e);
  float force_seed = -1.f;
  if (const char* e = getenv("LDW_DBG_FORCE_SEED")) force_seed = (float)atof(e);
  double sel_margin0 = 4e-6;
  if (const char* e = getenv("LDW_DBG_SEL_MARGIN")) sel_margin0 = atof(e);
  auto run_block = [&](size_t b, size_t seq, int force_emit_all, uint32_t cap_override, bool use_chain, double sel_margin) -> int {
    Sel& s = sel[b];
    if (s.skip) return 0;
    int slot = (int)(seq % ScanWS::RING);
    BlockDev& D = W->ring[slot];
    BlockHost& H = W->hring[slot];
    if (D.used) LDW_CUDA(cudaEventSynchronize(D.done));
    if (D.used2) { LDW_CUDA(cudaEventSynchronize(D.done2)); D.used2 = false; }
    ScanWS::LrBuf& L = W->lr[seq % ScanWS::NLR];
    uint32_t* d_count = L.state.as<uint32_t>();
    uint32_t* d_tcand = d_count + 1;
    uint32_t* d_overflow = d_count + 2;
    uint32_t* d_chain = d_chain2;
    auto hp0 = std::chrono::steady_clock::now();
    int e;
    if (seq == 0 && first_guess == (int64_t)b && first_rc >= 0 && first_rc <= 1 && !force_emit_all && !cap_override) {
      e = first_rc;
      first_rc = -1;
    } else {
      e = prepare_block(P, blocks[b].bf, blocks[b].bt, cfg, H);
    }
    if (e > 1) return e;
    LDW_TRY(upload_block(P->ctx->upload_stream, D, H));
    LDW_CUDA(cudaEventRecord(D.uploaded, P->ctx->upload_stream));
    LDW_CUDA(cudaStreamWaitEvent(st, D.uploaded, 0));
    host_prep_ms += std::chrono::duration<double, std::milli>(std::chrono::steady_clock::now() - hp0).count();
    D.used = true;
    ScanParams sp;
    fill_scan_params(P, D, H, cfg, sp);
    sp.sr_out = W->d_sr_f32.as<float>() + s.sr_base;
    if (dbg_block >= 0 && (int64_t)b == dbg_block) {
      LDW_TRY(W->d_dbg.ensure(4096 * 16 * 8));
      LDW_CUDA(cudaMemsetAsync(W->d_dbg.p, 0, 4096 * 16 * 8, st));
      sp.dbg = W->d_dbg.as<unsigned long long>();
    }
    const bool lr = !sr_only && s.n_lr > 0;
    const int emit_all = force_emit_all || s.emit_all;
    uint32_t cap = cap_override ? cap_override : s.cap;
    if (lr) {
      if (L.used) LDW_CUDA(cudaStreamWaitEvent(st, L.sel_done, 0));
      const int n_pilot = (int)H.tiles.size() - H.n_real_tiles;
      if (seq == 0 && use_chain && !emit_all && n_pilot > 0) {
        mi_block_begin_kernel<<<1, 256, 0, st>>>(d_count, L.hist.as<uint32_t>(), d_chain, 0);
        ScanParams pp = sp;
        pp.tiles = D.tiles.as<TileDesc>() + H.n_real_tiles;
        pp.n_tiles = n_pilot;
        pp.cand = L.cand.as<Cand>(); pp.cand_cap = cap; pp.cand_count = d_count; pp.tcand_bits = d_tcand;
        pp.hist = L.hist.as<uint32_t>(); pp.kprime = s.kprime; pp.delta = s.delta ? s.delta : 1; pp.overflow = d_overflow;
        pp.emit_all = 1;
        pp.dbg = nullptr;
        LDW_TRY(launch_scan(P, pp, st, 0));
        mi_pilot_seed_kernel<<<1, 1024, 0, st>>>(L.cand.as<Cand>(), d_count, cap, (unsigned long long)s.k_lo, (double)s.n_lr, d_chain);
        LDW_CUDA(cudaGetLastError());
        n_launches += 3;
      }
      if (force_seed >= 0.f && use_chain && !emit_all) {
        static_assert(sizeof(float) == 4, "float bits");
        LDW_CUDA(cudaMemcpyAsync(d_chain, &force_seed, 4, cudaMemcpyHostToDevice, st));
        LDW_CUDA(cudaStreamSynchronize(st));
      }
      mi_block_begin_kernel<<<1, 256, 0, st>>>(d_count, L.hist.as<uint32_t>(), d_chain, (use_chain && !emit_all) ? 1 : 0);
      LDW_CUDA(cudaGetLastError());
      n_launches++;
      sp.cand = L.cand.as<Cand>();
      sp.cand_cap = cap;
      sp.cand_count = d_count;
      sp.tcand_bits = d_tcand;
      sp.hist = L.hist.as<uint32_t>();
      sp.kprime = s.kprime;
      sp.delta = s.delta ? s.delta : 1;
      sp.overflow = d_overflow;
      sp.emit_all = emit_all;
    } else {
      sp.sr_only = 1;
    }
    if (sp.n_tiles > 0) {
      cudaEvent_t k0, k1;
      LDW_CUDA(cudaEventCreate(&k0));
      LDW_CUDA(cudaEventCreate(&k1));
      kev.push_back(k0);
      kev.push_back(k1);
      LDW_CUDA(cudaEventRecord(k0, st));
      LDW_TRY(launch_scan(P, sp, st, lr ? scan_reserve : 0));
      LDW_CUDA(cudaEventRecord(k1, st));
      n_launches++; n_scan_launches++;
      n_tiles += sp.n_tiles;
      for (int32_t ti = 0; ti < H.n_real_tiles; ti++) {
        const TileDesc& td = H.tiles[ti];
        exec_ops += 8.0 * 256.0 * (double)(td.PA * td.PB * (1 << td.njlog2)) * (double)P->Kpad;
        const int RA = td.PA + 1, RB = td.PB + 1;
        const int halves = ((td.flags & TILE_NULL) ? 0 : 1) + ((td.flags1 & TILE_NULL) ? 0 : 1);
        exec_mufu += halves * 128.0 * (double)(1 << td.njlog2) * (double)(RA * (RB + (sp.qcorr ? (RB + 1) / 2 : 0)));
      }
    }
    if (lr) {
      n_launches += 2;
      LDW_CUDA(cudaEventRecord(L.scan_done, st));
      LDW_CUDA(cudaStreamWaitEvent(sst, L.scan_done, 0));
      RefineParams R = make_refine_params(P, D, H, cfg);
      n_launches++;
      mi_presel_kernel<<<1, 1024, 0, sst>>>(L.cand.as<Cand>(), d_count, cap, d_tcand, emit_all, (unsigned long long)s.k_lo, (float)sel_margin,
                                           L.vcand.as<Cand>(), d_count + 5);
      LDW_CUDA(cudaGetLastError());
      mi_refine_list_kernel<<<P->ctx->num_sms * 4, 32 * REFINE_WARPS, 0, sst>>>(R, L.vcand.as<Cand>(), d_count + 5, L.mi64.as<double>());
      LDW_CUDA(cudaGetLastError());
      SelectParams q;
      memset(&q, 0, sizeof(q));
      q.cand = L.vcand.as<Cand>(); q.mi64 = L.mi64.as<double>(); q.vcount = d_count + 5; q.count = d_count; q.cap = cap;
      q.overflow = d_overflow; q.tcand_bits = d_tcand; q.emit_all = emit_all;
      q.k_lo = s.k_lo; q.k_hi = s.k_hi; q.h = s.h; q.interpolate = s.interp;
      q.tol_safe = sel_margin; q.tol_border = 1e-9;
      q.from_idx = D.from_idx.as<int32_t>(); q.to_idx = D.to_idx.as<int32_t>();
      q.nf = H.nf; q.nt = H.nt; q.diag = H.diag; q.block = (int32_t)blocks[b].index;
      q.kept_key = W->d_kept_key.as<uint64_t>(); q.kept_gi = W->d_kept_gi.as<int32_t>(); q.kept_gj = W->d_kept_gj.as<int32_t>();
      q.kept_mi = W->d_kept_mi.as<double>(); q.kept_count = W->d_kept_count.as<unsigned long long>(); q.kept_cap = kept_cap;
      q.kept_overflow = d_kept_overflow;
      q.chain_bits = d_chain;
      q.result = W->h_results.as<BlockResult>() + b;
      mi_select_kernel<<<1, 1024, 0, sst>>>(q);
      LDW_CUDA(cudaGetLastError());
      LDW_CUDA(cudaEventRecord(L.sel_done, sst));
      LDW_CUDA(cudaEventRecord(D.done2, sst));
      L.used = true;
      D.used2 = true;
    }
    if (s.n_sr > 0 && sr_rows) {
      n_launches++;
      SrMatParams m;
      m.col = D.colinfo.as<ColInfo>(); m.from_idx = D.from_idx.as<int32_t>(); m.to_idx = D.to_idx.as<int32_t>();
      m.pos = P->d_pos.as<int32_t>(); m.paint = P->d_paint.as<int32_t>();
      m.sr_mi = W->d_sr_f32.as<float>() + s.sr_base;
      m.nf = H.nf; m.nt = H.nt; m.diag = H.diag; m.block = (int32_t)blocks[b].index; m.g = (int64_t)g;
      m.o_pos1 = W->d_sr.pos1.as<int32_t>() + s.sr_base; m.o_pos2 = W->d_sr.pos2.as<int32_t>() + s.sr_base;
      m.o_c1 = W->d_sr.c1.as<int32_t>() + s.sr_base; m.o_c2 = W->d_sr.c2.as<int32_t>() + s.sr_base;
      m.o_len = W->d_sr.len.as<int32_t>() + s.sr_base; m.o_blk = W->d_sr.blk.as<int32_t>() + s.sr_base;
      m.o_mi = W->d_sr.mi.as<double>() + s.sr_base;
      mi_sr_materialize_kernel<<<H.nt, 128, 0, st>>>(m);
      LDW_CUDA(cudaGetLastError());
      if (flags & LDW_SCAN_SR_EXACT) {
        n_launches++;
        mi_sr_exact_kernel<<<H.nt, 32 * REFINE_WARPS, 0, st>>>(m, make_refine_params(P, D, H, cfg));
        LDW_CUDA(cudaGetLastError());
      }
      if (sr_to_host) {
        LDW_CUDA(cudaEventRecord(ev_blk, st));
        LDW_CUDA(cudaStreamWaitEvent(cst, ev_blk, 0));
        HostLinks& h = hsr;
        const size_t o = (size_t)s.sr_hbase, nb4 = (size_t)s.n_sr * 4, nb8 = (size_t)s.n_sr * 8;
        LDW_CUDA(cudaMemcpyAsync(h.pos1.as<int32_t>() + o, m.o_pos1, nb4, cudaMemcpyDeviceToHost, cst));
        LDW_CUDA(cudaMemcpyAsync(h.pos2.as<int32_t>() + o, m.o_pos2, nb4, cudaMemcpyDeviceToHost, cst));
        LDW_CUDA(cudaMemcpyAsync(h.c1.as<int32_t>() + o, m.o_c1, nb4, cudaMemcpyDeviceToHost, cst));
        LDW_CUDA(cudaMemcpyAsync(h.c2.as<int32_t>() + o, m.o_c2, nb4, cudaMemcpyDeviceToHost, cst));
        LDW_CUDA(cudaMemcpyAsync(h.len.as<int32_t>() + o, m.o_len, nb4, cudaMemcpyDeviceToHost, cst));
        LDW_CUDA(cudaMemcpyAsync(h.blk.as<int32_t>() + o, m.o_blk, nb4, cudaMemcpyDeviceToHost, cst));
        LDW_CUDA(cudaMemcpyAsync(h.mi.as<double>() + o, m.o_mi, nb8, cudaMemcpyDeviceToHost, cst));
      }
    }
    LDW_CUDA(cudaEventRecord(D.done, st));
    return 0;
  };
  std::vector<size_t> order;
  for (size_t b = 0; b < blocks.size(); b++) if (sel[b].n_sr > 0) order.push_back(b);
  for (size_t b = 0; b < blocks.size(); b++) if (!(sel[b].n_sr > 0)) order.push_back(b);
  for (size_t k = 0; k < order.size(); k++) LDW_TRY(run_block(order[k], k, 0, 0, true, sel_margin0));
  for (auto& l : W->lr)
    if (l.used) LDW_CUDA(cudaStreamWaitEvent(st, l.sel_done, 0));
  LDW_CUDA(cudaEventRecord(ev1, st));
  const bool dbg_timing = getenv("LDW_DBG_TIMING") != nullptr;
  auto tp0 = std::chrono::steady_clock::now();
  auto lap = [&](const char* what) {
    if (!dbg_timing) return;
    cudaStreamSynchronize(st);
    auto t = std::chrono::steady_clock::now();
    fprintf(stderr, "ldw timing: %-28s %8.3f ms\n", what, std::chrono::duration<double, std::milli>(t - tp0).count());
    tp0 = t;
  };
  if (dbg_timing) fprintf(stderr, "ldw timing: %-28s %8.3f ms\n", "sizes + workspace (host)", std::chrono::duration<double, std::milli>(tpre - t_entry).count());
  if (dbg_timing) fprintf(stderr, "ldw timing: %-28s %8.3f ms\n", "submit blocks (host)", std::chrono::duration<double, std::milli>(tp0 - tpre).count());
  lap("drain blocks");

  LDW_CUDA(cudaStreamSynchronize(st));
  P->results.assign(W->h_results.as<BlockResult>(), W->h_results.as<BlockResult>() + blocks.size());
  if (!sr_only) {
    for (size_t b = 0; b < blocks.size(); b++) {
      if (sel[b].skip || sel[b].n_lr == 0) continue;
      if (P->results[b].bad) {
        double margin = sel_margin0;
        for (int attempt = 0; attempt < 2 && P->results[b].bad; attempt++) {
          n_reruns++;
          if (P->results[b].bad & 8) margin = std::max(std::max(margin, 4e-6), 8.0 * (double)P->results[b].eps_obs);
          uint32_t cap = 0;
          if (attempt == 1) {
            if ((uint64_t)sel[b].n_lr > 0xFFFFFFF0ull) return set_error(LDW_ERR_UNSUPPORTED, "block %lld needs an exhaustive long-range pass over more than 2^32 links", (long long)blocks[b].index);
            cap = (uint32_t)sel[b].n_lr;
            ScanWS::LrBuf& L = W->lr[0];
            LDW_TRY(L.cand.ensure((size_t)cap * sizeof(Cand)));
            LDW_TRY(L.mi64.ensure((size_t)cap * 8));
            LDW_TRY(L.vcand.ensure((size_t)cap * sizeof(Cand)));
          }
          LDW_TRY(run_block(b, 0, attempt == 1, cap, false, margin));
          LDW_CUDA(cudaStreamWaitEvent(st, W->lr[0].sel_done, 0));
          LDW_CUDA(cudaStreamSynchronize(st));
          P->results[b] = W->h_results.as<BlockResult>()[b];
        }
        if (P->results[b].bad) return set_error(LDW_ERR_INTERNAL, "long-range selection failed for block %lld (flags %u)", (long long)blocks[b].index, P->results[b].bad);
      }
    }
  }
  lap("results + reruns");
  unsigned long long n_kept = 0;
  uint32_t state[4] = {0, 0, 0, 0};
  publish_kernel<<<1, 1, 0, st>>>(W->d_kept_count.as<unsigned long long>(), W->d_state.as<uint32_t>(), W->h_pub.as<unsigned long long>());
  LDW_CUDA(cudaGetLastError());
  LDW_CUDA(cudaStreamSynchronize(st));
  n_kept = W->h_pub.as<unsigned long long>()[0];
  state[3] = (uint32_t)W->h_pub.as<unsigned long long>()[1];
  if (state[3] || n_kept > kept_cap) return set_error(LDW_ERR_UNSUPPORTED, "more long-range links pass their block thresholds (%llu) than the output buffer holds (%llu): massive ties at the threshold", n_kept, (unsigned long long)kept_cap);

  int64_t n_border = 0;
  for (auto& r : P->results) n_border += r.n_border;
  if (n_kept > 0 && !(flags & LDW_SCAN_NO_LINKS)) {
    n_launches += 2 + 4;
    LDW_TRY(W->d_keys_sorted.ensure(n_kept * 8));
    LDW_TRY(W->d_order_in.ensure(n_kept * 4));
    LDW_TRY(W->d_order_out.ensure(n_kept * 4));
    iota_u32_kernel<<<(unsigned)((n_kept + 255) / 256), 256, 0, st>>>(W->d_order_in.as<uint32_t>(), (int64_t)n_kept);
    size_t tmp_bytes = 0;
    cub::DeviceRadixSort::SortPairs(nullptr, tmp_bytes, W->d_kept_key.as<uint64_t>(), W->d_keys_sorted.as<uint64_t>(),
                                    W->d_order_in.as<uint32_t>(), W->d_order_out.as<uint32_t>(), (int)n_kept, 0, 64, st);
    LDW_TRY(W->d_sort_tmp.ensure(tmp_bytes));
    LDW_CUDA(cub::DeviceRadixSort::SortPairs(W->d_sort_tmp.p, tmp_bytes, W->d_kept_key.as<uint64_t>(), W->d_keys_sorted.as<uint64_t>(),
                                             W->d_order_in.as<uint32_t>(), W->d_order_out.as<uint32_t>(), (int)n_kept, 0, 64, st));
    LDW_TRY(W->d_lr.ensure((int64_t)n_kept));
    mi_lr_materialize_kernel<<<(unsigned)((n_kept + 255) / 256), 256, 0, st>>>(
        W->d_order_out.as<uint32_t>(), W->d_keys_sorted.as<uint64_t>(), W->d_kept_gi.as<int32_t>(), W->d_kept_gj.as<int32_t>(),
        W->d_kept_mi.as<double>(), P->d_pos.as<int32_t>(), P->d_paint.as<int32_t>(), (int64_t)n_kept, (int64_t)g,
        W->d_lr.pos1.as<int32_t>(), W->d_lr.pos2.as<int32_t>(), W->d_lr.c1.as<int32_t>(), W->d_lr.c2.as<int32_t>(),
        W->d_lr.len.as<int32_t>(), W->d_lr.mi.as<double>(), W->d_lr.blk.as<int32_t>());
    LDW_CUDA(cudaGetLastError());
  }
  LDW_CUDA(cudaEventRecord(ev2, st));
  lap("lr sort + materialise");

  P->ctx->h_sr.n = 0; P->ctx->h_lr.n = 0; P->ctx->h_border.n = 0;
  if (!(flags & (LDW_SCAN_NO_LINKS | LDW_SCAN_NO_D2H))) {
    auto d2h = [&](HostLinks& h, DevLinks& d, int64_t m) -> int {
      LDW_TRY(h.ensure(m));
      h.n = m;
      if (m == 0) return 0;
      LDW_CUDA(cudaMemcpyAsync(h.pos1.p, d.pos1.p, (size_t)m * 4, cudaMemcpyDeviceToHost, st));
      LDW_CUDA(cudaMemcpyAsync(h.pos2.p, d.pos2.p, (size_t)m * 4, cudaMemcpyDeviceToHost, st));
      LDW_CUDA(cudaMemcpyAsync(h.c1.p, d.c1.p, (size_t)m * 4, cudaMemcpyDeviceToHost, st));
      LDW_CUDA(cudaMemcpyAsync(h.c2.p, d.c2.p, (size_t)m * 4, cudaMemcpyDeviceToHost, st));
      LDW_CUDA(cudaMemcpyAsync(h.len.p, d.len.p, (size_t)m * 4, cudaMemcpyDeviceToHost, st));
      LDW_CUDA(cudaMemcpyAsync(h.blk.p, d.blk.p, (size_t)m * 4, cudaMemcpyDeviceToHost, st));
      LDW_CUDA(cudaMemcpyAsync(h.mi.p, d.mi.p, (size_t)m * 8, cudaMemcpyDeviceToHost, st));
      return 0;
    };
    if (!shared) P->ctx->h_sr.n = (sr_rows && sr_to_host) ? total_sr : 0;
    LDW_TRY(d2h(P->ctx->h_lr, W->d_lr, (int64_t)n_kept));
  }
  LDW_CUDA(cudaEventRecord(ev3, st));
  LDW_CUDA(cudaStreamSynchronize(st));
  lap("lr d2h");
  if (sr_to_host) LDW_CUDA(cudaStreamSynchronize(cst));
  lap("copy stream drain");
  if (ev_blk) cudaEventDestroy(ev_blk);

  if (borderline_out) {
    std::vector<int64_t> idx;
    const int32_t* blkcol = P->ctx->h_lr.blk.as<int32_t>();
    const double* micol = P->ctx->h_lr.mi.as<double>();
    std::vector<double> thr_by_index(nblk_total, NAN);
    for (size_t b = 0; b < blocks.size(); b++)
      if (!sel[b].skip && sel[b].n_lr > 0 && !sr_only) thr_by_index[blocks[b].index] = P->results[b].thr;
    for (int64_t i = 0; i < P->ctx->h_lr.n; i++)
      if (std::fabs(micol[i] - thr_by_index[blkcol[i]]) <= 1e-9) idx.push_back(i);
    LDW_TRY(P->ctx->h_border.ensure((int64_t)idx.size()));
    P->ctx->h_border.n = (int64_t)idx.size();
    for (size_t k = 0; k < idx.size(); k++) {
      int64_t i = idx[k];
      P->ctx->h_border.pos1.as<int32_t>()[k] = P->ctx->h_lr.pos1.as<int32_t>()[i];
      P->ctx->h_border.pos2.as<int32_t>()[k] = P->ctx->h_lr.pos2.as<int32_t>()[i];
      P->ctx->h_border.c1.as<int32_t>()[k] = P->ctx->h_lr.c1.as<int32_t>()[i];
      P->ctx->h_border.c2.as<int32_t>()[k] = P->ctx->h_lr.c2.as<int32_t>()[i];
      P->ctx->h_border.len.as<int32_t>()[k] = P->ctx->h_lr.len.as<int32_t>()[i];
      P->ctx->h_border.blk.as<int32_t>()[k] = blkcol[i];
      P->ctx->h_border.mi.as<double>()[k] = micol[i];
    }
    P->ctx->h_border.fill(borderline_out);
  }
  if (flags & (LDW_SCAN_NO_LINKS | LDW_SCAN_NO_D2H)) {
    if (sr_out) { memset(sr_out, 0, sizeof(*sr_out)); sr_out->n = total_sr; }
    if (lr_out) { memset(lr_out, 0, sizeof(*lr_out)); lr_out->n = (int64_t)n_kept; }
  } else {
    if (shared || !sr_to_host) { if (sr_out) { memset(sr_out, 0, sizeof(*sr_out)); sr_out->n = sr_rows ? total_sr : 0; } }
    else P->ctx->h_sr.fill(sr_out);

    P->ctx->h_lr.fill(lr_out);
  }
  if (sr_rows && n_parts == 1) {
    ldw_ctx::DevSr& d = P->ctx->dev_sr;
    d.pos1 = W->d_sr.pos1.as<int32_t>(); d.pos2 = W->d_sr.pos2.as<int32_t>(); d.c1 = W->d_sr.c1.as<int32_t>();
    d.c2 = W->d_sr.c2.as<int32_t>(); d.len = W->d_sr.len.as<int32_t>(); d.blk = W->d_sr.blk.as<int32_t>();
    d.mi = W->d_sr.mi.as<double>();
    d.n = total_sr;
  }
  for (size_t b = 0; b < blocks.size(); b++) {
    if (sel[b].skip || sel[b].n_lr == 0 || sr_only) continue;
    if (thr_out) thr_out[blocks[b].index] = P->results[b].thr;
    if (prob_out) prob_out[blocks[b].index] = sel[b].prob;
  }
  if (stats_out) {
    memset(stats_out, 0, sizeof(*stats_out));
    stats_out->n_blocks = (int64_t)blocks.size();
    stats_out->n_pairs = total_pairs;
    stats_out->n_sr = total_sr;
    stats_out->n_lr_total = sr_only ? 0 : total_lr;
    stats_out->n_lr_kept = (int64_t)n_kept;
    stats_out->n_borderline = n_border;
    {
      int64_t nc = 0;
      for (auto& r : P->results) nc += r.n_cand;
      stats_out->n_candidates = nc;
    }
    stats_out->n_reruns = n_reruns;
    float a = 0, b = 0, c = 0;
    cudaEventElapsedTime(&a, ev0, ev1);
    cudaEventElapsedTime(&b, ev1, ev2);
    cudaEventElapsedTime(&c, ev2, ev3);
    stats_out->t_pack_ms = P->t_pack_ms;
    stats_out->t_scan_ms = a;
    stats_out->t_select_ms = b;
    stats_out->t_d2h_ms = c;
    double tk = 0;
    for (size_t k = 0; k + 1 < kev.size(); k += 2) {
      float ms = 0;
      cudaEventElapsedTime(&ms, kev[k], kev[k + 1]);
      tk += ms;
    }
    stats_out->t_kernel_ms = tk;
    if (dbg_timing && kev.size() >= 4) {
      double gaps = 0, gmax = 0;
      std::string detail;
      for (size_t k = 1; k + 1 < kev.size(); k += 2) {
        float ms = 0;
        cudaEventElapsedTime(&ms, kev[k], kev[k + 1]);
        gaps += ms;
        gmax = std::max<double>(gmax, ms);
        char b[32];
        snprintf(b, sizeof(b), " %.0f", 1e3 * ms);
        detail += b;
      }
      float first = 0, last = 0;
      cudaEventElapsedTime(&first, ev0, kev[0]);
      cudaEventElapsedTime(&last, kev[kev.size() - 1], ev1);
      fprintf(stderr, "ldw timing: gaps between scan kernels: sum %.3f ms, max %.3f ms; before first %.3f ms, after last %.3f ms; us:%s\n",
              gaps, gmax, first, last, detail.c_str());
    }
    stats_out->n_scan_launches = n_scan_launches;
    stats_out->n_launches = n_launches;
    stats_out->n_tiles = n_tiles;
    stats_out->exec_int8_ops = exec_ops;
    stats_out->t_host_prep_ms = host_prep_ms;
    stats_out->exec_mufu_ops = exec_mufu;
    {
      double em = 0;
      for (size_t b = 0; b < blocks.size(); b++)
        if (!sel[b].skip && sel[b].n_lr > 0 && !sr_only) em = std::max(em, (double)P->results[b].eps_obs);
      stats_out->eps_obs_max = em;
    }
  }
  if (dbg_block >= 0 && W->d_dbg.p) {
    std::vector<unsigned long long> h(4096 * 16);
    cudaMemcpy(h.data(), W->d_dbg.p, h.size() * 8, cudaMemcpyDeviceToHost);
    double s[16] = {0};
    int nb = 0;
    for (int c = 0; c < 4096; c++)
      if (h[c * 16 + 3]) { nb++; for (int k = 0; k < 16; k++) s[k] += (double)h[c * 16 + k]; }
    if (nb) {
      fprintf(stderr, "ldw dbg block %lld (%d CTAs, kilo-cycles avg): producer total %.0f wait_jempty %.0f wait_empty %.0f | "
              "mma total %.0f wait_tempty %.0f wait_ready %.0f | expander total %.0f wait_full %.0f | epi(first) total %.0f "
              "wait_jfull %.0f wait_tfull %.0f | epi(last) total %.0f wait_jfull %.0f wait_tfull %.0f\n", (long long)dbg_block, nb,
              s[0] / nb / 1e3, s[1] / nb / 1e3, s[2] / nb / 1e3, s[3] / nb / 1e3, s[4] / nb / 1e3, s[5] / nb / 1e3, s[12] / nb / 1e3,
              s[13] / nb / 1e3, s[6] / nb / 1e3, s[7] / nb / 1e3, s[8] / nb / 1e3, s[9] / nb / 1e3, s[10] / nb / 1e3, s[11] / nb / 1e3);
    }
  }
  kev_cleanup();
  cudaEventDestroy(ev0); cudaEventDestroy(ev1); cudaEventDestroy(ev2); cudaEventDestroy(ev3);
  lap("borderline + stats (host)");
  return 0;
}
```

ldweaver_b200/csrc/mi_types.h:

```cpp
#pragma once
#include <cuda.h>
#include <stdint.h>

namespace ldw {

struct __align__(16) Rec {
  uint32_t T[4];
  float rp[4];
  float q[4];
  uint32_t T4;
  float rp4;
  float q4;
  uint32_t pad;
};
static_assert(sizeof(Rec) == 64, "Rec must be 64 bytes");

struct RowDyn {
  int32_t il;
  float rtl;
};

struct __align__(16) ColDyn {
  int32_t jl;
  float rfl;
  int32_t a0, a1, b0, b1;
  uint32_t baseU, baseL;
};
static_assert(sizeof(ColDyn) == 32, "ColDyn must be 32 bytes");

enum : uint32_t { TILE_HAS_SR = 1u, TILE_NULL = 2u };

struct __align__(16) TileDesc {
  int32_t a_row0, a_pstride;
  int32_t b_row0, b_pstride;
  int32_t i_slot0, j_slot0;
  int32_t i_dyn0, j_dyn0;
  uint8_t PA, PB, njlog2, flags;
  uint8_t flags1, pad8[3];
  int32_t pad[2];
};
static_assert(sizeof(TileDesc) == 48, "TileDesc must be 48 bytes");

struct Cand {
  int32_t il, jl;
  float mi;
};

constexpr int MI_HIST_BINS = 4096;

struct ScanParams {
  const TileDesc* tiles;
  int32_t n_tiles;
  const Rec* rec;
  int64_t rec_vstride;
  const RowDyn* rowdyn;
  const ColDyn* coldyn;
  int32_t nkb;
  int32_t nf, nt;
  int32_t diag, ragged, qcorr, sr_only, dense, emit_all;
  const uint8_t* rfl_arr;
  const uint8_t* rtl_arr;
  float kT;
  uint32_t sa, sb;
  uint32_t M;
  float scale[4][4];
  float q0s[4][4];
  float qod[4][4];
  float rp_qc[4][4];
  float rp_plain[4][4];
  float* sr_out;
  float* dense_out;
  Cand* cand;
  uint32_t cand_cap;
  uint32_t* cand_count;
  uint32_t* tcand_bits;
  uint32_t* hist;
  uint32_t kprime, delta;
  uint32_t* overflow;
  const uint8_t* dig;
  int64_t kpad;
  unsigned long long* dbg;
};

struct TmapSet {
  CUtensorMap a;
  CUtensorMap b[4];
};

}
```

ldweaver_b200/csrc/umma.cuh:

```cuda
#pragma once
#include <cuda_runtime.h>
#include <stdint.h>
#include <stdio.h>

namespace ldw {

__device__ __forceinline__ uint32_t smem_u32(const void* p) { return (uint32_t)__cvta_generic_to_shared(p); }

__device__ __forceinline__ bool elect_one() {
  uint32_t pred;
  asm volatile(
      "{\n"
      ".reg .pred P;\n"
      "elect.sync _|P, 0xffffffff;\n"
      "selp.u32 %0, 1, 0, P;\n"
      "}\n"
      : "=r"(pred));
  return pred != 0;
}

__device__ __forceinline__ void mbar_init(uint64_t* bar, uint32_t count) {
  asm volatile("mbarrier.init.shared::cta.b64 [%0], %1;" ::"r"(smem_u32(bar)), "r"(count) : "memory");
}
__device__ __forceinline__ void fence_barrier_init() { asm volatile("fence.mbarrier_init.release.cluster;" ::: "memory"); }
__device__ __forceinline__ void fence_proxy_async_smem() { asm volatile("fence.proxy.async.shared::cta;" ::: "memory"); }
__device__ __forceinline__ void mbar_arrive_expect_tx(uint64_t* bar, uint32_t bytes) {
  asm volatile("mbarrier.arrive.expect_tx.shared::cta.b64 _, [%0], %1;" ::"r"(smem_u32(bar)), "r"(bytes) : "memory");
}
__device__ __forceinline__ void mbar_arrive(uint64_t* bar) {
  asm volatile("mbarrier.arrive.shared::cta.b64 _, [%0];" ::"r"(smem_u32(bar)) : "memory");
}
__device__ __forceinline__ bool mbar_try_wait(uint64_t* bar, uint32_t parity) {
  uint32_t ok;
  asm volatile(
      "{\n"
      ".reg .pred p;\n"
      "mbarrier.try_wait.parity.shared::cta.b64 p, [%1], %2, %3;\n"
      "selp.u32 %0, 1, 0, p;\n"
      "}\n"
      : "=r"(ok)
      : "r"(smem_u32(bar)), "r"(parity), "r"(0x989680u)
      : "memory");
  return ok != 0;
}
__device__ __forceinline__ uint64_t globaltimer_ns() {
  uint64_t t;
  asm volatile("mov.u64 %0, %%globaltimer;" : "=l"(t));
  return t;
}
#ifndef LDW_WAIT_TIMEOUT_NS
#define LDW_WAIT_TIMEOUT_NS 4000000000ull
#endif
__device__ __forceinline__ void mbar_wait(uint64_t* bar, uint32_t parity, int tag = 0) {
  if (mbar_try_wait(bar, parity)) return;
  uint32_t spins = 0;
  uint64_t t0 = 0;
  while (!mbar_try_wait(bar, parity)) {
    if ((++spins & 0x3FFu) == 0) {
      uint64_t now = globaltimer_ns();
      if (t0 == 0) t0 = now;
      if (now - t0 > LDW_WAIT_TIMEOUT_NS) {
        printf("ldw: mbarrier wait timeout tag=%d block=%d thread=%d parity=%u\n", tag, (int)blockIdx.x,
               (int)threadIdx.x, parity);
        __trap();
      }
    }
  }
}

__device__ __forceinline__ void mbar_arrive_cluster(uint64_t* bar, uint32_t rank) {
  uint32_t ra;
  asm volatile("mapa.shared::cluster.u32 %0, %1, %2;" : "=r"(ra) : "r"(smem_u32(bar)), "r"(rank));
  asm volatile("mbarrier.arrive.shared::cluster.b64 _, [%0];" ::"r"(ra) : "memory");
}

__device__ __forceinline__ void tma_prefetch_desc(const void* tmap) {
  asm volatile("prefetch.tensormap [%0];" ::"l"(reinterpret_cast<uint64_t>(tmap)) : "memory");
}
__device__ __forceinline__ void tma_load_2d(void* smem_dst, const void* tmap, uint64_t* bar, int32_t c0, int32_t c1) {
  asm volatile(
      "cp.async.bulk.tensor.2d.shared::cluster.global.mbarrier::complete_tx::bytes [%0], [%1, {%2, %3}], [%4];"
      ::"r"(smem_u32(smem_dst)), "l"(reinterpret_cast<uint64_t>(tmap)), "r"(c0), "r"(c1), "r"(smem_u32(bar))
      : "memory");
}

__device__ __forceinline__ void tma_load_2d_mc(void* smem_dst, const void* tmap, uint64_t* bar, int32_t c0, int32_t c1,
                                               uint16_t cta_mask) {
  asm volatile(
      "cp.async.bulk.tensor.2d.shared::cluster.global.mbarrier::complete_tx::bytes.multicast::cluster [%0], [%1, {%2, %3}], [%4], %5;"
      ::"r"(smem_u32(smem_dst)), "l"(reinterpret_cast<uint64_t>(tmap)), "r"(c0), "r"(c1), "r"(smem_u32(bar)), "h"(cta_mask)
      : "memory");
}
__device__ __forceinline__ uint32_t cluster_ctarank() {
  uint32_t r;
  asm volatile("mov.u32 %0, %%cluster_ctarank;" : "=r"(r));
  return r;
}
__device__ __forceinline__ void cluster_sync_all() {
  asm volatile("barrier.cluster.arrive.release.aligned;" ::: "memory");
  asm volatile("barrier.cluster.wait.acquire.aligned;" ::: "memory");
}

__device__ __forceinline__ void bulk_load_1d(void* smem_dst, const void* gsrc, uint32_t bytes, uint64_t* bar) {
  asm volatile("cp.async.bulk.shared::cluster.global.mbarrier::complete_tx::bytes [%0], [%1], %2, [%3];" ::"r"(
                   smem_u32(smem_dst)),
               "l"(reinterpret_cast<uint64_t>(gsrc)), "r"(bytes), "r"(smem_u32(bar))
               : "memory");
}

__device__ __forceinline__ void tmem_alloc(uint32_t* smem_dst, uint32_t ncols) {
  asm volatile("tcgen05.alloc.cta_group::1.sync.aligned.shared::cta.b32 [%0], %1;" ::"r"(smem_u32(smem_dst)),
               "r"(ncols)
               : "memory");
  asm volatile("tcgen05.relinquish_alloc_permit.cta_group::1.sync.aligned;" ::: "memory");
}
__device__ __forceinline__ void tmem_dealloc(uint32_t taddr, uint32_t ncols) {
  asm volatile("tcgen05.dealloc.cta_group::1.sync.aligned.b32 %0, %1;" ::"r"(taddr), "r"(ncols) : "memory");
}
__device__ __forceinline__ void tmem_alloc_pair(uint32_t* smem_dst, uint32_t ncols) {
  asm volatile("tcgen05.alloc.cta_group::2.sync.aligned.shared::cta.b32 [%0], %1;" ::"r"(smem_u32(smem_dst)),
               "r"(ncols)
               : "memory");
  asm volatile("tcgen05.relinquish_alloc_permit.cta_group::2.sync.aligned;" ::: "memory");
}
__device__ __forceinline__ void tmem_dealloc_pair(uint32_t taddr, uint32_t ncols) {
  asm volatile("tcgen05.dealloc.cta_group::2.sync.aligned.b32 %0, %1;" ::"r"(taddr), "r"(ncols) : "memory");
}
__device__ __forceinline__ void tc_fence_before() { asm volatile("tcgen05.fence::before_thread_sync;" ::: "memory"); }
__device__ __forceinline__ void tc_fence_after() { asm volatile("tcgen05.fence::after_thread_sync;" ::: "memory"); }

__device__ __forceinline__ void umma_i8(uint32_t tmem_d, uint64_t adesc, uint64_t bdesc, uint32_t idesc,
                                        uint32_t accumulate) {
  asm volatile(
      "{\n"
      ".reg .pred p;\n"
      "setp.ne.b32 p, %4, 0;\n"
      "tcgen05.mma.cta_group::1.kind::i8 [%0], %1, %2, %3, p;\n"
      "}\n" ::"r"(tmem_d),
      "l"(adesc), "l"(bdesc), "r"(idesc), "r"(accumulate)
      : "memory");
}
__device__ __forceinline__ void umma_commit(uint64_t* bar) {
  asm volatile("tcgen05.commit.cta_group::1.mbarrier::arrive::one.shared::cluster.b64 [%0];" ::"r"(smem_u32(bar))
               : "memory");
}

__device__ __forceinline__ void umma_commit_mc(uint64_t* bar, uint16_t cta_mask) {
  asm volatile("tcgen05.commit.cta_group::1.mbarrier::arrive::one.shared::cluster.multicast::cluster.b64 [%0], %1;" ::"r"(
                   smem_u32(bar)),
               "h"(cta_mask)
               : "memory");
}

__device__ __forceinline__ void umma_i8_pair(uint32_t tmem_d, uint64_t adesc, uint64_t bdesc, uint32_t idesc,
                                             uint32_t accumulate) {
  asm volatile(
      "{\n"
      ".reg .pred p;\n"
      "setp.ne.b32 p, %4, 0;\n"
      "tcgen05.mma.cta_group::2.kind::i8 [%0], %1, %2, %3, p;\n"
      "}\n" ::"r"(tmem_d),
      "l"(adesc), "l"(bdesc), "r"(idesc), "r"(accumulate)
      : "memory");
}
__device__ __forceinline__ void umma_commit_pair(uint64_t* bar) {
  asm volatile("tcgen05.commit.cta_group::2.mbarrier::arrive::one.shared::cluster.multicast::cluster.b64 [%0], %1;" ::"r"(
                   smem_u32(bar)),
               "h"((uint16_t)3)
               : "memory");
}

__device__ __forceinline__ void tmem_ld16(uint32_t taddr, uint32_t* v) {
  asm volatile(
      "tcgen05.ld.sync.aligned.32x32b.x16.b32 {%0, %1, %2, %3, %4, %5, %6, %7, %8, %9, %10, %11, %12, %13, %14, %15}, [%16];"
      : "=r"(v[0]), "=r"(v[1]), "=r"(v[2]), "=r"(v[3]), "=r"(v[4]), "=r"(v[5]), "=r"(v[6]), "=r"(v[7]), "=r"(v[8]),
        "=r"(v[9]), "=r"(v[10]), "=r"(v[11]), "=r"(v[12]), "=r"(v[13]), "=r"(v[14]), "=r"(v[15])
      : "r"(taddr));
}
__device__ __forceinline__ void tmem_ld8(uint32_t taddr, uint32_t* v) {
  asm volatile("tcgen05.ld.sync.aligned.32x32b.x8.b32 {%0, %1, %2, %3, %4, %5, %6, %7}, [%8];"
               : "=r"(v[0]), "=r"(v[1]), "=r"(v[2]), "=r"(v[3]), "=r"(v[4]), "=r"(v[5]), "=r"(v[6]), "=r"(v[7])
               : "r"(taddr));
}
__device__ __forceinline__ void tmem_ld4(uint32_t taddr, uint32_t* v) {
  asm volatile("tcgen05.ld.sync.aligned.32x32b.x4.b32 {%0, %1, %2, %3}, [%4];"
               : "=r"(v[0]), "=r"(v[1]), "=r"(v[2]), "=r"(v[3])
               : "r"(taddr));
}
__device__ __forceinline__ void tmem_ld2(uint32_t taddr, uint32_t* v) {
  asm volatile("tcgen05.ld.sync.aligned.32x32b.x2.b32 {%0, %1}, [%2];" : "=r"(v[0]), "=r"(v[1]) : "r"(taddr));
}
template <int N>
__device__ __forceinline__ void tmem_ldn(uint32_t taddr, uint32_t* v) {
  static_assert(N == 16 || N == 8 || N == 4 || N == 2 || N == 1, "unsupported tcgen05.ld width");
  if constexpr (N == 1) asm volatile("tcgen05.ld.sync.aligned.32x32b.x1.b32 {%0}, [%1];" : "=r"(v[0]) : "r"(taddr));
  else if constexpr (N == 16) tmem_ld16(taddr, v);
  else if constexpr (N == 8) tmem_ld8(taddr, v);
  else if constexpr (N == 4) tmem_ld4(taddr, v);
  else tmem_ld2(taddr, v);
}
__device__ __forceinline__ void tmem_ld_wait() { asm volatile("tcgen05.wait::ld.sync.aligned;" ::: "memory"); }

__device__ __forceinline__ uint64_t make_smem_desc_sw128(uint32_t smem_addr) {
  uint64_t d = 0;
  d |= (uint64_t)((smem_addr & 0x3FFFF) >> 4);
  d |= (uint64_t)1 << 16;
  d |= (uint64_t)(1024 >> 4) << 32;
  d |= (uint64_t)1 << 46;
  d |= (uint64_t)2 << 61;
  return d;
}
__host__ __device__ constexpr uint32_t make_idesc_u8(uint32_t M, uint32_t N) {
  return (2u << 4) | ((N >> 3) << 17) | ((M >> 4) << 24);
}
__host__ __device__ constexpr uint32_t make_idesc_s8u8(uint32_t M, uint32_t N) {
  return (2u << 4) | (1u << 7) | ((N >> 3) << 17) | ((M >> 4) << 24);
}

}
```

Baseline: 86.06 billion.

## Schedule MI tiles dynamically via atomic counter and cluster tile queue, add PDL launches

Replaces the static strided tile assignment per CTA pair with a global atomic tile counter. The cluster rank-0 producer fetches each tile index and broadcasts it through an 8-slot shared-memory queue using st.async to both CTAs' MMA and loader warps. A sentinel header now terminates the epilogue. Scan and block-begin kernels launch with programmatic stream serialization so the next kernel can start early, and kernel timing events span chained launches. The aim is to balance uneven tile costs and shrink the tail and launch gaps, at the cost of atomics, extra cluster barriers, and more complex termination logic; a tile-log debug API is added too.

```diff
diff --git a/include/ldw.h b/include/ldw.h
--- a/include/ldw.h
+++ b/include/ldw.h
@@ -151,6 +151,9 @@
 
 LDW_API int ldw_mi_block_dense(ldw_mi_plan* plan, int64_t block_index, double* mi_out, int64_t* nf_out, int64_t* nt_out);
 
+LDW_API int ldw_mi_block_tile_log(ldw_mi_plan* plan, int64_t block_index, uint32_t* log_out, int64_t log_cap,
+                          int64_t* n_tiles_out, int32_t* n_pairs_out);
+
 LDW_API int ldw_mi_pairs_exact(ldw_mi_plan* plan, int64_t block_index, const int32_t* from_local, const int32_t* to_local,
                        int64_t n_pairs, double* mi_out);
 
diff --git a/ldweaver_b200/_lib.py b/ldweaver_b200/_lib.py
--- a/ldweaver_b200/_lib.py
+++ b/ldweaver_b200/_lib.py
@@ -115,6 +115,7 @@
     L.ldw_mi_scan.argtypes = [C.c_void_p, f64, f64, f64, f64, C.c_int, C.c_int, C.c_int, P(Links), P(Links), P(Links),
                               C.c_void_p, C.c_void_p, P(ScanStats)]
     L.ldw_mi_block_dense.argtypes = [C.c_void_p, i64, C.c_void_p, P(i64), P(i64)]
+    L.ldw_mi_block_tile_log.argtypes = [C.c_void_p, i64, C.c_void_p, i64, P(i64), P(C.c_int32)]
     L.ldw_write_lr_tsv.argtypes = [C.c_char_p, P(Links), C.c_int]
     L.ldw_format_r_real.argtypes = [f64, C.c_char_p, C.c_int]
     L.ldw_sr_postprocess.argtypes = [P(Links), C.c_int32, f64, f64, P(SrPost)]
diff --git a/ldweaver_b200/api.py b/ldweaver_b200/api.py
--- a/ldweaver_b200/api.py
+++ b/ldweaver_b200/api.py
@@ -328,6 +328,14 @@
         out = np.zeros((nf.value, nt.value), dtype=np.float64, order="F")
         check(_lib.lib().ldw_mi_block_dense(self.handle, block_index, ptr(out), C.byref(nf), C.byref(nt)))
         return out
+
+    def block_tile_log(self, block_index: int):
+        nt, npairs = C.c_int64(), C.c_int32()
+        check(_lib.lib().ldw_mi_block_tile_log(self.handle, block_index, None, 0, C.byref(nt), C.byref(npairs)))
+        log = np.zeros(2 * max(nt.value, 1), dtype=np.uint32)
+        check(_lib.lib().ldw_mi_block_tile_log(self.handle, block_index, ptr(log), len(log), C.byref(nt), C.byref(npairs)))
+        log = log[:2 * nt.value].reshape(-1, 2)
+        return log[:, 0].copy(), log[:, 1].astype(np.int64), npairs.value
 
     def pairs_exact(self, block_index: int, from_local: np.ndarray, to_local: np.ndarray, out: Optional[np.ndarray] = None) -> np.ndarray:
         f = np.ascontiguousarray(from_local, dtype=np.int32)
diff --git a/ldweaver_b200/csrc/mi_kernel.cuh b/ldweaver_b200/csrc/mi_kernel.cuh
--- a/ldweaver_b200/csrc/mi_kernel.cuh
+++ b/ldweaver_b200/csrc/mi_kernel.cuh
@@ -31,6 +31,8 @@
 constexpr uint32_t MI_JDYN_BYTES = 128 * sizeof(ColDyn);
 constexpr uint32_t MI_IREC_BYTES = 128 * sizeof(Rec);
 constexpr uint32_t MI_IDYN_BYTES = 128 * sizeof(RowDyn);
+constexpr int MI_TQ_SLOTS = 8;
+constexpr int MI_TQ_READERS = 1 + 2 * MI_EXP_WARPS + 1;
 constexpr uint32_t MI_BAR_BYTES = 512;
 constexpr uint32_t MI_SMEM_BYTES = MI_STAGE_REGION + 2 * (MI_JREC_BYTES + MI_JDYN_BYTES) + MI_IREC_BYTES + MI_IDYN_BYTES + MI_BAR_BYTES + 1024;
 static_assert(MI_SMEM_BYTES <= 232448, "shared memory budget (227 KB opt-in)");
@@ -452,14 +454,20 @@
   uint64_t* rempty = bars + 22;
   uint32_t* tmem_slot = reinterpret_cast<uint32_t*>(bars + 23);
   uint32_t* thdr = reinterpret_cast<uint32_t*>(bars + 24);
+  uint64_t* qfull = bars + 40;
+  uint64_t* qempty = bars + 48;
+  uint2* qidx = reinterpret_cast<uint2*>(bars + 56);
+  static_assert((56 + MI_TQ_SLOTS) * 8 <= MI_BAR_BYTES, "barrier region");
 
   const int warp = threadIdx.x >> 5, lane = threadIdx.x & 31;
   const uint32_t rank = cluster_ctarank();
+  if (DBG && p.dbg && threadIdx.x == 0) p.dbg[blockIdx.x * 16 + 15] = globaltimer_ns();
   if (warp == 0 && lane == 0) {
     tma_prefetch_desc(&tm.a);
     for (int i = 0; i < MI_MAX_STAGES; i++) {
       mbar_init(&full[i], 1); mbar_init(&empty[i], 1); mbar_init(&ready[i], 2 * MI_EXP_WARPS);
     }
+    for (int i = 0; i < MI_TQ_SLOTS; i++) { mbar_init(&qfull[i], 1); mbar_init(&qempty[i], MI_TQ_READERS); }
     mbar_init(drained, 1);
     mbar_init(rfull, 1); mbar_init(rempty, MI_EPI_WARPS);
     for (int i = 0; i < 2; i++) {
@@ -473,7 +481,16 @@
   cluster_sync_all();
   tc_fence_after();
   const uint32_t tmem_base = *tmem_slot;
-  const int tile0 = (int)(blockIdx.x >> 1), tstep = (int)(gridDim.x >> 1);
+  auto tq_take = [&](int q, int tag) -> uint2 {
+    const int s = q & (MI_TQ_SLOTS - 1);
+    mbar_wait(&qfull[s], (uint32_t)(q / MI_TQ_SLOTS) & 1, tag);
+    uint2 v = lds64(smem_u32(&qidx[s]));
+    v.x = __shfl_sync(0xffffffffu, v.x, 0);
+    v.y = __shfl_sync(0xffffffffu, v.y, 0);
+    if (lane == 0) mbar_arrive_cluster(&qempty[s], 0);
+    return v;
+  };
+  auto tile_kind = [&](uint32_t t) -> uint32_t { return __ldg(reinterpret_cast<const uint32_t*>(p.tiles + t) + 8) & 0xFFFFFFu; };
 
   if (warp < MI_EPI_WARP0) {
   asm volatile("setmaxnreg.dec.sync.aligned.u32 " LDW_STR(MI_REGS_CTRL) ";");
@@ -481,7 +498,34 @@
     int st = 0; uint32_t phb = 0; int geo = -1; uint32_t dph = 0;
     int it = 0, rit = 0;
     long long w_jempty = 0, w_empty = 0, t_begin = DBG ? clock64() : 0;
-    for (int t = tile0; t < p.n_tiles; t += tstep, it++) {
+    uint32_t cur = 0, nxt = 0, nkind = 0;
+    auto publish = [&](int q) {
+      const int s = q & (MI_TQ_SLOTS - 1);
+      timed_wait<DBG>(&qempty[s], ((uint32_t)(q / MI_TQ_SLOTS) & 1) ^ 1, 14, w_jempty);
+      if (lane == 0) {
+        st_async_v2_cluster(&qidx[s], nxt, nkind, &qfull[s], 0);
+        st_async_v2_cluster(&qidx[s], nxt, nkind, &qfull[s], 1);
+        cur = nxt;
+        if (nxt < (uint32_t)p.n_tiles) nxt = atomicAdd(p.tile_ctr, 1u);
+      }
+    };
+    if (rank == 0) {
+      if (lane == 0) {
+        nxt = atomicAdd(p.tile_ctr, 1u);
+        if (nxt < (uint32_t)p.n_tiles) nkind = tile_kind(nxt);
+      }
+      publish(0);
+      if (lane == 0 && nxt < (uint32_t)p.n_tiles) nkind = tile_kind(nxt);
+    }
+    for (;; it++) {
+      int t;
+      if (rank == 0) {
+        t = (int)__shfl_sync(0xffffffffu, cur, 0);
+        if (t < p.n_tiles) publish(it + 1);
+      } else {
+        t = (int)tq_take(it, 15).x;
+      }
+      if (t >= p.n_tiles) break;
       const TileDesc td = p.tiles[t];
       const int PA = td.PA, PB = td.PB, NJ = 1 << td.njlog2, NJh = NJ >> 1;
       const int njidx = 7 - td.njlog2;
@@ -530,6 +574,17 @@
         __syncwarp();
         rit++;
       }
+      if (rank == 0 && lane == 0 && nxt < (uint32_t)p.n_tiles) nkind = tile_kind(nxt);
+    }
+    grid_launch_dependents();
+    {
+      const int jb = it & 1;
+      timed_wait<DBG>(&jempty[jb], ((it >> 1) & 1) ^ 1, 10, w_jempty);
+      if (elect_one()) {
+        thdr[jb] = 0;
+        mbar_arrive(&jfull[jb]);
+      }
+      __syncwarp();
     }
     if (DBG && p.dbg && lane == 0) {
       p.dbg[blockIdx.x * 16 + 0] = (unsigned long long)(clock64() - t_begin);
@@ -541,17 +596,19 @@
     int st = 0; uint32_t phb = 0; int geo = -1; int as = 0; uint32_t aph = 0;
     long long w_tempty = 0, w_ready = 0, t_begin = DBG ? clock64() : 0;
     const uint32_t desc_hi = (uint32_t)(make_smem_desc_sw128(0) >> 32);
-    for (int t = tile0; t < p.n_tiles; t += tstep) {
-      const TileDesc td = p.tiles[t];
-      const int PA = td.PA, PB = td.PB, NJ = 1 << td.njlog2;
-      const int g = mi_stage_geo(PA, PB, td.njlog2);
+    for (int q = 0;; q++) {
+      const uint2 tq = tq_take(q, 23);
+      const int t = (int)tq.x;
+      if (t >= p.n_tiles) break;
+      const int PA = (int)(tq.y & 0xFF), PB = (int)((tq.y >> 8) & 0xFF), njlog2 = (int)(tq.y >> 16);
+      const int NJ = 1 << njlog2;
+      const int g = mi_stage_geo(PA, PB, njlog2);
       const int nst = mi_geo_stages(g);
       const uint32_t sbytes = mi_geo_bytes(g);
-      if (g != geo) { geo = g; st = 0; }
-      bool sw = false;
-      if (t + tstep < p.n_tiles) {
-        const TileDesc tn = p.tiles[t + tstep];
-        sw = mi_stage_geo(tn.PA, tn.PB, tn.njlog2) != g;
+      if (g != geo) {
+        if (geo >= 0 && elect_one()) umma_commit_pair(drained);
+        __syncwarp();
+        geo = g; st = 0;
       }
       const bool big = 2 * PA * PB * NJ > 256;
       const uint32_t ncols = (uint32_t)(2 * PB * NJ);
@@ -599,7 +656,7 @@
         }
       }
       if (elect_one()) {
-        if (sw) umma_commit_pair(drained);
+        if (p.tile_log) { atomicAdd(&p.tile_log[2 * t], 1u); p.tile_log[2 * t + 1] = blockIdx.x >> 1; }
         if (big) {
           umma_commit_pair(&tfull[0]);
           umma_commit_pair(&tfull[1]);
@@ -622,11 +679,13 @@
     const int h = (warp - 2) * 32 + lane;
     int st = 0; uint32_t phb = 0; int geo = -1;
     long long w_full = 0, t_begin = DBG ? clock64() : 0;
-    for (int t = tile0; t < p.n_tiles; t += tstep) {
-      const TileDesc td = p.tiles[t];
-      const int PA = td.PA, PB = td.PB, NJh = (1 << td.njlog2) >> 1;
+    for (int q = 0;; q++) {
+      const uint2 tq = tq_take(q, 41);
+      if ((int)tq.x >= p.n_tiles) break;
+      const int PA = (int)(tq.y & 0xFF), PB = (int)((tq.y >> 8) & 0xFF), njlog2 = (int)(tq.y >> 16);
+      const int NJh = (1 << njlog2) >> 1;
       const int brows = PB * NJh;
-      const int g = mi_stage_geo(PA, PB, td.njlog2);
+      const int g = mi_stage_geo(PA, PB, njlog2);
       const int nst = mi_geo_stages(g);
       const uint32_t sbytes = mi_geo_bytes(g);
       if (g != geo) { geo = g; st = 0; }
@@ -662,6 +721,7 @@
   }
   } else {
     asm volatile("setmaxnreg.inc.sync.aligned.u32 " LDW_STR(MI_REGS_EPI) ";");
+    grid_dependency_wait();
     EpiCtx c;
     c.q = warp & 3;
     c.cg = (warp - MI_EPI_WARP0) >> 2;
@@ -674,11 +734,12 @@
     c.idyn_saddr = smem_u32(idyn);
     c.rempty_saddr = smem_u32(rempty);
     c.scr_saddr = smem_u32(bars + 32) + (uint32_t)(warp - MI_EPI_WARP0) * 4u;
-    for (int t = tile0; t < p.n_tiles; t += tstep, it++) {
+    for (;; it++) {
       const int jb = it & 1;
       timed_wait<DBG>(&jfull[jb], (it >> 1) & 1, 30, w_jfull);
       uint32_t hdr;
       asm volatile("ld.shared.u32 %0, [%1];" : "=r"(hdr) : "r"(smem_u32(&thdr[jb])));
+      if (hdr == 0) break;
       const int tPA = (int)(hdr & 0xFF), tPB = (int)((hdr >> 8) & 0xFF);
       c.tflags = hdr >> 24;
       const int NJ = 1 << ((hdr >> 16) & 0xFF);
@@ -731,6 +792,7 @@
   }
   tc_fence_before();
   cluster_sync_all();
+  if (DBG && p.dbg && threadIdx.x == 0) p.dbg[blockIdx.x * 16 + 14] = globaltimer_ns();
   if (warp == 2) {
     tc_fence_after();
     tmem_dealloc_pair(tmem_base, 512);
diff --git a/ldweaver_b200/csrc/mi_scan.cu b/ldweaver_b200/csrc/mi_scan.cu
--- a/ldweaver_b200/csrc/mi_scan.cu
+++ b/ldweaver_b200/csrc/mi_scan.cu
@@ -56,7 +56,7 @@
   static constexpr int RING = 4;
   BlockDev ring[RING];
   BlockHost hring[RING];
-  DevBuf d_dbg;
+  DevBuf d_dbg, d_tile_ctr , d_tile_log;
   struct LrBuf {
     DevBuf cand, vcand, mi64, state , hist;
     cudaEvent_t scan_done = nullptr, sel_done = nullptr;
@@ -634,10 +634,19 @@
 
 int launch_scan(const ldw_mi_plan* P, const ScanParams& sp, cudaStream_t st, int reserve = 0) {
   if (sp.n_tiles <= 0) return 0;
-  int grid = 2 * std::min<int>(sp.n_tiles, std::max(1, (P->ctx->num_sms - reserve) / 2));
-  if (sp.dbg) mi_scan_kernel<true><<<grid, MI_THREADS, MI_SMEM_BYTES, st>>>(P->tm, sp);
-  else mi_scan_kernel<false><<<grid, MI_THREADS, MI_SMEM_BYTES, st>>>(P->tm, sp);
-  LDW_CUDA(cudaGetLastError());
+  const int grid = 2 * std::min<int>(sp.n_tiles, std::max(1, (P->ctx->num_sms - reserve) / 2));
+  cudaLaunchAttribute attr[1];
+  attr[0].id = cudaLaunchAttributeProgrammaticStreamSerialization;
+  attr[0].val.programmaticStreamSerializationAllowed = 1;
+  cudaLaunchConfig_t cfg = {};
+  cfg.gridDim = dim3((unsigned)grid);
+  cfg.blockDim = dim3(MI_THREADS);
+  cfg.dynamicSmemBytes = MI_SMEM_BYTES;
+  cfg.stream = st;
+  cfg.attrs = attr;
+  cfg.numAttrs = 1;
+  if (sp.dbg) LDW_CUDA(cudaLaunchKernelEx(&cfg, mi_scan_kernel<true>, P->tm, sp));
+  else LDW_CUDA(cudaLaunchKernelEx(&cfg, mi_scan_kernel<false>, P->tm, sp));
   return 0;
 }
 
@@ -725,7 +734,10 @@
   delete plan;
 }
 
-int ldw_mi_block_dense(ldw_mi_plan* P, int64_t block_index, double* mi_out, int64_t* nf_out, int64_t* nt_out) {
+}
+
+static int block_dense_impl(ldw_mi_plan* P, int64_t block_index, double* mi_out, int64_t* nf_out, int64_t* nt_out,
+                            uint32_t* tile_log, int64_t log_cap, int64_t* n_tiles_out, int32_t* n_pairs_out) {
   if (!P) return set_error(LDW_ERR_ARG, "null plan");
   LDW_TRY(ctx_bind(P->ctx));
   cudaStream_t st = P->ctx->stream;
@@ -749,22 +761,48 @@
   if (e > 1) return e;
   if (nf_out) *nf_out = H.nf;
   if (nt_out) *nt_out = H.nt;
-  if (!mi_out) return 0;
+  if (n_tiles_out) *n_tiles_out = H.n_real_tiles;
+  if (n_pairs_out) *n_pairs_out = std::min<int>(H.n_real_tiles, std::max(1, P->ctx->num_sms / 2));
+  if (!mi_out && !tile_log) return 0;
+  if (tile_log && log_cap < 2 * (int64_t)H.n_real_tiles) return set_error(LDW_ERR_ARG, "tile log holds %lld words, the block needs %lld", (long long)log_cap, 2 * (long long)H.n_real_tiles);
   LDW_TRY(upload_block(st, D, H));
   size_t cells = (size_t)H.nf * H.nt;
   LDW_TRY(W->d_dense.ensure(cells * 4));
   LDW_CUDA(cudaMemsetAsync(W->d_dense.p, 0, cells * 4, st));
+  LDW_TRY(W->d_tile_ctr.ensure(4));
+  LDW_CUDA(cudaMemsetAsync(W->d_tile_ctr.p, 0, 4, st));
   ScanParams sp;
   fill_scan_params(P, D, H, cfg, sp);
   sp.dense = 1;
   sp.dense_out = W->d_dense.as<float>();
+  sp.tile_ctr = W->d_tile_ctr.as<uint32_t>();
+  const size_t log_bytes = (size_t)std::max<int32_t>(H.n_real_tiles, 1) * 8;
+  if (tile_log) {
+    LDW_TRY(W->d_tile_log.ensure(log_bytes));
+    LDW_CUDA(cudaMemsetAsync(W->d_tile_log.p, 0, log_bytes, st));
+    sp.tile_log = W->d_tile_log.as<uint32_t>();
+  }
   LDW_TRY(launch_scan(P, sp, st));
-  DevBuf d64;
-  LDW_TRY(d64.alloc(cells * 8));
-  f32_to_f64_kernel<<<(unsigned)((cells + 255) / 256), 256, 0, st>>>(W->d_dense.as<float>(), (int64_t)cells, d64.as<double>());
-  LDW_CUDA(cudaMemcpyAsync(mi_out, d64.p, cells * 8, cudaMemcpyDeviceToHost, st));
+  if (tile_log) LDW_CUDA(cudaMemcpyAsync(tile_log, W->d_tile_log.p, (size_t)H.n_real_tiles * 8, cudaMemcpyDeviceToHost, st));
+  if (mi_out) {
+    DevBuf d64;
+    LDW_TRY(d64.alloc(cells * 8));
+    f32_to_f64_kernel<<<(unsigned)((cells + 255) / 256), 256, 0, st>>>(W->d_dense.as<float>(), (int64_t)cells, d64.as<double>());
+    LDW_CUDA(cudaMemcpyAsync(mi_out, d64.p, cells * 8, cudaMemcpyDeviceToHost, st));
+  }
   LDW_CUDA(cudaStreamSynchronize(st));
   return 0;
+}
+
+extern "C" {
+
+int ldw_mi_block_dense(ldw_mi_plan* P, int64_t block_index, double* mi_out, int64_t* nf_out, int64_t* nt_out) {
+  return block_dense_impl(P, block_index, mi_out, nf_out, nt_out, nullptr, 0, nullptr, nullptr);
+}
+
+int ldw_mi_block_tile_log(ldw_mi_plan* P, int64_t block_index, uint32_t* log_out, int64_t log_cap, int64_t* n_tiles_out,
+                          int32_t* n_pairs_out) {
+  return block_dense_impl(P, block_index, nullptr, nullptr, nullptr, log_out, log_cap, n_tiles_out, n_pairs_out);
 }
 
 int ldw_mi_pairs_exact(ldw_mi_plan* P, int64_t block_index, const int32_t* from_local, const int32_t* to_local,
@@ -991,6 +1029,9 @@
   uint32_t* d_kept_overflow = W->d_state.as<uint32_t>() + 3;
   uint32_t* d_chain2 = W->d_state.as<uint32_t>() + 8;
   LDW_CUDA(cudaMemsetAsync(W->d_state.p, 0, 64, st));
+  LDW_TRY(W->d_tile_ctr.ensure((blocks.size() + 1) * 4));
+  LDW_CUDA(cudaMemsetAsync(W->d_tile_ctr.p, 0, (blocks.size() + 1) * 4, st));
+  uint32_t* d_tile_ctr = W->d_tile_ctr.as<uint32_t>();
   cudaStream_t sst = P->ctx->select_stream;
 
   const bool want_host = !(flags & (LDW_SCAN_NO_LINKS | LDW_SCAN_NO_D2H));
@@ -1021,7 +1062,9 @@
   if (const char* e = getenv("LDW_DBG_FORCE_SEED")) force_seed = (float)atof(e);
   double sel_margin0 = 4e-6;
   if (const char* e = getenv("LDW_DBG_SEL_MARGIN")) sel_margin0 = atof(e);
-  auto run_block = [&](size_t b, size_t seq, int force_emit_all, uint32_t cap_override, bool use_chain, double sel_margin) -> int {
+  bool span_open = false;
+  auto run_block = [&](size_t b, size_t seq, int force_emit_all, uint32_t cap_override, bool use_chain, double sel_margin,
+                       bool chain_next) -> int {
     Sel& s = sel[b];
     if (s.skip) return 0;
     int slot = (int)(seq % ScanWS::RING);
@@ -1051,6 +1094,8 @@
     ScanParams sp;
     fill_scan_params(P, D, H, cfg, sp);
     sp.sr_out = W->d_sr_f32.as<float>() + s.sr_base;
+    sp.tile_ctr = d_tile_ctr + b;
+    if (!use_chain) LDW_CUDA(cudaMemsetAsync(sp.tile_ctr, 0, 4, st));
     if (dbg_block >= 0 && (int64_t)b == dbg_block) {
       LDW_TRY(W->d_dbg.ensure(4096 * 16 * 8));
       LDW_CUDA(cudaMemsetAsync(W->d_dbg.p, 0, 4096 * 16 * 8, st));
@@ -1067,6 +1112,7 @@
         ScanParams pp = sp;
         pp.tiles = D.tiles.as<TileDesc>() + H.n_real_tiles;
         pp.n_tiles = n_pilot;
+        pp.tile_ctr = d_tile_ctr + blocks.size();
         pp.cand = L.cand.as<Cand>(); pp.cand_cap = cap; pp.cand_count = d_count; pp.tcand_bits = d_tcand;
         pp.hist = L.hist.as<uint32_t>(); pp.kprime = s.kprime; pp.delta = s.delta ? s.delta : 1; pp.overflow = d_overflow;
         pp.emit_all = 1;
@@ -1081,8 +1127,19 @@
         LDW_CUDA(cudaMemcpyAsync(d_chain, &force_seed, 4, cudaMemcpyHostToDevice, st));
         LDW_CUDA(cudaStreamSynchronize(st));
       }
-      mi_block_begin_kernel<<<1, 256, 0, st>>>(d_count, L.hist.as<uint32_t>(), d_chain, (use_chain && !emit_all) ? 1 : 0);
-      LDW_CUDA(cudaGetLastError());
+      {
+        cudaLaunchAttribute attr[1];
+        attr[0].id = cudaLaunchAttributeProgrammaticStreamSerialization;
+        attr[0].val.programmaticStreamSerializationAllowed = 1;
+        cudaLaunchConfig_t lc = {};
+        lc.gridDim = dim3(1);
+        lc.blockDim = dim3(256);
+        lc.stream = st;
+        lc.attrs = attr;
+        lc.numAttrs = 1;
+        LDW_CUDA(cudaLaunchKernelEx(&lc, mi_block_begin_kernel, d_count, L.hist.as<uint32_t>(), (const uint32_t*)d_chain,
+                                    (use_chain && !emit_all) ? 1 : 0));
+      }
       n_launches++;
       sp.cand = L.cand.as<Cand>();
       sp.cand_cap = cap;
@@ -1097,14 +1154,20 @@
       sp.sr_only = 1;
     }
     if (sp.n_tiles > 0) {
-      cudaEvent_t k0, k1;
-      LDW_CUDA(cudaEventCreate(&k0));
-      LDW_CUDA(cudaEventCreate(&k1));
-      kev.push_back(k0);
-      kev.push_back(k1);
-      LDW_CUDA(cudaEventRecord(k0, st));
+      if (!span_open) {
+        cudaEvent_t k0, k1;
+        LDW_CUDA(cudaEventCreate(&k0));
+        LDW_CUDA(cudaEventCreate(&k1));
+        kev.push_back(k0);
+        kev.push_back(k1);
+        LDW_CUDA(cudaEventRecord(k0, st));
+        span_open = true;
+      }
       LDW_TRY(launch_scan(P, sp, st, lr ? scan_reserve : 0));
-      LDW_CUDA(cudaEventRecord(k1, st));
+      if (!chain_next || (s.n_sr > 0 && sr_rows)) {
+        LDW_CUDA(cudaEventRecord(kev.back(), st));
+        span_open = false;
+      }
       n_launches++; n_scan_launches++;
       n_tiles += sp.n_tiles;
       for (int32_t ti = 0; ti < H.n_real_tiles; ti++) {
@@ -1184,7 +1247,11 @@
   std::vector<size_t> order;
   for (size_t b = 0; b < blocks.size(); b++) if (sel[b].n_sr > 0) order.push_back(b);
   for (size_t b = 0; b < blocks.size(); b++) if (!(sel[b].n_sr > 0)) order.push_back(b);
-  for (size_t k = 0; k < order.size(); k++) LDW_TRY(run_block(order[k], k, 0, 0, true, sel_margin0));
+  for (size_t k = 0; k < order.size(); k++) LDW_TRY(run_block(order[k], k, 0, 0, true, sel_margin0, k + 1 < order.size()));
+  if (span_open) {
+    LDW_CUDA(cudaEventRecord(kev.back(), st));
+    span_open = false;
+  }
   for (auto& l : W->lr)
     if (l.used) LDW_CUDA(cudaStreamWaitEvent(st, l.sel_done, 0));
   LDW_CUDA(cudaEventRecord(ev1, st));
@@ -1220,7 +1287,7 @@
             LDW_TRY(L.mi64.ensure((size_t)cap * 8));
             LDW_TRY(L.vcand.ensure((size_t)cap * sizeof(Cand)));
           }
-          LDW_TRY(run_block(b, 0, attempt == 1, cap, false, margin));
+          LDW_TRY(run_block(b, 0, attempt == 1, cap, false, margin, false));
           LDW_CUDA(cudaStreamWaitEvent(st, W->lr[0].sel_done, 0));
           LDW_CUDA(cudaStreamSynchronize(st));
           P->results[b] = W->h_results.as<BlockResult>()[b];
@@ -1406,6 +1473,16 @@
               "wait_jfull %.0f wait_tfull %.0f | epi(last) total %.0f wait_jfull %.0f wait_tfull %.0f\n", (long long)dbg_block, nb,
               s[0] / nb / 1e3, s[1] / nb / 1e3, s[2] / nb / 1e3, s[3] / nb / 1e3, s[4] / nb / 1e3, s[5] / nb / 1e3, s[12] / nb / 1e3,
               s[13] / nb / 1e3, s[6] / nb / 1e3, s[7] / nb / 1e3, s[8] / nb / 1e3, s[9] / nb / 1e3, s[10] / nb / 1e3, s[11] / nb / 1e3);
+      unsigned long long t0 = ~0ull, e0 = ~0ull, e1 = 0;
+      for (int c = 0; c < 4096; c++)
+        if (h[c * 16 + 14]) {
+          t0 = std::min(t0, h[c * 16 + 15]);
+          e0 = std::min(e0, h[c * 16 + 14]);
+          e1 = std::max(e1, h[c * 16 + 14]);
+        }
+      if (e1 > t0)
+        fprintf(stderr, "ldw dbg block %lld: launch %.1f us (first CTA start to last CTA end), CTA end times spread over %.1f us "
+                "(%.2f %% of the launch)\n", (long long)dbg_block, (e1 - t0) / 1e3, (e1 - e0) / 1e3, 100.0 * (double)(e1 - e0) / (double)(e1 - t0));
     }
   }
   kev_cleanup();
diff --git a/ldweaver_b200/csrc/mi_types.h b/ldweaver_b200/csrc/mi_types.h
--- a/ldweaver_b200/csrc/mi_types.h
+++ b/ldweaver_b200/csrc/mi_types.h
@@ -79,7 +79,9 @@
   uint32_t* overflow;
   const uint8_t* dig;
   int64_t kpad;
+  uint32_t* tile_ctr;
   unsigned long long* dbg;
+  uint32_t* tile_log;
 };
 
 struct TmapSet {
diff --git a/ldweaver_b200/csrc/umma.cuh b/ldweaver_b200/csrc/umma.cuh
--- a/ldweaver_b200/csrc/umma.cuh
+++ b/ldweaver_b200/csrc/umma.cuh
@@ -73,6 +73,17 @@
   asm volatile("mapa.shared::cluster.u32 %0, %1, %2;" : "=r"(ra) : "r"(smem_u32(bar)), "r"(rank));
   asm volatile("mbarrier.arrive.shared::cluster.b64 _, [%0];" ::"r"(ra) : "memory");
 }
+__device__ __forceinline__ void st_async_v2_cluster(uint2* dst, uint32_t a, uint32_t b, uint64_t* bar, uint32_t rank) {
+  uint32_t rd, rb;
+  asm volatile("mapa.shared::cluster.u32 %0, %1, %2;" : "=r"(rd) : "r"(smem_u32(dst)), "r"(rank));
+  asm volatile("mapa.shared::cluster.u32 %0, %1, %2;" : "=r"(rb) : "r"(smem_u32(bar)), "r"(rank));
+  asm volatile("mbarrier.arrive.expect_tx.shared::cluster.b64 _, [%0], 8;" ::"r"(rb) : "memory");
+  asm volatile("st.async.shared::cluster.mbarrier::complete_tx::bytes.v2.u32 [%0], {%1, %2}, [%3];" ::"r"(rd), "r"(a), "r"(b),
+               "r"(rb)
+               : "memory");
+}
+__device__ __forceinline__ void grid_launch_dependents() { asm volatile("griddepcontrol.launch_dependents;" ::: "memory"); }
+__device__ __forceinline__ void grid_dependency_wait() { asm volatile("griddepcontrol.wait;" ::: "memory"); }
 
 __device__ __forceinline__ void tma_prefetch_desc(const void* tmap) {
   asm volatile("prefetch.tensormap [%0];" ::"l"(reinterpret_cast<uint64_t>(tmap)) : "memory");
```

After: 78.44 billion (median of 6 runs). 0.912x the previous value.
